# blairstar/NaturalDiffusion

Measured on AMD Instinct MI355X. Metric: images/sec at 15-step Natural Inference (CIFAR10 32x32, NCSN++), 3-stream throughput, higher is better.
Workload: dtype bf16; 1 GPU; CIFAR10 NI 15-step step_15_weight_173.npz B=512/GPU NCSN++ 61.8M bf16, ni_step fp64 history; nfe=15, batch_per_gpu=512, streams=3

## Files before the change

include/natinf_ncsnpp.h:

```cpp
#ifndef NATINF_NCSNPP_H
#define NATINF_NCSNPP_H

#include <stdint.h>
#include "natinf.h"

#ifdef __cplusplus
extern "C" {
#endif

typedef struct natinf_ncsnpp* natinf_ncsnpp_t;

#define NATINF_NCSNPP_KEEP_ACTIVATIONS 1
#define NATINF_NCSNPP_DDPM 2

int64_t natinf_ncsnpp_param_count(void);
int64_t natinf_ncsnpp_packed_bytes(void);
int64_t natinf_ncsnpp_handle_param_count(natinf_ncsnpp_t h);
int64_t natinf_ncsnpp_handle_packed_bytes(natinf_ncsnpp_t h);
int64_t natinf_ncsnpp_workspace_bytes(natinf_ncsnpp_t h, int max_batch);

int natinf_ncsnpp_create(natinf_ncsnpp_t* out, int flags);
int natinf_ncsnpp_destroy(natinf_ncsnpp_t h);

int natinf_ncsnpp_describe(natinf_ncsnpp_t h, char* buf, int cap);

int natinf_ncsnpp_load(natinf_ncsnpp_t h, const float* params_f32, int64_t n_params,
                       void* packed, int64_t packed_bytes, natinf_stream_t stream);

int natinf_ncsnpp_share(natinf_ncsnpp_t h, natinf_ncsnpp_t loaded);

int natinf_ncsnpp_forward(natinf_ncsnpp_t h, const float* x, const float* labels, float* out, int B,
                          void* workspace, int64_t workspace_bytes, natinf_stream_t stream);

int natinf_ncsnpp_describe_gemms(natinf_ncsnpp_t h, int B, char* buf, int cap);

int natinf_debug_gemm(int variant, int M, int N, int K0, int K1, int taps, int logW, int batch,
                      const void* a0, const void* a1, const void* b, const float* bias_n, void* c, int c_f32, float scale,
                      int iters, natinf_stream_t stream);
int natinf_debug_quant_fp8_rows(const float* w, void* q, float* row_scale, int rows, int cols, natinf_stream_t stream);
int natinf_debug_gemm_fused(int variant, int M, int N, int K, const void* a, const void* b, const float* bias_n, const float* bias_m,
                            const float* rowvec, const float* gate, int log_rows_per_sample, const void* resid_bf16, const float* resid_f32,
                            float scale, int act, void* c, int c_f32, float* gn_part, int* bm_out, int fp32_slab, natinf_stream_t stream);
int natinf_debug_set_conv_operand(int logW, const void* a1, int c1);
int natinf_debug_gemm_fp8(int M, int N, int K, const void* a8, const float* a_scale, const void* a_mx, const void* b8, const float* b_scale,
                          const float* bias_n, void* c, void* c_mx, int c_mode, int iters, natinf_stream_t stream);
int natinf_debug_conv_gn_up(int flags);
int natinf_debug_conv_gn_fin(float* fin_scale, float* fin_shift, const float* gamma, const float* beta, int channels_per_group, float mul);
int natinf_debug_conv_gn(int res, int B, int N, int cin, int c1, const void* x, const float* scale, const float* shift, const void* w_packed, void* w_frag,
                         const void* a1, const float* bias_n, const void* resid, float out_scale, void* out, float* gn_part, int iters,
                         natinf_stream_t stream);
#define NATINF_ATTN_BLOCK_OFF_WQKV 0
#define NATINF_ATTN_BLOCK_OFF_W3 393216
#define NATINF_ATTN_BLOCK_OFF_FOLD_WQK 524288
#define NATINF_ATTN_BLOCK_OFF_FOLD_WVO 786432
#define NATINF_ATTN_BLOCK_OFF_FOLD_CQ 1048576
#define NATINF_ATTN_BLOCK_OFF_FOLD_BO 1049600
#define NATINF_ATTN_BLOCK_OFF_WQK_PACKED 1050624
#define NATINF_ATTN_BLOCK_OFF_WVO_PACKED 1181696
#define NATINF_ATTN_BLOCK_PACKED_BYTES 1312768
#define NATINF_ATTN_BLOCK_SCRATCH_BYTES_PER_SAMPLE 393216
int natinf_debug_attn_block(int plan, int B, const void* x, int x_ld, const float* scale, const float* shift, const float* w, const float* bias,
                            void* packed, void* scratch, void* out, int o_ld, float out_scale, float* gn_part, natinf_stream_t stream);
int natinf_set_gemm_variant(int variant);
int natinf_set_gemm_epilogue(int fp32_slab);
int natinf_set_gemm_pref512(int on);
int natinf_set_gemm_half_issue(int on);
int natinf_set_gemm_round_model(int on);
int natinf_set_gemm_w128(int on);
int natinf_set_gemm_raster(int rows);
int natinf_set_fuse_gn(int on);
int natinf_set_conv_gn_wide(int mask);
int natinf_set_conv_gn_w128(int mask);
int natinf_set_conv_gn_w128_min_k(int shape, int k);
int natinf_set_conv_gn_regw(int on);
int natinf_set_fuse_up(int on);
int natinf_set_fuse_up_fold(int on);
int natinf_debug_fold_up_weights(const float* w, int N, int cin, float w_mul, float* out_f32, void* out_packed, natinf_stream_t stream);
int natinf_debug_conv_up_fold(int B, int N, int cin, const void* x, const float* scale, const float* shift, const float* w, void* w_packed, void* h_scratch,
                              const float* bias_n, const float* rowvec, float out_scale, void* out, float* gn_part, int iters, natinf_stream_t stream);
int natinf_set_fuse_head(int on);
int natinf_set_fuse_gn8(int on);
int natinf_set_fuse_gn4(int on);
int natinf_set_fuse_fin(int on);
int natinf_set_conv_gn_warm(int mask);
int natinf_set_attn256(int on);
int natinf_set_attn_proj(int on);
int natinf_set_attn_waves8(int on);
int natinf_set_attn_block(int on);
int natinf_set_attn_qkv(int on);
int natinf_set_conv_gn8_tile(int one_image);
int natinf_set_gemm_splitk(int on);
int natinf_debug_set_splitk_workspace(float* ws, int max_slices);
int natinf_debug_timestamps(void* dev_buf16);

int natinf_ncsnpp_profile(natinf_ncsnpp_t h, int enable);
int natinf_ncsnpp_profile_read(natinf_ncsnpp_t h, double* ms_by_class , int64_t* launches_by_class );

int natinf_gemm_profile(int enable);
int natinf_gemm_profile_read(char* buf, int cap);

int natinf_ncsnpp_debug_tap(natinf_ncsnpp_t h, int module_idx, float* out, int64_t capacity_elems,
                            natinf_stream_t stream);

int natinf_debug_gn_stats(const void* x, int ld, int C, int HW, int B, const float* gamma, const float* beta, float* scale, float* shift, float eps, float out_mul,
                          natinf_stream_t stream);
int natinf_debug_gn_finalize(const float* P0, int tps0, int quads0, const float* P1, int tps1, int quads1, int C, int HW, int B, const float* gamma, const float* beta,
                             float* scale, float* shift, float eps, float out_mul, natinf_stream_t stream);
int natinf_debug_gn_fold(const float* P, int tps, int quads, int fold, int B, float* out, natinf_stream_t stream);
int natinf_debug_gn_apply(const void* x, int ld, int C, int logW, int logHW, int B, const float* scale, const float* shift, void* y, void* xr, int act, int mode, int pad,
                          natinf_stream_t stream);
int natinf_debug_head_conv(const void* x, int ld, int B, const float* scale, const float* shift, const void* w16, const float* bias, float* out, natinf_stream_t stream);
int natinf_debug_time_embed(const float* labels, void* emb, int B, natinf_stream_t stream);
int natinf_debug_stem_im2col(const float* x, void* A, int B, natinf_stream_t stream);
int natinf_debug_pack_conv(const float* src, void* dst, int N, int Cin, int taps, int dst_ld, int koff, int tap_stride_c, int chunked, float wmul, natinf_stream_t stream);
int natinf_debug_pack_transpose(const float* src, void* dst, int K, int N, int dst_ld, natinf_stream_t stream);
int natinf_debug_nhwc_to_nchw(const void* x, int ld, int C, int HW, int B, float* out, natinf_stream_t stream);

#ifdef __cplusplus
}
#endif
#endif
```

naturaldiffusion_amd/_lib.py:

```python
from __future__ import annotations

import ctypes as C
import os
from pathlib import Path

os.environ.setdefault("GPU_MAX_HW_QUEUES", "8")

_HERE = Path(__file__).resolve().parent
LIB_PATH = Path(os.environ.get("NATINF_LIB", _HERE / "libnatinf.so"))

if not LIB_PATH.exists():
    raise ImportError(
        f"{LIB_PATH} not found: build it with `make -C {_HERE / 'csrc'}` "
        "(or `python -c 'import __graft_entry__ as g; g.build()'`). "
        "naturaldiffusion_amd has no CPU or eager-PyTorch fallback.")

lib = C.CDLL(str(LIB_PATH))

_p, _i32, _i64, _f32, _f64 = C.c_void_p, C.c_int, C.c_int64, C.c_float, C.c_double

SIGNATURES = {
    "natinf_abi_version": (C.c_int, []),
    "natinf_strerror": (C.c_char_p, [_i32]),
    "natinf_probe": (C.c_int, []),
    "natinf_step_f64hist": (C.c_int, [_p, _p, _p, _p, _p, _p, _p, _i32, _f64, _i32, _f64, _f64, _f32, _f32, _i64, _p]),
    "natinf_step_f32hist": (C.c_int, [_p, _p, _p, _p, _p, _p, _p, _i32, _f32, _i32, _f32, _f32, _f32, _f32, _i64, _p]),
    "natinf_weighted_sum_f64": (C.c_int, [_p, _p, _p, _p, _i32, _i64, _p]),
    "natinf_randn_philox_f32": (C.c_int, [_p, _i64, _i64, _p, _i64, _i64, C.c_uint64, _p]),
    "natinf_randn_philox_col_f32": (C.c_int, [_p, _i64, _i64, _p, _i64, _i64, C.c_uint64, C.c_uint32, _p]),
    "natinf_step_f64hist_noise": (C.c_int, [_p, _p, _p, _p, _p, _p, _p, _i32, _f64, _p, _p, _i32, _i32, _f64, _f64, _f32,
                                            C.c_uint64, _p, _i64, _i64, _i64, _i64, _p]),
    "natinf_known_blend_f32": (C.c_int, [_p, _p, _p, _p, _i64, _i64, _f32, _f32, C.c_uint32, C.c_uint64, _p, _i64, _i64, _i64, _i64, _p]),
    "natinf_step_f64hist_inpaint": (C.c_int, [_p, _p, _p, _p, _p, _p, _p, _i32, _f64, _p, _p, _i32, _i32, _f64, _f64, _f32,
                                              C.c_uint64, _p, _i64, _i64, _i64, _i64, _p, _p, _i64, _i64, _f32, _f32, C.c_uint32, _p]),
    "natinf_x0_threshold_f64": (C.c_int, [_p, _p, _i64, _i64, _i32, _f64, _f64, _p]),
    "natinf_step_f64hist_x0fix": (C.c_int, [_p, _p, _p, _p, _p, _p, _p, _i32, _f64, _p, _p, _i32, _i32, _f64, _f64, _f32,
                                            C.c_uint64, _p, _i64, _i64, _i64, _i64, _p, _p, _i64, _i64, _f32, _f32, C.c_uint32,
                                            _i32, _f64, _f64, _p, _p]),
    "natinf_color_blend_f32": (C.c_int, [_p, _p, _p, _i64, _p, _p, _f32, _f32, C.c_uint32, C.c_uint64, _p, _i64, _i64, _i64, _i64, _p]),
    "natinf_step_f64hist_colorize": (C.c_int, [_p, _p, _p, _p, _p, _p, _p, _i32, _f64, _p, _p, _i32, _i32, _f64, _f64, _f32,
                                               C.c_uint64, _p, _i64, _i64, _i64, _i64, _p, _i64, _p, _p, _f32, _f32, C.c_uint32, _p]),
    "natinf_to_pixel_u8": (C.c_int, [_p, _p, _i32, _i32, _i32, _i32, _i32, _p]),
    "natinf_step_f32prod": (C.c_int, [_p, _p, _p, _f32, _i64, _i64, _p, _p, _p, _p, _p, _i32, _f32, _p, _p, _i32,
                                      _i32, _f32, _f32, _i64, _p]),
    "natinf_step_f32prod_noise": (C.c_int, [_p, _p, _p, _f32, _i64, _i64, _p, _p, _p, _p, _p, _i32, _f32, _p, _p, _i32,
                                            _i32, _f32, _f32, C.c_uint64, _p, _i64, _i64, _i64, _p]),
    "natinf_step_f32prod_noise_guided": (C.c_int, [_p, _p, _p, _p, _p, _i32, _i64, _i64, _p, _p, _p, _p, _p, _i32, _f32, _p, _p, _i32,
                                                   _i32, _f32, _f32, C.c_uint64, _p, _i64, _i64, _i64, _p]),
    "natinf_step_f32prod_inpaint": (C.c_int, [_p, _p, _p, _p, _p, _i32, _i64, _i64, _p, _p, _p, _p, _p, _i32, _f32, _p, _p, _i32,
                                              _i32, _f32, _f32, C.c_uint64, _p, _i64, _i64, _i64,
                                              _p, _p, _i64, _i64, _f32, _f32, C.c_uint32, _p]),
    "natinf_weighted_sum_f32prod": (C.c_int, [_p, _p, _p, _p, _i32, _i64, _p]),
    "natinf_step_f16chain": (C.c_int, [_p, _p, _p, _p, _p, _p, _p, _p, _p, _i32, _f32, _f32, _i32, _f32, _f32, _f32,
                                       _f32, _i32, _i64, _p]),
    "natinf_step_f16chain_guided": (C.c_int, [_p, _p, _p, _p, _p, _i32, _i64, _p, _p, _p, _p, _p, _p, _i32, _f32, _f32, _i32, _f32, _f32,
                                              _f32, _i32, _i64, _p]),
    "natinf_known_blend_f16": (C.c_int, [_p, _p, _p, _p, _p, _i64, _i64, _f32, _f32, C.c_uint32, C.c_uint64, _p, _i64, _i64, _i64, _i64, _p]),
    "natinf_step_f16chain_inpaint": (C.c_int, [_p, _p, _p, _p, _p, _i32, _i64, _p, _p, _p, _p, _p, _p, _i32, _f32, _f32, _i32, _f32, _f32,
                                               _f32, _i32, _i64, _p, _p, _i64, _i64, C.c_uint32, C.c_uint64, _p, _i64, _i64, _p]),
    "natinf_weighted_mean_f16": (C.c_int, [_p, _p, _p, _p, _i32, _f32, _i64, _p]),
    "natinf_flow_input_f16": (C.c_int, [_p, _p, _p, _f32, _f32, _i64, _p]),
    "natinf_ncsnpp_param_count": (C.c_int64, []),
    "natinf_ncsnpp_workspace_bytes": (C.c_int64, [_p, _i32]),
    "natinf_ncsnpp_packed_bytes": (C.c_int64, []),
    "natinf_ncsnpp_handle_param_count": (_i64, [_p]),
    "natinf_ncsnpp_handle_packed_bytes": (_i64, [_p]),
    "natinf_ncsnpp_create": (C.c_int, [C.POINTER(_p), _i32]),
    "natinf_ncsnpp_describe": (C.c_int, [_p, C.c_char_p, _i32]),
    "natinf_ncsnpp_destroy": (C.c_int, [_p]),
    "natinf_ncsnpp_load": (C.c_int, [_p, _p, _i64, _p, _i64, _p]),
    "natinf_ncsnpp_share": (C.c_int, [_p, _p]),
    "natinf_ncsnpp_forward": (C.c_int, [_p, _p, _p, _p, _i32, _p, _i64, _p]),
    "natinf_ncsnpp_debug_tap": (C.c_int, [_p, _i32, _p, _i64, _p]),
    "natinf_ncsnpp_describe_gemms": (C.c_int, [_p, _i32, C.c_char_p, _i32]),
    "natinf_debug_gemm": (C.c_int, [_i32, _i32, _i32, _i32, _i32, _i32, _i32, _i32, _p, _p, _p, _p, _p, _i32, _f32, _i32, _p]),
    "natinf_set_gemm_variant": (C.c_int, [_i32]),
    "natinf_debug_timestamps": (C.c_int, [_p]),
    "natinf_set_gemm_epilogue": (C.c_int, [_i32]),
    "natinf_debug_gemm_fused": (C.c_int, [_i32, _i32, _i32, _i32, _p, _p, _p, _p, _p, _p, _i32, _p, _p, _f32, _i32, _p, _i32, _p, _p, _i32, _p]),
    "natinf_set_gemm_pref512": (C.c_int, [_i32]),
    "natinf_set_gemm_half_issue": (C.c_int, [_i32]),
    "natinf_set_gemm_raster": (C.c_int, [_i32]),
    "natinf_set_gemm_round_model": (C.c_int, [_i32]),
    "natinf_set_gemm_w128": (C.c_int, [_i32]),
    "natinf_set_fuse_gn": (C.c_int, [_i32]),
    "natinf_set_conv_gn_wide": (C.c_int, [_i32]),
    "natinf_set_attn_block": (C.c_int, [_i32]),
    "natinf_set_conv_gn_w128": (C.c_int, [_i32]),
    "natinf_set_conv_gn_w128_min_k": (C.c_int, [_i32, _i32]),
    "natinf_set_conv_gn_regw": (C.c_int, [_i32]),
    "natinf_set_fuse_up": (C.c_int, [_i32]),
    "natinf_set_fuse_up_fold": (C.c_int, [_i32]),
    "natinf_debug_fold_up_weights": (C.c_int, [_p, _i32, _i32, _f32, _p, _p, _p]),
    "natinf_debug_conv_up_fold": (C.c_int, [_i32, _i32, _i32, _p, _p, _p, _p, _p, _p, _p, _p, _f32, _p, _p, _i32, _p]),
    "natinf_set_fuse_head": (C.c_int, [_i32]),
    "natinf_set_fuse_gn8": (C.c_int, [_i32]),
    "natinf_set_fuse_gn4": (C.c_int, [_i32]),
    "natinf_set_fuse_fin": (C.c_int, [_i32]),
    "natinf_set_attn_proj": (C.c_int, [_i32]),
    "natinf_set_attn_waves8": (C.c_int, [_i32]),
    "natinf_set_attn_qkv": (C.c_int, [_i32]),
    "natinf_set_conv_gn_warm": (C.c_int, [_i32]),
    "natinf_set_attn256": (C.c_int, [_i32]),
    "natinf_set_conv_gn8_tile": (C.c_int, [_i32]),
    "natinf_set_gemm_splitk": (C.c_int, [_i32]),
    "natinf_debug_set_splitk_workspace": (C.c_int, [_p, _i32]),
    "natinf_debug_set_conv_operand": (C.c_int, [_i32, _p, _i32]),
    "natinf_debug_conv_gn": (C.c_int, [_i32, _i32, _i32, _i32, _i32, _p, _p, _p, _p, _p, _p, _p, _p, _f32, _p, _p, _i32, _p]),
    "natinf_debug_conv_gn_up": (C.c_int, [_i32]),
    "natinf_debug_conv_gn_fin": (C.c_int, [_p, _p, _p, _p, _i32, _f32]),
    "natinf_debug_attn_block": (C.c_int, [_i32, _i32, _p, _i32, _p, _p, _p, _p, _p, _p, _p, _i32, _f32, _p, _p]),
    "natinf_debug_gn_stats": (C.c_int, [_p, _i32, _i32, _i32, _i32, _p, _p, _p, _p, _f32, _f32, _p]),
    "natinf_debug_gn_finalize": (C.c_int, [_p, _i32, _i32, _p, _i32, _i32, _i32, _i32, _i32, _p, _p, _p, _p, _f32, _f32, _p]),
    "natinf_debug_gn_fold": (C.c_int, [_p, _i32, _i32, _i32, _i32, _p, _p]),
    "natinf_debug_gn_apply": (C.c_int, [_p, _i32, _i32, _i32, _i32, _i32, _p, _p, _p, _p, _i32, _i32, _i32, _p]),
    "natinf_debug_head_conv": (C.c_int, [_p, _i32, _i32, _p, _p, _p, _p, _p, _p]),
    "natinf_debug_time_embed": (C.c_int, [_p, _p, _i32, _p]),
    "natinf_debug_stem_im2col": (C.c_int, [_p, _p, _i32, _p]),
    "natinf_debug_pack_conv": (C.c_int, [_p, _p, _i32, _i32, _i32, _i32, _i32, _i32, _i32, _f32, _p]),
    "natinf_debug_pack_transpose": (C.c_int, [_p, _p, _i32, _i32, _i32, _p]),
    "natinf_debug_nhwc_to_nchw": (C.c_int, [_p, _i32, _i32, _i32, _i32, _p, _p]),
    "natinf_ncsnpp_profile": (C.c_int, [_p, _i32]),
    "natinf_ncsnpp_profile_read": (C.c_int, [_p, C.POINTER(C.c_double), C.POINTER(C.c_int64)]),
    "natinf_debug_quant_fp8_rows": (C.c_int, [_p, _p, _p, _i32, _i32, _p]),
    "natinf_debug_gemm_fp8": (C.c_int, [_i32, _i32, _i32, _p, _p, _p, _p, _p, _p, _p, _p, _i32, _i32, _p]),
    "natinf_dit_create": (C.c_int, [C.POINTER(_p), _i32, _i32, _i32, _i32]),
    "natinf_dit_create_sized": (C.c_int, [C.POINTER(_p), _i32, _i32, _i32, _i32, _i32]),
    "natinf_dit_input_size": (C.c_int, [_p]),
    "natinf_dit_attention_bf16": (C.c_int, [_p, _p, _p, _i32, _p, _i32, _i32, _i32, _i32, _i32, _i32, _p]),
    "natinf_dit_destroy": (C.c_int, [_p]),
    "natinf_dit_param_count": (C.c_int64, [_p]),
    "natinf_dit_packed_bytes": (C.c_int64, [_p]),
    "natinf_dit_workspace_bytes": (C.c_int64, [_p, _i32]),
    "natinf_dit_load": (C.c_int, [_p, _p, _i64, _p, _i64, _p]),
    "natinf_dit_forward": (C.c_int, [_p, _p, _p, _p, _p, _i32, _p, _i64, _p]),
    "natinf_dit_stream_sites": (C.c_int, [_p]),
    "natinf_dit_stream_status_reset": (C.c_int, [_p, _p, _p]),
    "natinf_dit_stream_status": (C.c_int, [_p, _p, _p, _p]),
    "natinf_debug_ln_modulate": (C.c_int, [_p, _i32, _p, _p, _i32, _p, _p, _p, _i32, _i64, _i32, C.POINTER(_i32), _p]),
    "natinf_debug_softmax_rows": (C.c_int, [_i32, _p, _p, _i32, _i64, _p]),
    "natinf_mmdit_create": (C.c_int, [C.POINTER(_p), _i32, _i32, _i32, _i32, _i32, _i32, _i32, _i32]),
    "natinf_mmdit_destroy": (C.c_int, [_p]),
    "natinf_mmdit_param_count": (C.c_int64, [_p]),
    "natinf_mmdit_packed_bytes": (C.c_int64, [_p]),
    "natinf_mmdit_workspace_bytes": (C.c_int64, [_p, _i32]),
    "natinf_mmdit_load": (C.c_int, [_p, _p, _i64, _p, _i64, _p]),
    "natinf_mmdit_forward": (C.c_int, [_p, _p, _p, _p, _p, _p, _i32, _p, _i64, _p]),
    "natinf_mmdit_stream_sites": (C.c_int, [_p]),
    "natinf_mmdit_stream_status_reset": (C.c_int, [_p, _p, _p]),
    "natinf_mmdit_stream_status": (C.c_int, [_p, _p, _p, _p]),
    "natinf_attention_hd64_bf16": (C.c_int, [_p, _p, _i32, _i64, _p, _p, _i32, _i64, _i32, _i32, _i32, _i32, C.c_float, _p]),
    "natinf_debug_attention_hd64_fp8out": (C.c_int, [_p, _p, _i32, _i64, _p, _p, _p, _i32, _i32, _i32, _i32, C.c_float, _p]),
    "natinf_inception_create": (C.c_int, [_p, _i32, _i32]),
    "natinf_inception_destroy": (C.c_int, [_p]),
    "natinf_set_inception_conv": (C.c_int, [_i32]),
    "natinf_debug_conv_ring": (C.c_int, [_i32] * 14 + [_p, _p, _p, _p, _p, _p, _i32, _p]),
    "natinf_debug_inc_stem": (C.c_int, [_p, _i32, _i32, _i32, _i32, _i32, _i32, _p, _p]),
    "natinf_debug_inc_pool": (C.c_int, [_i32] * 8 + [_p, _i32, _p, _i32, _p]),
    "natinf_debug_inc_global_avg": (C.c_int, [_i32, _i32, _i32, _i32, _p, _p, _p]),
    "natinf_debug_inc_pack": (C.c_int, [_i32, _p, _p, _p, _p, _p] + [_i32] * 7 + [_p, _p, _p, _p]),
    "natinf_debug_inc_im2col": (C.c_int, [_i32] * 11 + [_p, _p, _p]),
    "natinf_inception_param_count": (_i64, [_p]),
    "natinf_inception_packed_bytes": (_i64, [_p]),
    "natinf_inception_workspace_bytes": (_i64, [_p, _i32]),
    "natinf_inception_load": (C.c_int, [_p, _p, _i64, _p, _i64, _p]),
    "natinf_inception_forward": (C.c_int, [_p, _p, _i32, _p, _i32, _p, _i64, _p]),
    "natinf_gemm_profile": (C.c_int, [_i32]),
    "natinf_gemm_profile_read": (C.c_int, [_p, _i32]),
    "natinf_set_mmdit_stream16": (C.c_int, [_i32]),
    "natinf_set_dit_stream16": (C.c_int, [_i32]),
    "natinf_set_mmdit_text_flat": (C.c_int, [_i32]),
    "natinf_attention_profile": (C.c_int, [_i32]),
    "natinf_set_mmdit_text_stream": (C.c_int, [_i32]),
    "natinf_set_flash_mode": (C.c_int, [_i32]),
    "natinf_attention_profile_read": (C.c_int, [_p, _p]),
    "natinf_vae_create": (C.c_int, [C.POINTER(_p), _i32, _i32]),
    "natinf_vae_destroy": (C.c_int, [_p]),
    "natinf_vae_param_count": (C.c_int64, [_p]),
    "natinf_vae_packed_bytes": (C.c_int64, [_p]),
    "natinf_vae_workspace_bytes": (C.c_int64, [_p, _i32]),
    "natinf_vae_load": (C.c_int, [_p, _p, _i64, _p, _i64, _p]),
# ... 100 lines not shown
```

naturaldiffusion_amd/csrc/attn_blk256.h:

```cpp
#pragma once
#include "attn_qkv.h"
#include "attn256.h"

namespace ncsn {

constexpr int ABLK_STAGES = 4, ABLK_LDS_BYTES = ABLK_STAGES * A256_STAGE + QKV_BIAS_BYTES;

__device__ __forceinline__ float dpp_row_sum_tau(float a, float b) {
    asm volatile("s_nop 4" : "+v"(a), "+v"(b));
    a += __builtin_bit_cast(float, __builtin_amdgcn_update_dpp(0, __builtin_bit_cast(int, a), 0x128, 0xF, 0xF, true));
    b += __builtin_bit_cast(float, __builtin_amdgcn_update_dpp(0, __builtin_bit_cast(int, b), 0x128, 0xF, 0xF, true));
    asm volatile("" : "+v"(a), "+v"(b));
    a += __builtin_bit_cast(float, __builtin_amdgcn_update_dpp(0, __builtin_bit_cast(int, a), 0xB1, 0xF, 0xF, true));
    b += __builtin_bit_cast(float, __builtin_amdgcn_update_dpp(0, __builtin_bit_cast(int, b), 0xB1, 0xF, 0xF, true));
    asm volatile("" : "+v"(a), "+v"(b));
    a += __builtin_bit_cast(float, __builtin_amdgcn_update_dpp(0, __builtin_bit_cast(int, a), 0x4E, 0xF, 0xF, true));
    b += __builtin_bit_cast(float, __builtin_amdgcn_update_dpp(0, __builtin_bit_cast(int, b), 0x4E, 0xF, 0xF, true));
    asm volatile("" : "+v"(a), "+v"(b));
    float v = a + b;
    asm volatile("s_nop 1" : "+v"(v));
    v += __builtin_bit_cast(float, __builtin_amdgcn_update_dpp(0, __builtin_bit_cast(int, v), 0x141, 0xF, 0xF, true));
    asm volatile("" : "+v"(v));
    return v;
}
// ... 237 lines not shown
            for (int i = 0; i < 4; ++i) { of[g][kc][i] = (bf16)oacc[g][2 * kc][i]; of[g][kc][4 + i] = (bf16)oacc[g][2 * kc + 1][i]; }
    __builtin_amdgcn_sched_barrier(0);
    int le;
    asm volatile("v_mbcnt_lo_u32_b32 %0, -1, 0\n\tv_mbcnt_hi_u32_b32 %0, -1, %0" : "=v"(le));
    const int re = le & 15, qe = le >> 4;
    float2* const sred = reinterpret_cast<float2*>(smem);
    float2 part[16];
#pragma unroll
    for (int t = 0; t < 4; ++t) {
        asm volatile("s_waitcnt vmcnt(0)" ::: "memory");
        __syncthreads();
        if (t + 3 < 4) issue(2 * NKT + t + 3);
        __builtin_amdgcn_sched_barrier(0);
        const unsigned char* sW = smem + ((2 * NKT + t) & 3) * A256_STAGE;
        f32x4 a3[2][4];
#pragma unroll
        for (int ntl = 0; ntl < 4; ++ntl) { a3[0][ntl] = f32x4{0.f, 0.f, 0.f, 0.f}; a3[1][ntl] = f32x4{0.f, 0.f, 0.f, 0.f}; }
#pragma unroll
        for (int ntl = 0; ntl < 4; ++ntl)
#pragma unroll
            for (int kc = 0; kc < 8; ++kc) {
                const bf16x8 fa = *reinterpret_cast<const bf16x8*>(sW + (ntl * 8 + kc) * 1024 + le * 16);
                a3[0][ntl] = __builtin_amdgcn_mfma_f32_16x16x32_bf16(fa, of[0][kc], a3[0][ntl], 0, 0, 0);
                a3[1][ntl] = __builtin_amdgcn_mfma_f32_16x16x32_bf16(fa, of[1][kc], a3[1][ntl], 0, 0, 0);
            }
#pragma unroll
        for (int pr = 0; pr < 2; ++pr) {
            const int n = 64 * t + 32 * pr + 8 * qe;
            const float4 b0 = *reinterpret_cast<const float4*>(b3 + n), b1 = *reinterpret_cast<const float4*>(b3 + n + 4);
            float s0[2], ss0[2], s1[2], ss1[2];
#pragma unroll
            for (int g = 0; g < 2; ++g) {
                const int64_t row = (int64_t)b * T + tok0 + 8 * (re >> 2) + 4 * g + (re & 3);
                const bf16x8 rx = *reinterpret_cast<const bf16x8*>(x + row * x_ld + n);
                const f32x4 lo = a3[g][2 * pr], hi = a3[g][2 * pr + 1];
                float v[8] = {lo[0] + b0.x, lo[1] + b0.y, lo[2] + b0.z, lo[3] + b0.w, hi[0] + b1.x, hi[1] + b1.y, hi[2] + b1.z, hi[3] + b1.w};
                bf16x8 w;
#pragma unroll
                for (int i = 0; i < 8; ++i) { v[i] = (v[i] + (float)rx[i]) * out_scale; w[i] = (bf16)v[i]; }
                *reinterpret_cast<bf16x8*>(o + row * o_ld + n) = w;
                s0[g] = (v[0] + v[1]) + (v[2] + v[3]);  ss0[g] = (v[0] * v[0] + v[1] * v[1]) + (v[2] * v[2] + v[3] * v[3]);
                s1[g] = (v[4] + v[5]) + (v[6] + v[7]);  ss1[g] = (v[4] * v[4] + v[5] * v[5]) + (v[6] * v[6] + v[7] * v[7]);
            }
            part[4 * t + 2 * pr] = make_float2(dpp_row_sum_tau(s0[0], s0[1]), dpp_row_sum_tau(ss0[0], ss0[1]));
            part[4 * t + 2 * pr + 1] = make_float2(dpp_row_sum_tau(s1[0], s1[1]), dpp_row_sum_tau(ss1[0], ss1[1]));
        }
    }
    if (gn_part) {
        __syncthreads();
        if (re == 0) {
#pragma unroll
            for (int k = 0; k < 16; ++k) sred[wave * 64 + 8 * (k >> 1) + 2 * qe + (k & 1)] = part[k];
        }
        __syncthreads();
        if (tid < 64) {
            float s = 0.f, ss = 0.f;
#pragma unroll
            for (int w = 0; w < 8; ++w) { s += sred[w * 64 + tid].x; ss += sred[w * 64 + tid].y; }
            gn_part[(int64_t)b * gn_quads + tid] = make_float2(s, ss);
        }
    }
}

constexpr int ABLK2_IMG = 131072, ABLK2_LDS_BYTES = ABLK2_IMG + A256_STAGE;
static_assert(4 * QKV_STAGE <= ABLK2_IMG && ABLK2_LDS_BYTES <= 163840, "the q phase's four stages inside the image's bytes; image + one W3 tile in 160 KB");

__global__ __launch_bounds__(256) void k_attn_fold_w(const float* __restrict__ w0, const float* __restrict__ w1, const float* __restrict__ w2, const float* __restrict__ w3,
                                                      const float* __restrict__ b0, const float* __restrict__ b2, const float* __restrict__ b3,
                                                      float* __restrict__ wqk, float* __restrict__ cq, float* __restrict__ wvo, float* __restrict__ bo)
{
    const int o = threadIdx.x, i = blockIdx.x;
    float a = 0.f, c = 0.f;
    if (i < 256) {
        for (int m = 0; m < 256; ++m) { a += w0[i * 256 + m] * w1[o * 256 + m]; c += w2[i * 256 + m] * w3[m * 256 + o]; }
        wqk[i * 256 + o] = a; wvo[i * 256 + o] = c;
    } else {
        for (int m = 0; m < 256; ++m) { a += b0[m] * w1[o * 256 + m]; c += b2[m] * w3[m * 256 + o]; }
        cq[o] = a; bo[o] = c + b3[o];
    }
}

__global__ __launch_bounds__(512, 1) void k_attn_blk256_v2(const bf16* __restrict__ x, int x_ld, const float* __restrict__ gsc, const float* __restrict__ gsh,
                                                          const bf16* __restrict__ wqf, const float* __restrict__ cq, float scale, const bf16* __restrict__ wvof,
                                                          const float* __restrict__ bo, bf16* __restrict__ o, int o_ld, float out_scale, float2* __restrict__ gn_part, int gn_quads)
{
    constexpr int T = 256, C = 256, NTQ = 8;
    extern __shared__ __attribute__((aligned(16))) unsigned char smem[];
    lds_poison();
    typedef __attribute__((address_space(3))) void lds_void;
    typedef __attribute__((address_space(3))) unsigned char lds_u8;
    const int tid = threadIdx.x, lane = tid & 63, r = lane & 15, q = lane >> 4;
    const int wave = __builtin_amdgcn_readfirstlane(tid >> 6);
    const int b = blockIdx.x;
    const int tok0 = wave * 32;
    const unsigned lds0 = (unsigned)(uintptr_t)((lds_u8*)smem);

    constexpr int NST = 4, AHEAD = NST - 1;
    auto issue_w = [&](int i) __attribute__((always_inline)) {
        unsigned char* st = smem + (i & (NST - 1)) * QKV_STAGE;
        int l;
        asm volatile("v_mbcnt_lo_u32_b32 %0, -1, 0\n\tv_mbcnt_hi_u32_b32 %0, -1, %0" : "=v"(l));
        const bf16* base = wqf + (int64_t)i * (QKV_STAGE / 2);
#pragma unroll
        for (int j = 0; j < QKV_STAGE / 8192; ++j) {
            const int p = wave * (QKV_STAGE / 8192) + j;
            __builtin_amdgcn_global_load_lds(base + p * 512 + l * 8, (lds_void*)(st + p * 1024), 16, 0, 0);
        }
    };
    issue_w(0); issue_w(1); issue_w(2);
    float* const sBias = reinterpret_cast<float*>(smem + ABLK2_IMG);
    const unsigned lds_bias = lds0 + ABLK2_IMG;
    if (tid < 64) reinterpret_cast<float4*>(sBias)[tid] = reinterpret_cast<const float4*>(cq)[tid];

    bf16x8 qf[2][8];
    {
        bf16x8 hf[2][8];
        {
            const bf16* xb = x + ((int64_t)b * T + tok0 + 8 * (r >> 2) + (r & 3)) * x_ld + 8 * q;
            bf16x8 raw[2][8];
#pragma unroll
            for (int g = 0; g < 2; ++g)
#pragma unroll
                for (int kc = 0; kc < 8; ++kc) raw[g][kc] = *reinterpret_cast<const bf16x8*>(xb + (int64_t)(4 * g) * x_ld + 32 * kc);
            const float* sc = gsc + (int64_t)b * C + 8 * q;
            const float* sh = gsh + (int64_t)b * C + 8 * q;
#pragma unroll
            for (int kc = 0; kc < 8; ++kc) {
                const float4 s0 = *reinterpret_cast<const float4*>(sc + 32 * kc), s1 = *reinterpret_cast<const float4*>(sc + 32 * kc + 4);
                const float4 h0 = *reinterpret_cast<const float4*>(sh + 32 * kc), h1 = *reinterpret_cast<const float4*>(sh + 32 * kc + 4);
                const float s[8] = {s0.x, s0.y, s0.z, s0.w, s1.x, s1.y, s1.z, s1.w}, h[8] = {h0.x, h0.y, h0.z, h0.w, h1.x, h1.y, h1.z, h1.w};
#pragma unroll
                for (int g = 0; g < 2; ++g)
#pragma unroll
                    for (int j = 0; j < 8; ++j) hf[g][kc][j] = (bf16)((float)raw[g][kc][j] * s[j] + h[j]);
            }
        }
        int le;
        asm volatile("v_mbcnt_lo_u32_b32 %0, -1, 0\n\tv_mbcnt_hi_u32_b32 %0, -1, %0" : "=v"(le));
        const int qe = le >> 4;
        auto q_tile = [&](auto t_tag, bf16x8 (&w)[2]) __attribute__((always_inline)) {
            constexpr int t = decltype(t_tag)::value;
            constexpr int ahead = 2 * ((t + 1 < NTQ) + (t + 2 < NTQ));
            asm volatile("s_waitcnt vmcnt(%0) lgkmcnt(0)" :: "n"(ahead) : "memory");
            __builtin_amdgcn_s_barrier();
            if constexpr (t + AHEAD < NTQ) issue_w(t + AHEAD);
            __builtin_amdgcn_sched_barrier(0);
            const unsigned char* sW = smem + (t & (NST - 1)) * QKV_STAGE;
            f32x4 a[2][2];
#pragma unroll
            for (int ntl = 0; ntl < 2; ++ntl) {
                a[ntl][0] = f32x4{0.f, 0.f, 0.f, 0.f}; a[ntl][1] = a[ntl][0];
#pragma unroll
                for (int kc = 0; kc < 8; ++kc) {
                    const bf16x8 fa = *reinterpret_cast<const bf16x8*>(sW + (ntl * 8 + kc) * 1024 + le * 16);
                    a[ntl][0] = __builtin_amdgcn_mfma_f32_16x16x32_bf16(fa, hf[0][kc], a[ntl][0], 0, 0, 0);
                    a[ntl][1] = __builtin_amdgcn_mfma_f32_16x16x32_bf16(fa, hf[1][kc], a[ntl][1], 0, 0, 0);
                }
            }
            const int n = 32 * t + 8 * qe;
            f32x4 b0, b1;
            asm volatile("ds_read_b128 %0, %2\n\tds_read_b128 %1, %2 offset:16" : "=&v"(b0), "=&v"(b1) : "v"(lds_bias + (unsigned)n * 4u) : "memory");
            asm volatile("s_waitcnt lgkmcnt(0)" : "+v"(b0), "+v"(b1) :: "memory");
#pragma unroll
            for (int g = 0; g < 2; ++g)
#pragma unroll
                for (int i = 0; i < 4; ++i) { w[g][i] = (bf16)(a[0][g][i] + b0[i]); w[g][4 + i] = (bf16)(a[1][g][i] + b1[i]); }
        };
// ... 89 lines not shown
            for (int cc = 0; cc < 2; ++cc)
#pragma unroll
                for (int dt = 0; dt < 16; ++dt) {
                    const unsigned a = abase + (unsigned)((64 * vt + 32 * cc) * 512) + ((((unsigned)dt ^ kh) << 5) | (kl << 4));
                    const s16x4 lo = __builtin_amdgcn_ds_read_tr16_b64_v4i16((lds_s16x4*)(uintptr_t)a);
                    const s16x4 hi = __builtin_amdgcn_ds_read_tr16_b64_v4i16((lds_s16x4*)(uintptr_t)(a + 4 * 512));
                    typedef short s16x8 __attribute__((ext_vector_type(8)));
                    const s16x8 both = {lo[0], lo[1], lo[2], lo[3], hi[0], hi[1], hi[2], hi[3]};
                    const bf16x8 fv = __builtin_bit_cast(bf16x8, both);
                    oacc[0][dt] = __builtin_amdgcn_mfma_f32_16x16x32_bf16(fv, pf[0][2 * vt + cc], oacc[0][dt], 0, 0, 0);
                    oacc[1][dt] = __builtin_amdgcn_mfma_f32_16x16x32_bf16(fv, pf[1][2 * vt + cc], oacc[1][dt], 0, 0, 0);
                }
    }
    bf16x8 of[2][8];
#pragma unroll
    for (int g = 0; g < 2; ++g)
#pragma unroll
        for (int kc = 0; kc < 8; ++kc)
#pragma unroll
            for (int i = 0; i < 4; ++i) { of[g][kc][i] = (bf16)oacc[g][2 * kc][i]; of[g][kc][4 + i] = (bf16)oacc[g][2 * kc + 1][i]; }
    __builtin_amdgcn_sched_barrier(0);
    asm volatile("s_waitcnt lgkmcnt(0)" ::: "memory");
    __syncthreads();
    issue3(1); issue3(2); issue3(3);

    int le;
    asm volatile("v_mbcnt_lo_u32_b32 %0, -1, 0\n\tv_mbcnt_hi_u32_b32 %0, -1, %0" : "=v"(le));
    const int re = le & 15, qe = le >> 4;
    float2 part[16];
#pragma unroll
    for (int t = 0; t < 4; ++t) {
        if (t == 0) {
            asm volatile("s_waitcnt vmcnt(0)" ::: "memory");
            __syncthreads();
        }
        __builtin_amdgcn_sched_barrier(0);
        const unsigned char* sW = t == 0 ? smem + ABLK2_IMG : smem + (t - 1) * A256_STAGE;
        f32x4 a3[2][4];
#pragma unroll
        for (int ntl = 0; ntl < 4; ++ntl) { a3[0][ntl] = f32x4{0.f, 0.f, 0.f, 0.f}; a3[1][ntl] = f32x4{0.f, 0.f, 0.f, 0.f}; }
#pragma unroll
        for (int ntl = 0; ntl < 4; ++ntl)
#pragma unroll
            for (int kc = 0; kc < 8; ++kc) {
                const bf16x8 fa = *reinterpret_cast<const bf16x8*>(sW + (ntl * 8 + kc) * 1024 + le * 16);
                a3[0][ntl] = __builtin_amdgcn_mfma_f32_16x16x32_bf16(fa, of[0][kc], a3[0][ntl], 0, 0, 0);
                a3[1][ntl] = __builtin_amdgcn_mfma_f32_16x16x32_bf16(fa, of[1][kc], a3[1][ntl], 0, 0, 0);
            }
#pragma unroll
        for (int pr = 0; pr < 2; ++pr) {
            const int n = 64 * t + 32 * pr + 8 * qe;
            const float4 b0 = *reinterpret_cast<const float4*>(bo + n), b1 = *reinterpret_cast<const float4*>(bo + n + 4);
            float s0[2], ss0[2], s1[2], ss1[2];
#pragma unroll
            for (int g = 0; g < 2; ++g) {
                const int64_t row = (int64_t)b * T + tok0 + 8 * (re >> 2) + 4 * g + (re & 3);
                const bf16x8 rx = *reinterpret_cast<const bf16x8*>(x + row * x_ld + n);
                const f32x4 lo = a3[g][2 * pr], hi = a3[g][2 * pr + 1];
                float v[8] = {lo[0] + b0.x, lo[1] + b0.y, lo[2] + b0.z, lo[3] + b0.w, hi[0] + b1.x, hi[1] + b1.y, hi[2] + b1.z, hi[3] + b1.w};
                bf16x8 w;
#pragma unroll
                for (int i = 0; i < 8; ++i) { v[i] = (v[i] + (float)rx[i]) * out_scale; w[i] = (bf16)v[i]; }
                *reinterpret_cast<bf16x8*>(o + row * o_ld + n) = w;
                s0[g] = (v[0] + v[1]) + (v[2] + v[3]);  ss0[g] = (v[0] * v[0] + v[1] * v[1]) + (v[2] * v[2] + v[3] * v[3]);
                s1[g] = (v[4] + v[5]) + (v[6] + v[7]);  ss1[g] = (v[4] * v[4] + v[5] * v[5]) + (v[6] * v[6] + v[7] * v[7]);
            }
            part[4 * t + 2 * pr] = make_float2(dpp_row_sum_tau(s0[0], s0[1]), dpp_row_sum_tau(ss0[0], ss0[1]));
            part[4 * t + 2 * pr + 1] = make_float2(dpp_row_sum_tau(s1[0], s1[1]), dpp_row_sum_tau(ss1[0], ss1[1]));
        }
    }
    if (gn_part) {
        float2* const sred = reinterpret_cast<float2*>(smem + 3 * A256_STAGE);
        __syncthreads();
        if (re == 0) {
#pragma unroll
            for (int k = 0; k < 16; ++k) sred[wave * 64 + 8 * (k >> 1) + 2 * qe + (k & 1)] = part[k];
        }
        __syncthreads();
        if (tid < 64) {
            float s = 0.f, ss = 0.f;
#pragma unroll
            for (int w = 0; w < 8; ++w) { s += sred[w * 64 + tid].x; ss += sred[w * 64 + tid].y; }
            gn_part[(int64_t)b * gn_quads + tid] = make_float2(s, ss);
        }
    }
}

}
```

naturaldiffusion_amd/csrc/engine_core.h:

```cpp
#pragma once
#include <functional>
#include <map>
#include <vector>

#include "natinf_ncsnpp.h"
#include "gemm_launch.h"

namespace ncsn {

__global__ void k_transpose_f32(const float* __restrict__ src, float* __restrict__ dst, int N, int K)
{
    const int64_t i = (int64_t)blockIdx.x * blockDim.x + threadIdx.x;
    if (i >= (int64_t)N * K) return;
    const int n = (int)(i / K), k = (int)(i - (int64_t)n * K);
    dst[(int64_t)k * N + n] = src[i];
}
}

namespace {

inline int ilog2(int v) { int l = 0; while ((1 << l) < v) ++l; return l; }
inline int64_t align_up(int64_t v, int64_t a) { return (v + a - 1) / a * a; }

struct TRef { int64_t off = -1; int C = 0, ld = 0, res = 0, coff = 0, pad = 0; };

struct Ctx {
    int B; unsigned char* ws; const unsigned char* wp; hipStream_t stream;
    const float* x; const float* labels; float* out;
    int* part_bm;
    hipStream_t stream2 = nullptr; hipEvent_t* ev = nullptr;
    unsigned char* fin_done = nullptr;
    uint32_t* guard = nullptr;
    uint32_t* site(int i) const { return guard ? guard + 2 * i : nullptr; }
    bf16* act(const TRef& t) const { return reinterpret_cast<bf16*>(ws + t.off * B) + t.coff; }
    template <class T> T* at(int64_t off) const { return reinterpret_cast<T*>(ws + off * B); }
    template <class T> const T* w(int64_t off) const { return reinterpret_cast<const T*>(wp + off); }
};
using OpFn = std::function<void(const Ctx&)>;

struct PackCtx { const float* params; unsigned char* packed; hipStream_t stream; };
using PackFn = std::function<void(const PackCtx&)>;

struct Arena {
    bool keep = false; int64_t top = 0, peak = 0;
    std::map<int64_t, int64_t> free_;
    std::map<int64_t, int64_t> live_;
    int64_t alloc(int64_t bytes) {
        bytes = align_up(bytes, 256);
        if (!keep)
            for (auto it = free_.begin(); it != free_.end(); ++it)
                if (it->second >= bytes) {
                    const int64_t off = it->first, rest = it->second - bytes;
                    free_.erase(it);
                    if (rest) free_[off + bytes] = rest;
                    live_[off] = bytes;
                    return off;
                }
        const int64_t off = top; top += bytes; if (top > peak) peak = top;
        live_[off] = bytes;
        return off;
    }
    void release(int64_t off) {
        if (keep || off < 0) return;
        auto it = live_.find(off);
        if (it == live_.end()) return;
        int64_t o = off, s = it->second;
        live_.erase(it);
        auto nx = free_.lower_bound(o);
        if (nx != free_.end() && o + s == nx->first) { s += nx->second; nx = free_.erase(nx); }
        if (nx != free_.begin()) { auto pv = std::prev(nx); if (pv->first + pv->second == o) { o = pv->first; s += pv->second; free_.erase(pv); } }
        if (o + s == top) top = o; else free_[o] = s;
    }
};

}

struct EngineCore {
    int64_t n_params = 0, packed_bytes = 0, ws_per_image = 0;
    std::vector<OpFn> ops;
    std::vector<PackFn> packs;
    const unsigned char* packed = nullptr;
    bool configured = false;
    std::vector<int> part_bm{128};
    int guard_sites = 0;
    int64_t guard_bytes() const { return guard_sites ? align_up((int64_t)guard_sites * 8, 256) : 0; }
    int64_t workspace_bytes(int max_batch) const { return ws_per_image * (int64_t)max_batch + guard_bytes(); }
    int status_reset(void* ws, hipStream_t s) const {
        if (!guard_sites || !ws) return NATINF_EINVAL;
        return hipMemsetAsync(ws, 0, (size_t)guard_sites * 8, s) == hipSuccess ? NATINF_OK : NATINF_ELAUNCH;
    }
    int status_read(const void* ws, uint32_t* out_dev, hipStream_t s) const {
        if (!guard_sites || !ws || !out_dev) return NATINF_EINVAL;
        return hipMemcpyAsync(out_dev, ws, (size_t)guard_sites * 8, hipMemcpyDeviceToDevice, s) == hipSuccess ? NATINF_OK : NATINF_ELAUNCH;
    }
    int load(const float* params_f32, int64_t n, void* dst, int64_t dst_bytes, hipStream_t s) {
        if (!params_f32 || !dst || n != n_params || dst_bytes < packed_bytes) return NATINF_EINVAL;
        PackCtx p{params_f32, reinterpret_cast<unsigned char*>(dst), s};
        for (const auto& f : packs) f(p);
        packed = reinterpret_cast<const unsigned char*>(dst);
        return hipGetLastError() == hipSuccess ? NATINF_OK : NATINF_ELAUNCH;
    }
    int run(const float* x, const float* t, float* out, int B, void* ws, int64_t ws_bytes, hipStream_t s, hipStream_t s2 = nullptr, hipEvent_t* ev = nullptr) {
        if (!x || !t || !out || !ws || B <= 0) return NATINF_EINVAL;
        if (!packed) return NATINF_ESTATE;
        if (ws_bytes < workspace_bytes(B)) return NATINF_EINVAL;
        if (!configured) { if (!configure_gemm_kernels()) return NATINF_ENODEV; configured = true; }
        Ctx c{B, reinterpret_cast<unsigned char*>(ws) + guard_bytes(), packed, s, x, t, out, part_bm.data()};
        c.stream2 = s2; c.ev = ev;
        if (guard_sites) { c.guard = reinterpret_cast<uint32_t*>(ws); g_launch_error = 0; }
        for (const auto& f : ops) f(c);
        if (guard_sites && g_launch_error) { g_launch_error = 0; return NATINF_ESTATE; }
        return hipGetLastError() == hipSuccess ? NATINF_OK : NATINF_ELAUNCH;
    }
};

// ... 59 lines not shown
```

naturaldiffusion_amd/csrc/gemm_launch.h:

```cpp
#pragma once
#include <hip/hip_runtime.h>
#include <stdint.h>
#include <stdio.h>
#include <string.h>
#include <string>
#include <type_traits>
#include <utility>
#include <vector>

#include "ncsnpp_kernels.h"
#include "gemm_dma.h"
#include "gemm_w128.h"
#include "conv_gn2.h"
#include "gemm_fp8.h"

using namespace ncsn;

bool configure_conv_ring();
namespace { bool configure_ncsnpp_kernels();
            bool configure_dit_attention();
            bool configure_flash_attention(); }
namespace ncsn_sg { bool configure(); bool has_tile(int variant); void launch_tile(const void* gemm_args, int variant, int raster, void* stream);
                    void launch_fp8(const void* gemm_args, int mxa, int w128, int raster, void* stream); void launch_splitk_reduce(const void* gemm_args, int slices, void* stream);
                    void launch_patch_embed(const float* z, const float* Wt, const float* bias, const float* pos, float* x, int C, int g, int D, int64_t rows, int x_f16, uint32_t* guard, void* stream); }
namespace ncsn_upf { bool configure(); void launch(const void* gemm_args, int epi, void* stream); void fold(const float* w, void* dst_bf16, float* dst_f32, int N, int Cin, float wmul, void* stream); }
namespace ncsn_cg3 { bool configure(); int tile_rows(int shape); int tile_cols(int shape); void launch(const void* gemm_args, int shape, int epi, void* stream); }

namespace {

int g_epi_fp32_slab = 0;
GemmArgs gemm_defaults() {
    GemmArgs g;
    memset(&g, 0, sizeof(g));
    g.epi_fp32_slab = g_epi_fp32_slab;
    g.taps = 1; g.batch = 1; g.scale = 1.0f; g.act = ACT_NONE; g.c_mode = OUT_BF16;
    return g;
}
constexpr int NUM_CU = 256;
enum GemmVariant {
    V_AUTO = 0, V_GENERIC = 1,
    V_DMA_256x256 = 2, V_DMA_256x128 = 3, V_DMA_128x128 = 4,
    V_RING_256x256 = 5, V_RING_256x128 = 6, V_RING_128x128 = 7,
    V_RING_64x128 = 8,
    V_RING_256x128_W4 = 9,
    V_DMA_256x128_W4 = 10,
    V_DMA_256x256_S = 11, V_DMA_128x128_S = 12,
    V_DMA_512x128 = 13,
    V_PATCH_256x256 = 14, V_PATCH_256x128 = 15,
    V_DMA_256x256_P = 16, V_DMA_256x128W4_P = 18,
    V_DMA_128x128_P = 17,
    V_8PH_256x256 = 19, V_8PH_NOPRIO = 20, V_8PH_READFIRST = 21, V_8PH_BOTH = 22,
    V_FP8_256x256 = 23,
    V_ABL_NODMA = 24, V_ABL_NOMFMA = 25,
    V_DMA_256x256_H = 26, V_DMA_512x128_H = 27,
    V_CONV_GN = 28,
    V_W128 = 29,
    V_W128_A = 30, V_W128_D = 31, V_W128_X = 32,
    V_COUNT
};
const char* variant_name(int v) {
    static const char* n[] = {"auto", "generic128", "dma256x256", "dma256x128", "dma128x128", "ring256x256", "ring256x128",
                              "ring128x128", "ring64x128", "ring256x128w4", "dma256x128w4", "dma256x256s", "dma128x128s", "dma512x128", "patch256x256", "patch256x128", "dma256x256p", "dma128x128p", "dma256x128w4p", "gemm8ph", "gemm8ph_np", "gemm8ph_rf", "gemm8ph_nprf", "fp8_256x256", "abl_nodma", "abl_nomfma", "dma256x256h", "dma512x128h", "conv_gn", "w128_256x256", "w128_a", "w128_d", "w128_x"};
    return v >= 0 && v < V_COUNT ? n[v] : "?";
}
unsigned long long* g_dbg_ts = nullptr;
int g_force_variant = V_AUTO;
int g_round_model = 1;
int g_round_model_w128 = 13;
int g_pref_512 = 1;
std::string* g_record = nullptr;

int g_raster_g = 8;
template <class Cfg, class K>
inline void launch_tiles(K kernel, const GemmArgs& g0, hipStream_t s) {
    const int nM = (g0.M + Cfg::BM_ - 1) / Cfg::BM_, nN = (g0.N + Cfg::BN_ - 1) / Cfg::BN_;
    GemmArgs g = g0;
    g.raster_g = (g_raster_g > 1 && nN >= 8 && nM >= g_raster_g) ? g_raster_g : 0;
    hipLaunchKernelGGL(kernel, dim3(nM * nN, 1, g.batch), dim3(Cfg::THREADS), Cfg::LDS_BYTES, s, g);
}
template <class Cfg, class K>
inline bool set_lds(K kernel) {
    return hipFuncSetAttribute(reinterpret_cast<const void*>(kernel), hipFuncAttributeMaxDynamicSharedMemorySize, Cfg::LDS_BYTES) == hipSuccess;
}
int g_cg_warm = 15;

constexpr unsigned EPI_ALL = 0x1FF;
template <unsigned MASK, int E, class F> inline void epi_case(F&& f) { if constexpr ((MASK >> E) & 1u) f(std::integral_constant<int, E>{}); }
template <unsigned MASK, class F> inline bool for_each_epi(F&& f) {
    bool ok = true;
    auto one = [&](auto tag) { ok = ok && f(tag); };
    epi_case<MASK, 0>(one); epi_case<MASK, 1>(one); epi_case<MASK, 2>(one); epi_case<MASK, 3>(one); epi_case<MASK, 4>(one);
    epi_case<MASK, 5>(one); epi_case<MASK, 6>(one); epi_case<MASK, 7>(one); epi_case<MASK, 8>(one);
    return ok;
}
#define NATINF_EPI_OF(tag) decltype(tag)::value

template <class... F> struct FamList {};
template <class Fam> bool configure_family() {
    return for_each_epi<Fam::EPI>([](auto t) { return set_lds<typename Fam::Cfg>(Fam::template kernel<NATINF_EPI_OF(t)>()); });
}
template <class... F> bool configure_families(FamList<F...>) { return (configure_family<F>() && ...); }
template <class Fam> void launch_family(int e, const GemmArgs& g, hipStream_t s) {
    for_each_epi<Fam::EPI>([&](auto t) {
        if (NATINF_EPI_OF(t) != e) return true;
        launch_tiles<typename Fam::Cfg>(Fam::template kernel<NATINF_EPI_OF(t)>(), g, s);
        return false;
    });
}
// ... 310 lines not shown
```

naturaldiffusion_amd/csrc/ncsnpp.hip:

```cpp
#include <hip/hip_runtime.h>
#include <stdint.h>
#include <stdio.h>
#include <string.h>
#include <stdlib.h>
#include <functional>
#include <map>
#include <memory>
#include <string>
#include <vector>

#include "natinf_ncsnpp.h"
#include "gemm_launch.h"
#include "engine_core.h"
#include "head_conv.h"
#include "attn256.h"
#include "attn_qkv.h"
#include "attn_blk256.h"

namespace {

constexpr int NF = 128, IMG = 32, TEMB = 512, NLEVEL = 4;
constexpr int CH_MULT[NLEVEL] = {1, 2, 2, 2};
constexpr float GN_EPS = 1e-6f;
constexpr float INV_SQRT2 = 0.70710678118654752440f;
inline bool attn_at(int res) { return res == 16; }

enum Kind { K_LIN, K_CONV, K_RES, K_ATTN, K_GN, K_DOWN, K_UP };
const char* kind_name(int k) { static const char* n[] = {"lin", "conv", "res", "attn", "gn", "down", "up"}; return n[k]; }

struct Mod { int idx, kind, cin, cout, up, down, res; int64_t poff; };

enum { CLS_GEMM = 0, CLS_OTHER = 1, CLS_CONV_GN = 2, CLS_CONV_GN8 = 3, N_CLS = 4 };

int g_fuse_head = 1;
constexpr int ATTN_BLK_DEFAULT = 2;
int g_attn_blk = ATTN_BLK_DEFAULT;
int g_attn_qkv = 1;
int g_attn_w8 = 1;
int g_attn_proj = 1;
int g_fuse_gn8 = 1;
int g_fuse_fin = 3;
int g_fuse_gn4 = 1;
int g_fuse_gn = 1;
constexpr int UP_FOLD_DEFAULT = 1;
int g_fuse_up_fold = UP_FOLD_DEFAULT;
int g_fuse_up = 1;

}

struct natinf_ncsnpp : EngineCore {
    int flags = 0;
    std::vector<Mod> mods;
    std::vector<int> op_cls;
    bool prof = false;
    struct Rec { hipEvent_t a, b; int cls; };
    std::vector<Rec> recs;
    std::vector<hipEvent_t> pool;
    std::map<int, TRef> taps;
    uint64_t plan_sig = 0;
    int last_B = 0; unsigned char* last_ws = nullptr;
    std::vector<unsigned char> fin_done;
};

namespace {

bool configure_ncsnpp_kernels() {
    return hipFuncSetAttribute(reinterpret_cast<const void*>(&k_head_conv), hipFuncAttributeMaxDynamicSharedMemorySize, HeadConvCfg::LDS_BYTES) == hipSuccess &&
           hipFuncSetAttribute(reinterpret_cast<const void*>(&k_qkv256), hipFuncAttributeMaxDynamicSharedMemorySize, QKV_LDS_BYTES) == hipSuccess &&
           hipFuncSetAttribute(reinterpret_cast<const void*>(&k_attn256<false>), hipFuncAttributeMaxDynamicSharedMemorySize, A256_LDS_BYTES) == hipSuccess &&
           hipFuncSetAttribute(reinterpret_cast<const void*>(&k_attn256<true>), hipFuncAttributeMaxDynamicSharedMemorySize, A256_LDS_BYTES) == hipSuccess &&
           hipFuncSetAttribute(reinterpret_cast<const void*>(&k_attn256<true, 8>), hipFuncAttributeMaxDynamicSharedMemorySize, A256_LDS_BYTES) == hipSuccess &&
           hipFuncSetAttribute(reinterpret_cast<const void*>(&k_attn_blk256), hipFuncAttributeMaxDynamicSharedMemorySize, ABLK_LDS_BYTES) == hipSuccess &&
           hipFuncSetAttribute(reinterpret_cast<const void*>(&k_attn_blk256_v2), hipFuncAttributeMaxDynamicSharedMemorySize, ABLK2_LDS_BYTES) == hipSuccess;
}

struct AttnBlk256 {
    int plan = 0;
    int B = 0;
    const bf16* x = nullptr; int x_ld = 0;
    const float* sc = nullptr; const float* sh = nullptr;
    const bf16* wqkvf = nullptr; const float* bqk = nullptr; const float* bv = nullptr; bf16* qk = nullptr; bf16* vT = nullptr;
    const bf16* w3f = nullptr; const float* b3 = nullptr;
    const bf16* wqf2 = nullptr; const float* cq2 = nullptr; const bf16* wvof2 = nullptr; const float* bo2 = nullptr;
    bf16* out = nullptr; int o_ld = 0; float out_scale = 1.0f;
    float2* gn_part = nullptr; int gn_quads = 0;
};
void pack_attn_qkv_w(const float* w0, const float* w1, const float* w2, bf16* wqkvf, hipStream_t s) {
    hipLaunchKernelGGL(k_pack_qkv_w, dim3(3 * 256), dim3(256), 0, s, w0, w1, w2, wqkvf);
}
void pack_attn_w3(const float* w3, bf16* w3f, hipStream_t s) { hipLaunchKernelGGL(k_pack_attn_w3, dim3(256), dim3(256), 0, s, w3, w3f); }
void pack_attn_fold(const float* w0, const float* w1, const float* w2, const float* w3, const float* b0, const float* b2, const float* b3,
                    float* fq, float* cq, float* fv, float* bo, bf16* wqf2, bf16* wvof2, hipStream_t s) {
    hipLaunchKernelGGL(k_attn_fold_w, dim3(257), dim3(256), 0, s, w0, w1, w2, w3, b0, b2, b3, fq, cq, fv, bo);
    hipLaunchKernelGGL(k_pack_qkv_w, dim3(256), dim3(256), 0, s, (const float*)fq, (const float*)fq, (const float*)fq, wqf2, 1);
    hipLaunchKernelGGL(k_pack_attn_w3, dim3(256), dim3(256), 0, s, (const float*)fv, wvof2);
}
void launch_attn_qkv256(const AttnBlk256& a, hipStream_t s) {
    hipLaunchKernelGGL(k_qkv256, dim3((unsigned)a.B), dim3(512), QKV_LDS_BYTES, s, a.x, a.x_ld, a.sc, a.sh, a.wqkvf, a.bqk, a.bv, a.qk, a.vT);
}
int launch_attn_blk256(const AttnBlk256& a, hipStream_t s) {
    constexpr int C = 256;
    if (a.plan == 2) {
        hipLaunchKernelGGL(k_attn_blk256_v2, dim3((unsigned)a.B), dim3(512), ABLK2_LDS_BYTES, s, a.x, a.x_ld, a.sc, a.sh,
                           a.wqf2, a.cq2, 1.0f / sqrtf((float)C), a.wvof2, a.bo2, a.out, a.o_ld, a.out_scale, a.gn_part, a.gn_quads);
        return 256;
    }
    if (a.plan == 1) {
        hipLaunchKernelGGL(k_attn_blk256, dim3((unsigned)a.B), dim3(512), ABLK_LDS_BYTES, s, a.x, a.x_ld, a.sc, a.sh,
                           a.wqkvf, a.bqk, a.bv, a.qk, a.vT, 1.0f / sqrtf((float)C), a.w3f, a.b3, a.out, a.o_ld, a.out_scale, a.gn_part, a.gn_quads);
        return 256;
    }
    if (g_attn_w8) {
        hipLaunchKernelGGL((k_attn256<true, 8>), dim3((unsigned)a.B), dim3(512), A256_LDS_BYTES, s, (const bf16*)a.qk, 2 * C, C, (const bf16*)a.vT, a.out, a.o_ld,
                           1.0f / sqrtf((float)C), a.w3f, a.b3, a.x, a.x_ld, a.out_scale, a.gn_part, a.gn_quads);
        return 256;
    }
    hipLaunchKernelGGL(k_attn256<true>, dim3((unsigned)(2 * a.B)), dim3(256), A256_LDS_BYTES, s, (const bf16*)a.qk, 2 * C, C, (const bf16*)a.vT, a.out, a.o_ld,
                       1.0f / sqrtf((float)C), a.w3f, a.b3, a.x, a.x_ld, a.out_scale, a.gn_part, a.gn_quads);
    return 128;
}

struct Builder : PlanBuilder {
    natinf_ncsnpp& E;
    int dense_total = 0; int64_t dense_w = 0, dense_b = 0, dense_out = 0;

    const bool ddpm;
    const int NUM_RES;
    const float res_scale;
    explicit Builder(natinf_ncsnpp& e) : PlanBuilder(e), E(e), ddpm((e.flags & NATINF_NCSNPP_DDPM) != 0), NUM_RES(ddpm ? 2 : 4), res_scale(ddpm ? 1.0f : INV_SQRT2) {
        arena.keep = (e.flags & NATINF_NCSNPP_KEEP_ACTIVATIONS) != 0;
    }

    void op(int cls, OpFn f) { E.ops.push_back(std::move(f)); E.op_cls.push_back(cls); }

    void pack_conv(int64_t src, int64_t dst, int N, int Cin, int taps, int dst_ld, int koff, int tapstride, float wmul = 1.0f) {
        const int chunked = taps == 9 && Cin % BK == 0;
        E.packs.push_back([=](const PackCtx& p) {
            const int64_t n = (int64_t)N * Cin * taps;
            hipLaunchKernelGGL(k_pack_conv, dim3(grid1d(n, 256, 1 << 30)), dim3(256), 0, p.stream, p.params + src,
                               reinterpret_cast<bf16*>(p.packed + dst), N, Cin, taps, dst_ld, koff, tapstride, chunked, wmul);
        });
    }
    void pack_frag(int64_t src_packed, int64_t dst, int N, int ld, int cin, int c1) {
        E.packs.push_back([=](const PackCtx& p) {
            const int64_t n = (int64_t)(N / 16) * (9 * (cin / 32) + c1 / 32) * 64;
            hipLaunchKernelGGL(k_pack_frag, dim3(grid1d(n, 256, 1 << 30)), dim3(256), 0, p.stream, reinterpret_cast<const bf16*>(p.packed + src_packed),
                               reinterpret_cast<bf16*>(p.packed + dst), N, ld, cin, c1);
        });
    }
    void pack_fold_up(int64_t src, int64_t dst, int N, int Cin, float wmul) {
        E.packs.push_back([=](const PackCtx& p) {
            ncsn_upf::fold(p.params + src, p.packed + dst, nullptr, N, Cin, wmul, (void*)p.stream);
        });
    }
    void pack_transpose(int64_t src, int64_t dst, int K, int N, int dst_ld) {
        E.packs.push_back([=](const PackCtx& p) {
            hipLaunchKernelGGL(k_pack_transpose, dim3(grid1d((int64_t)K * N, 256, 1 << 30)), dim3(256), 0, p.stream,
                               p.params + src, reinterpret_cast<bf16*>(p.packed + dst), K, N, dst_ld);
        });
    }
    void pack_zero(int64_t dst, int64_t n) {
        E.packs.push_back([=](const PackCtx& p) {
            hipLaunchKernelGGL(k_fill_bf16_zero, dim3(grid1d(n, 256, 1 << 30)), dim3(256), 0, p.stream,
                               reinterpret_cast<bf16*>(p.packed + dst), n);
        });
    }

    struct GN { int64_t gamma, beta; };
    GN take_gn(int C) { GN g; g.gamma = pack_f32(take(C), C); g.beta = pack_f32(take(C), C); return g; }

    void emit_gn_stats(const TRef& x, GN gn, int64_t& sc, int64_t& sh, float out_mul = 1.0f) {
        if (emit_gn_from_parts(x, gn, sc, sh, out_mul)) return;
        const int HW = x.res * x.res;
        op(CLS_OTHER, [=](const Ctx& c) {
            hipLaunchKernelGGL(k_gn_stats, dim3(c.B), dim3(256), 0, c.stream, c.act(x), x.ld, x.C, HW,
                               c.w<float>(gn.gamma), c.w<float>(gn.beta), c.at<float>(sc), c.at<float>(sh), GN_EPS, out_mul);
        });
    }
    void emit_gn_apply(const TRef& x, int64_t sc, int64_t sh, const TRef& y, const TRef* xr, int act, int mode) {
        const int logW = ilog2(x.res), logHW = 2 * logW;
        const int rd = mode == RS_UP ? 2 * x.res : (mode == RS_DOWN ? x.res / 2 : x.res);
        const int rows_per_img = rd + 2 * y.pad;
        const TRef xrr = xr ? *xr : TRef();
        op(CLS_OTHER, [=](const Ctx& c) {
            hipLaunchKernelGGL(k_gn_apply, dim3((unsigned)((rows_per_img + GN_ROWS - 1) / GN_ROWS), (unsigned)c.B), dim3(256), 0, c.stream, c.act(x), x.ld, x.C,
                               logW, logHW, c.at<float>(sc), c.at<float>(sh), c.act(y),
                               xrr.off >= 0 ? c.act(xrr) : (bf16*)nullptr, act, mode, y.pad);
        });
    }
    TRef new_act(int res, int C, int pad = 0) {
        TRef t; t.off = arena.alloc((int64_t)(res + 2 * pad) * (res + 2 * pad) * C * 2); t.C = C; t.ld = C; t.res = res; t.pad = pad;
        return t;
    }

    void emit_res(const Mod& m, const TRef& x, const TRef& out) {
        const int cin = m.cin, cout = m.cout;
        const int ro = m.up ? m.res * 2 : (m.down ? m.res / 2 : m.res);
        const bool shortcut = cin != cout || m.up || m.down;
        const GN gn0 = take_gn(cin);
        const int64_t p_c0w = take((int64_t)cout * cin * 9), p_c0b = take(cout);
        const int64_t p_dw = take((int64_t)cout * TEMB), p_db = take(cout);
        const GN gn1 = take_gn(cout);
        const int64_t p_c1w = take((int64_t)cout * cout * 9), p_c1b = take(cout);
        const int64_t p_c2w = shortcut ? take((int64_t)cout * cin) : -1, p_c2b = shortcut ? take(cout) : -1;

        const int K0a = 9 * cin, K1tot = 9 * cout + (shortcut ? cin : 0);
        const bool fusable_res = g_fuse_gn && (ro == 32 || ro == 16 || (ro == 8 && g_fuse_gn8 && cout % 256 == 0) || (ro == 4 && g_fuse_gn4 && cout % 256 == 0));
        const bool fuse1 = fusable_res && cout % BK == 0;
        const bool fuse_up = fuse1 && ro > 8 && g_fuse_up && m.up && cin % BK == 0 && cout % 128 == 0;
        const bool fold_up = fuse_up && g_fuse_up_fold && !ddpm && ro == 2 * UPFOLD_W && cout == UPFOLD_BN;
        const bool fuse = (fusable_res && !m.up && !m.down && cin % BK == 0) || (fuse_up && !fold_up);
        const float LOG2E = 1.4426950408889634f, LN2 = 0.6931471805599453f;
        const float gn_mul = fuse ? -LOG2E : 1.0f, w_mul = fuse ? -LN2 : 1.0f, gn_mul1 = fuse1 ? -LOG2E : 1.0f, w_mul1 = fuse1 ? -LN2 : 1.0f;
        const int64_t w0 = wres((int64_t)cout * (fold_up ? 16 * cin : K0a) * 2), w1 = wres((int64_t)cout * K1tot * 2);
        if (fold_up) pack_fold_up(p_c0w, w0, cout, cin, w_mul);
        else pack_conv(p_c0w, w0, cout, cin, 9, K0a, 0, cin, w_mul);
        pack_conv(p_c1w, w1, cout, cout, 9, K1tot, 0, cout, w_mul1);
        if (shortcut && !ddpm) pack_conv(p_c2w, w1, cout, cin, 1, K1tot, 9 * cout, cin);
        if (shortcut && ddpm) pack_transpose(p_c2w, w1 + (int64_t)9 * cout * 2, cin, cout, K1tot);
        const int64_t w0f = (fuse && cout % 16 == 0) ? wres((int64_t)cout * K0a * 2) : -1, w1f = (fuse1 && cout % 16 == 0) ? wres((int64_t)cout * K1tot * 2) : -1;
        if (w0f >= 0) pack_frag(w0, w0f, cout, K0a, cin, 0);
        if (w1f >= 0) pack_frag(w1, w1f, cout, K1tot, cout, shortcut ? cin : 0);
        const int64_t b0 = pack_f32(p_c0b, cout), b1 = pack_f32(p_c1b, cout, shortcut ? p_c2b : -1);
        const int drow = dense_rows_next;
        pack_conv(p_dw, dense_w + (int64_t)drow * TEMB * 2, cout, TEMB, 1, TEMB, 0, TEMB);
        pack_f32_at(p_db, cout, dense_b + (int64_t)drow * 4);
        dense_rows_next += cout;

        const int64_t own_sc = arena.alloc((int64_t)std::max(cin, cout) * 4), own_sh = arena.alloc((int64_t)std::max(cin, cout) * 4);
        int64_t sc = own_sc, sh = own_sh;
        emit_gn_stats(x, gn0, sc, sh, gn_mul);
        TRef h, xr;
        if (fold_up) {
            h = new_act(m.res, cin, 1);
            emit_gn_apply(x, sc, sh, h, nullptr, ACT_SILU, RS_NONE);
        } else if (!fuse) {
            h = new_act(ro, cin, 1);
            if (m.up || m.down) xr = new_act(ro, cin);
            emit_gn_apply(x, sc, sh, h, (m.up || m.down) ? &xr : nullptr, ACT_SILU, m.up ? RS_UP : (m.down ? RS_DOWN : RS_NONE));
        }

        const int SK_MAX = 4;
        const int64_t skws = (ro <= 8) ? arena.alloc((int64_t)SK_MAX * ro * ro * cout * 4) : -1;
        TRef t = new_act(ro, cout);
        const Part pt = register_output(t, fuse);
        const int logW = ilog2(ro), logHW = 2 * logW, HWo = ro * ro;
        const int dtotal = dense_total; const int64_t dout = dense_out;
        op((fuse || fold_up) ? (ro <= 8 ? CLS_CONV_GN8 : CLS_CONV_GN) : CLS_GEMM, [=](const Ctx& c) {
            GemmArgs g = gemm_defaults();
            if (fold_up) {
                g.a0 = c.act(h); g.a0_ld = h.ld; g.a0_padded = 1; g.a0_C = cin; g.taps = 4; g.logW = logW - 1; g.logHW = logHW - 2;
                g.M = c.B * (HWo / 4); g.N = 4 * cout; g.b = c.w<bf16>(w0); g.b_ld = 4 * cin; g.bias_n = c.w<float>(b0);
                g.rowvec = c.at<float>(dout) + drow; g.rowvec_ld = dtotal; g.log_rows_per_sample = logHW - 2;
                g.c = c.act(t); g.c_ld = t.ld;
                if (pt.valid) { g.gn_part = c.at<float>(pt.off); g.gn_quads = pt.quads; }
                const int bm = launch_gemm(g, c.stream);
                if (pt.valid) c.part_bm[pt.id] = bm;
                return;
            }
            if (fuse) { g.a0 = c.act(x); g.a0_ld = x.ld; g.gn_scale = c.at<float>(sc); g.gn_shift = c.at<float>(sh); g.gn_ld = cin; g.gn_folded = 1; g.a0_up = fuse_up; }
            else { g.a0 = c.act(h); g.a0_ld = h.ld; g.a0_padded = 1; }
            g.a0_C = cin; g.taps = 9; g.logW = logW; g.logHW = logHW;
            g.M = c.B * HWo; g.N = cout; g.b = c.w<bf16>(w0); g.b_ld = K0a;
            if (w0f >= 0) g.b_frag = c.w<bf16>(w0f);
            g.bias_n = c.w<float>(b0);
            g.rowvec = c.at<float>(dout) + drow; g.rowvec_ld = dtotal; g.log_rows_per_sample = logHW;
            if (skws >= 0) { g.splitk_ws = c.at<float>(skws); g.splitk_max = SK_MAX; }
            g.c = c.act(t); g.c_ld = t.ld;
            if (pt.valid) { g.gn_part = c.at<float>(pt.off); g.gn_quads = pt.quads; set_fin(g, pt, c); }
            g_fin_written = false;
            const int bm = launch_gemm(g, c.stream);
            if (pt.valid) c.part_bm[pt.id] = bm;
            if (pt.fin && pt.fin->check) c.fin_done[pt.id] = g_fin_written;
        });
        if (!fuse) arena.release(h.off);
        int64_t sc1 = own_sc, sh1 = own_sh;
        emit_gn_stats(t, gn1, sc1, sh1, gn_mul1);
        TRef u;
        if (!fuse1) {
            u = new_act(ro, cout, 1);
            emit_gn_apply(t, sc1, sh1, u, nullptr, ACT_SILU, RS_NONE);
            arena.release(t.off);
        }
        if (pt.valid) arena.release(pt.off);
        const TRef xs = ((m.up || m.down) && !fuse_up) ? xr : x;
        const float rs = res_scale;
        const Part po = register_output(out, fuse1);
        op(fuse1 ? (ro <= 8 ? CLS_CONV_GN8 : CLS_CONV_GN) : CLS_GEMM, [=](const Ctx& c) {
            GemmArgs g = gemm_defaults();
            if (fuse1) { g.a0 = c.act(t); g.a0_ld = t.ld; g.gn_scale = c.at<float>(sc1); g.gn_shift = c.at<float>(sh1); g.gn_ld = cout; g.gn_folded = 1; }
            else { g.a0 = c.act(u); g.a0_ld = u.ld; g.a0_padded = 1; }
            g.a0_C = cout; g.taps = 9; g.logW = logW; g.logHW = logHW;
            if (shortcut) { g.a1 = c.act(xs); g.a1_ld = xs.ld; g.a1_C = cin; g.a1_up = fuse_up; }
            else { g.resid = c.act(xs); g.resid_ld = xs.ld; }
            g.M = c.B * HWo; g.N = cout; g.b = c.w<bf16>(w1); g.b_ld = K1tot;
            if (w1f >= 0) g.b_frag = c.w<bf16>(w1f);
            g.bias_n = c.w<float>(b1); g.scale = rs;
            if (skws >= 0) { g.splitk_ws = c.at<float>(skws); g.splitk_max = SK_MAX; }
            g.c = c.act(out); g.c_ld = out.ld;
            if (po.valid) { g.gn_part = c.at<float>(po.off); g.gn_quads = po.quads; set_fin(g, po, c); }
            g_fin_written = false;
            const int bm = launch_gemm(g, c.stream);
            if (po.valid) c.part_bm[po.id] = bm;
            if (po.fin && po.fin->check) c.fin_done[po.id] = g_fin_written;
        });
        if (skws >= 0) arena.release(skws);
        if (fuse1) arena.release(t.off); else arena.release(u.off);
        if ((m.up || m.down) && !fuse_up) arena.release(xr.off);
        arena.release(own_sc); arena.release(own_sh);
        if (sc != own_sc) { arena.release(sc); arena.release(sh); }
        if (sc1 != own_sc) { arena.release(sc1); arena.release(sh1); }
        E.taps[m.idx] = out;
    }

    void emit_attn(const Mod& m, const TRef& x, const TRef& out) {
        const int C = m.cin, T = m.res * m.res;
        const GN gn = take_gn(C);
        int64_t pw[4], pb[4];
        for (int i = 0; i < 4; ++i) { pw[i] = take((int64_t)C * C); pb[i] = take(C); }
        const int64_t wqk = wres((int64_t)2 * C * C * 2), wv = wres((int64_t)C * C * 2), w3 = wres((int64_t)C * C * 2);
        pack_transpose(pw[0], wqk, C, C, C);
        pack_transpose(pw[1], wqk + (int64_t)C * C * 2, C, C, C);
        pack_transpose(pw[2], wv, C, C, C);
        pack_transpose(pw[3], w3, C, C, C);
        const int64_t bqk = wres((int64_t)2 * C * 4);
        pack_f32_at(pb[0], C, bqk); pack_f32_at(pb[1], C, bqk + (int64_t)C * 4);
        const int64_t bv = pack_f32(pb[2], C), b3 = pack_f32(pb[3], C);

        const int64_t own_sc = arena.alloc((int64_t)C * 4), own_sh = arena.alloc((int64_t)C * 4);
        int64_t sc = own_sc, sh = own_sh;
        emit_gn_stats(x, gn, sc, sh);
        const bool fuse_qkv = T == 256 && C == 256 && g_attn_qkv;
        TRef h = new_act(m.res, C);
        if (!fuse_qkv) emit_gn_apply(x, sc, sh, h, nullptr, ACT_NONE, RS_NONE);
        const int64_t qk = arena.alloc((int64_t)T * 2 * C * 2), vT = arena.alloc((int64_t)C * T * 2);
        const bool blk = fuse_qkv && g_attn_proj && g_attn_w8 && g_attn_blk;
        int64_t wqkvf = -1;
        const int64_t sc_q = sc, sh_q = sh;
        if (fuse_qkv) {
            wqkvf = wres((int64_t)3 * C * C * 2);
            const int64_t s0 = pw[0], s1 = pw[1], s2 = pw[2];
            E.packs.push_back([=](const PackCtx& p) { pack_attn_qkv_w(p.params + s0, p.params + s1, p.params + s2, reinterpret_cast<bf16*>(p.packed + wqkvf), p.stream); });
            const int64_t sc_ = sc, sh_ = sh;
            if (!blk)
            op(CLS_GEMM, [=](const Ctx& c) {
                if (g_record) return;
                AttnBlk256 a;
                a.B = c.B; a.x = c.act(x); a.x_ld = x.ld; a.sc = c.at<float>(sc_); a.sh = c.at<float>(sh_);
                a.wqkvf = c.w<bf16>(wqkvf); a.bqk = c.w<float>(bqk); a.bv = c.w<float>(bv); a.qk = c.at<bf16>(qk); a.vT = c.at<bf16>(vT);
                launch_attn_qkv256(a, c.stream);
            });
        }
        if (!fuse_qkv)
        op(CLS_GEMM, [=](const Ctx& c) {
            GemmArgs g = gemm_defaults();
            g.a0 = c.act(h); g.a0_ld = C; g.a0_C = C; g.M = c.B * T; g.N = 2 * C;
            g.b = c.w<bf16>(wqk); g.b_ld = C; g.bias_n = c.w<float>(bqk);
            g.c = c.at<bf16>(qk); g.c_ld = 2 * C;
            launch_gemm(g, c.stream);
        });
        if (!fuse_qkv)
        op(CLS_GEMM, [=](const Ctx& c) {
            GemmArgs g = gemm_defaults();
            g.a0 = c.w<bf16>(wv); g.a0_ld = C; g.a0_C = C; g.a_bs = 0; g.M = C; g.N = T;
            g.b = c.act(h); g.b_ld = C; g.b_bs = (int64_t)T * C; g.bias_m = c.w<float>(bv);
            g.c = c.at<bf16>(vT); g.c_ld = T; g.c_bs = (int64_t)C * T; g.batch = c.B;
            launch_gemm(g, c.stream);
        });
        arena.release(h.off);
        const bool proj = T == 256 && C == 256 && g_attn_proj;
        int64_t w3f = -1;
        if (proj) {
            w3f = wres((int64_t)C * C * 2);
            const int64_t src = pw[3];
            E.packs.push_back([=](const PackCtx& p) { pack_attn_w3(p.params + src, reinterpret_cast<bf16*>(p.packed + w3f), p.stream); });
        }
        const bool blk2 = blk && g_attn_blk == 2;
        int64_t wqf2 = -1, wvof2 = -1, cq2 = -1, bo2 = -1;
        if (blk2) {
            const int64_t fq = wres((int64_t)C * C * 4), fv = wres((int64_t)C * C * 4);
            cq2 = wres((int64_t)C * 4); bo2 = wres((int64_t)C * 4);
            wqf2 = wres((int64_t)C * C * 2); wvof2 = wres((int64_t)C * C * 2);
            const int64_t w0_ = pw[0], w1_ = pw[1], w2_ = pw[2], w3_ = pw[3], b0_ = pb[0], b2_ = pb[2], b3_ = pb[3], cq_ = cq2, bo_ = bo2, wq_ = wqf2, wv_ = wvof2;
            E.packs.push_back([=](const PackCtx& p) {
                pack_attn_fold(p.params + w0_, p.params + w1_, p.params + w2_, p.params + w3_, p.params + b0_, p.params + b2_, p.params + b3_,
                               reinterpret_cast<float*>(p.packed + fq), reinterpret_cast<float*>(p.packed + cq_), reinterpret_cast<float*>(p.packed + fv),
                               reinterpret_cast<float*>(p.packed + bo_), reinterpret_cast<bf16*>(p.packed + wq_), reinterpret_cast<bf16*>(p.packed + wv_), p.stream);
            });
        }
        const Part po_attn = proj ? register_output(out) : Part();
        const float rs_attn = res_scale;
        TRef O = new_act(m.res, C);
        if (T == 256 && C == 256) {
            op(CLS_GEMM, [=](const Ctx& c) {
                if (g_record) return;
                if (proj) {
                    AttnBlk256 a;
                    a.plan = blk2 ? 2 : (blk ? 1 : 0); a.B = c.B; a.x = c.act(x); a.x_ld = x.ld; a.sc = c.at<float>(sc_q); a.sh = c.at<float>(sh_q);
                    if (wqkvf >= 0) a.wqkvf = c.w<bf16>(wqkvf);
                    a.bqk = c.w<float>(bqk); a.bv = c.w<float>(bv); a.qk = c.at<bf16>(qk); a.vT = c.at<bf16>(vT); a.w3f = c.w<bf16>(w3f); a.b3 = c.w<float>(b3);
                    if (blk2) { a.wqf2 = c.w<bf16>(wqf2); a.cq2 = c.w<float>(cq2); a.wvof2 = c.w<bf16>(wvof2); a.bo2 = c.w<float>(bo2); }
                    a.out = c.act(out); a.o_ld = out.ld; a.out_scale = rs_attn;
                    if (po_attn.valid) { a.gn_part = c.at<float2>(po_attn.off); a.gn_quads = po_attn.quads; }
                    const int rows = launch_attn_blk256(a, c.stream);
                    if (po_attn.valid) c.part_bm[po_attn.id] = rows;
                }
                else
                    hipLaunchKernelGGL(k_attn256<false>, dim3((unsigned)(2 * c.B)), dim3(256), A256_LDS_BYTES, c.stream, c.at<bf16>(qk), 2 * C, C, c.at<bf16>(vT), c.act(O), C,
                                       1.0f / sqrtf((float)C), (const bf16*)nullptr, (const float*)nullptr, (const bf16*)nullptr, 0, 1.0f, (float2*)nullptr, 0);
            });
            arena.release(vT); arena.release(qk);
        } else {
        const int64_t S = arena.alloc((int64_t)T * T * 4);
            op(CLS_GEMM, [=](const Ctx& c) {
                GemmArgs g = gemm_defaults();
                g.a0 = c.at<bf16>(qk); g.a0_ld = 2 * C; g.a0_C = C; g.a_bs = (int64_t)T * 2 * C; g.M = T; g.N = T;
                g.b = c.at<bf16>(qk) + C; g.b_ld = 2 * C; g.b_bs = (int64_t)T * 2 * C;
                g.scale = 1.0f / sqrtf((float)C);
                g.c = c.at<float>(S); g.c_ld = T; g.c_bs = (int64_t)T * T; g.c_mode = OUT_F32; g.batch = c.B;
                launch_gemm(g, c.stream);
            });
            const int64_t P = arena.alloc((int64_t)T * T * 2);
            op(CLS_OTHER, [=](const Ctx& c) {
                const int64_t rows = (int64_t)c.B * T;
                hipLaunchKernelGGL(k_softmax_rows, dim3((unsigned)((rows + 3) / 4)), dim3(256), 0, c.stream,
                                   c.at<float>(S), c.at<bf16>(P), T, rows);
            });
            arena.release(S);
            op(CLS_GEMM, [=](const Ctx& c) {
                GemmArgs g = gemm_defaults();
                g.a0 = c.at<bf16>(P); g.a0_ld = T; g.a0_C = T; g.a_bs = (int64_t)T * T; g.M = T; g.N = C;
                g.b = c.at<bf16>(vT); g.b_ld = T; g.b_bs = (int64_t)C * T;
                g.c = c.act(O); g.c_ld = C; g.c_bs = (int64_t)T * C; g.batch = c.B;
                launch_gemm(g, c.stream);
            });
            arena.release(P); arena.release(vT); arena.release(qk);
        }
        if (proj) {
            arena.release(O.off); arena.release(own_sc); arena.release(own_sh);
            if (sc != own_sc) { arena.release(sc); arena.release(sh); }
            E.taps[m.idx] = out;
            return;
        }
        const Part po = register_output(out);
        const float rs = res_scale;
        op(CLS_GEMM, [=](const Ctx& c) {
            GemmArgs g = gemm_defaults();
            g.a0 = c.act(O); g.a0_ld = C; g.a0_C = C; g.M = c.B * T; g.N = C;
            g.b = c.w<bf16>(w3); g.b_ld = C; g.bias_n = c.w<float>(b3);
            g.resid = c.act(x); g.resid_ld = x.ld; g.scale = rs;
            g.c = c.act(out); g.c_ld = out.ld;
            if (po.valid) { g.gn_part = c.at<float>(po.off); g.gn_quads = po.quads; }
            const int bm = launch_gemm(g, c.stream);
            if (po.valid) c.part_bm[po.id] = bm;
        });
        arena.release(O.off); arena.release(own_sc); arena.release(own_sh);
        if (sc != own_sc) { arena.release(sc); arena.release(sh); }
        E.taps[m.idx] = out;
    }

    void emit_downconv(const Mod& m, const TRef& x, const TRef& out) {
        const int C = m.cin, ro = m.res / 2, Kd = 9 * C;
        const int64_t pw = take((int64_t)C * C * 9), pb = take(C);
        const int64_t w = wres((int64_t)C * Kd * 2);
        E.packs.push_back([=](const PackCtx& p) {
            const int64_t n = (int64_t)C * C * 9;
            hipLaunchKernelGGL(k_pack_conv, dim3(grid1d(n, 256, 1 << 30)), dim3(256), 0, p.stream, p.params + pw, reinterpret_cast<bf16*>(p.packed + w), C, C, 9, Kd, 0, C, 0, 1.0f);
        });
        const int64_t b = pack_f32(pb, C);
        const int64_t col = arena.alloc((int64_t)ro * ro * Kd * 2);
        const Part po = register_output(out);
        const int rin = m.res;
        op(CLS_GEMM, [=](const Ctx& c) {
            const int64_t M = (int64_t)c.B * ro * ro;
            if (!g_record) {
                const int64_t total = M * (Kd / 8);
                hipLaunchKernelGGL(k_inc_im2col, dim3(grid1d(total, 256, 1 << 30)), dim3(256), 0, c.stream, c.act(x), rin, rin, x.ld, C, 3, 3, 2, 0, 0, ro, ro, Kd,
                                   c.at<bf16>(col), total);
            }
            GemmArgs g = gemm_defaults();
            g.a0 = c.at<bf16>(col); g.a0_ld = Kd; g.a0_C = Kd; g.M = (int)M; g.N = C; g.b = c.w<bf16>(w); g.b_ld = Kd; g.bias_n = c.w<float>(b);
            g.log_rows_per_sample = 2 * ilog2(ro); g.logHW = 2 * ilog2(ro); g.logW = ilog2(ro);
            g.c = c.act(out); g.c_ld = out.ld;
            if (po.valid) { g.gn_part = c.at<float>(po.off); g.gn_quads = po.quads; }
            const int bm = launch_gemm(g, c.stream);
            if (po.valid) c.part_bm[po.id] = bm;
        });
        arena.release(col);
        E.taps[m.idx] = out;
    }
    int64_t ident_sc = -1, ident_sh = -1;
    void emit_upconv(const Mod& m, const TRef& x, const TRef& out) {
        const int C = m.cin, ro = m.res * 2, Ku = 9 * C;
        const int64_t pw = take((int64_t)C * C * 9), pb = take(C);
        const int64_t w = wres((int64_t)C * Ku * 2);
        pack_conv(pw, w, C, C, 9, Ku, 0, C);
        const int64_t b = pack_f32(pb, C);
        if (ident_sc < 0) {
            ident_sc = arena.alloc((int64_t)2 * NF * 4); ident_sh = arena.alloc((int64_t)2 * NF * 4);
            const int64_t isc = ident_sc, ish = ident_sh;
            op(CLS_OTHER, [=](const Ctx& c) {
                const int64_t n = (int64_t)c.B * 2 * NF;
                hipLaunchKernelGGL(k_fill_f32, dim3(grid1d(n, 256, 1 << 30)), dim3(256), 0, c.stream, c.at<float>(isc), 1.0f, n);
                hipLaunchKernelGGL(k_fill_f32, dim3(grid1d(n, 256, 1 << 30)), dim3(256), 0, c.stream, c.at<float>(ish), 0.0f, n);
            });
        }
        TRef u = new_act(ro, C, 1);
        emit_gn_apply(x, ident_sc, ident_sh, u, nullptr, ACT_NONE, RS_UP);
        const Part po = register_output(out);
        const int logW = ilog2(ro);
        op(CLS_GEMM, [=](const Ctx& c) {
            GemmArgs g = gemm_defaults();
            g.a0 = c.act(u); g.a0_ld = u.ld; g.a0_C = C; g.taps = 9; g.logW = logW; g.logHW = 2 * logW; g.a0_padded = 1;
            g.M = c.B * ro * ro; g.N = C; g.b = c.w<bf16>(w); g.b_ld = Ku; g.bias_n = c.w<float>(b); g.log_rows_per_sample = 2 * logW;
            g.c = c.act(out); g.c_ld = out.ld;
            if (po.valid) { g.gn_part = c.at<float>(po.off); g.gn_quads = po.quads; }
            const int bm = launch_gemm(g, c.stream);
            if (po.valid) c.part_bm[po.id] = bm;
        });
        arena.release(u.off);
        E.taps[m.idx] = out;
    }

    int dense_rows_next = 0;

    struct Fin { int64_t sc = -1, sh = -1, gamma = -1, beta = -1; int C = 0; float out_mul = 1.0f; bool claimed = false, check = false; };
    struct Part { int64_t off = -1; int quads = 0, id = -1, res = 0; bool valid = false; std::shared_ptr<Fin> fin; };
    static void set_fin(GemmArgs& g, const Part& p, const Ctx& c) {
        if (!p.fin || !p.fin->claimed) return;
        const Fin& f = *p.fin;
        g.fin_scale = c.at<float>(f.sc); g.fin_shift = c.at<float>(f.sh); g.fin_gamma = c.w<float>(f.gamma); g.fin_beta = c.w<float>(f.beta);
        g.fin_ld = f.C; g.fin_cg = f.C / 32; g.fin_mul = f.out_mul; g.fin_eps = GN_EPS;
    }
    std::map<std::pair<int64_t, int>, Part> parts;
    int n_parts = 0;
    static bool fusable(int res) { return res >= 16; }
    Part new_part(int res, int C) {
        Part p; p.quads = C / 4; p.res = res; p.id = n_parts++; p.valid = true;
        p.off = arena.alloc((int64_t)std::max(res * res / 64, 1) * p.quads * 8);
        return p;
    }
    Part register_output(const TRef& out, bool fused8 = false) {
        Part p;
        if (fusable(out.res) || (out.res <= 8 && fused8)) p = new_part(out.res, out.C);
        if (p.valid && out.res <= 8 && fused8 && (g_fuse_fin & 1) && out.C == 256) {
            p.fin = std::make_shared<Fin>();
            p.fin->sc = arena.alloc((int64_t)out.C * 4); p.fin->sh = arena.alloc((int64_t)out.C * 4); p.fin->C = out.C;
        }
        if (p.valid && out.res == 16 && fused8 && (g_fuse_fin & 2) && out.C == 256 && !ddpm) {
            p.fin = std::make_shared<Fin>();
            p.fin->sc = arena.alloc((int64_t)out.C * 4); p.fin->sh = arena.alloc((int64_t)out.C * 4); p.fin->C = out.C; p.fin->check = true;
        }
        parts[{out.off, out.coff}] = p;
        return p;
    }
    bool emit_gn_from_parts(const TRef& x, GN gn, int64_t& sc, int64_t& sh, float out_mul) {
        std::vector<Part> src;
        int ch = 0;
        while (ch < x.C) {
            auto it = parts.find({x.off, x.coff + ch});
            if (it == parts.end() || !it->second.valid || it->second.res != x.res) return false;
            src.push_back(it->second);
            ch += it->second.quads * 4;
        }
        if (ch != x.C || src.empty() || src.size() > 2) return false;
        const Part p0 = src[0], p1 = src.size() > 1 ? src[1] : Part();
        const int HW = x.res * x.res, C = x.C;
        if (src.size() == 1 && p0.fin && !p0.fin->claimed && p0.fin->C == C) {
            Fin& f = *p0.fin;
            f.gamma = gn.gamma; f.beta = gn.beta; f.out_mul = out_mul; f.claimed = true;
            sc = f.sc; sh = f.sh;
            if (f.check) {
                const std::shared_ptr<Fin> fp = p0.fin;
                const int64_t fsc = f.sc, fsh = f.sh;
                op(CLS_OTHER, [=](const Ctx& c) {
                    if (c.fin_done[p0.id]) return;
                    hipLaunchKernelGGL(k_gn_finalize, dim3(c.B), dim3(256), 0, c.stream, c.at<float2>(p0.off), HW / c.part_bm[p0.id], p0.quads, (const float2*)nullptr, 0, 0, C, HW,
                                       c.w<float>(gn.gamma), c.w<float>(gn.beta), c.at<float>(fsc), c.at<float>(fsh), GN_EPS, out_mul);
                });
            }
            return true;
        }
        const int64_t sc_ = sc, sh_ = sh;
        op(CLS_OTHER, [=](const Ctx& c) {
            const int tps0 = HW / c.part_bm[p0.id], tps1 = p1.valid ? HW / c.part_bm[p1.id] : 0;
            hipLaunchKernelGGL(k_gn_finalize, dim3(c.B), dim3(256), 0, c.stream, c.at<float2>(p0.off), tps0, p0.quads,
                               p1.valid ? c.at<float2>(p1.off) : (const float2*)nullptr, tps1, p1.valid ? p1.quads : 0, C, HW,
                               c.w<float>(gn.gamma), c.w<float>(gn.beta), c.at<float>(sc_), c.at<float>(sh_), GN_EPS, out_mul);
        });
        return true;
    }

    void list_modules() {
        auto add = [&](int kind, int cin, int cout, int up, int down, int res) {
            Mod m; m.idx = (int)E.mods.size(); m.kind = kind; m.cin = cin; m.cout = cout; m.up = up; m.down = down; m.res = res; m.poff = 0;
            E.mods.push_back(m);
        };
        add(K_LIN, NF, TEMB, 0, 0, 0); add(K_LIN, TEMB, TEMB, 0, 0, 0); add(K_CONV, 3, NF, 0, 0, IMG);
        std::vector<int> skip = {NF};
        int ch = NF, res = IMG;
        for (int l = 0; l < NLEVEL; ++l) {
            for (int b = 0; b < NUM_RES; ++b) {
                add(K_RES, ch, NF * CH_MULT[l], 0, 0, res); ch = NF * CH_MULT[l];
                if (attn_at(res)) add(K_ATTN, ch, ch, 0, 0, res);
                skip.push_back(ch);
            }
            if (l != NLEVEL - 1) { if (ddpm) add(K_DOWN, ch, ch, 0, 0, res); else add(K_RES, ch, ch, 0, 1, res); res /= 2; skip.push_back(ch); }
        }
        add(K_RES, ch, ch, 0, 0, res); add(K_ATTN, ch, ch, 0, 0, res); add(K_RES, ch, ch, 0, 0, res);
        for (int l = NLEVEL - 1; l >= 0; --l) {
            for (int b = 0; b < NUM_RES + 1; ++b) { add(K_RES, ch + skip.back(), NF * CH_MULT[l], 0, 0, res); skip.pop_back(); ch = NF * CH_MULT[l]; }
            if (attn_at(res)) add(K_ATTN, ch, ch, 0, 0, res);
            if (l != 0) { if (ddpm) add(K_UP, ch, ch, 0, 0, res); else add(K_RES, ch, ch, 1, 0, res); res *= 2; }
        }
        add(K_GN, ch, ch, 0, 0, res); add(K_CONV, ch, 3, 0, 0, res);
    }

    void build() {
        list_modules();
        auto& M = E.mods;
        struct Cat { TRef buf; int ch_h, ch_s; };
        std::vector<Cat> cats;
        std::vector<int> skip_ch, skip_res;
        {
            int ch = NF, res = IMG; skip_ch.push_back(NF); skip_res.push_back(IMG);
            for (int l = 0; l < NLEVEL; ++l) {
                for (int b = 0; b < NUM_RES; ++b) { ch = NF * CH_MULT[l]; skip_ch.push_back(ch); skip_res.push_back(res); }
                if (l != NLEVEL - 1) { res /= 2; skip_ch.push_back(ch); skip_res.push_back(res); }
            }
            int sp = (int)skip_ch.size();
            for (int l = NLEVEL - 1; l >= 0; --l) {
                for (int b = 0; b < NUM_RES + 1; ++b) {
                    --sp;
                    Cat c; c.ch_h = ch; c.ch_s = skip_ch[sp];
                    c.buf = new_act(res, c.ch_h + c.ch_s);
                    cats.push_back(c);
                    ch = NF * CH_MULT[l];
                }
                if (l != 0) res *= 2;
            }
        }
        const int P = (int)skip_ch.size();
        auto skip_slot = [&](int i) { const Cat& c = cats[P - 1 - i]; TRef t = c.buf; t.C = c.ch_s; t.coff = c.ch_h; return t; };
        auto h_slot = [&](int j) { const Cat& c = cats[j]; TRef t = c.buf; t.C = c.ch_h; t.coff = 0; return t; };

        for (auto& m : M) if (m.kind == K_RES) dense_total += m.cout;
        dense_w = wres((int64_t)dense_total * TEMB * 2); dense_b = wres((int64_t)dense_total * 4);
        dense_out = arena.alloc((int64_t)dense_total * 4);
        const int64_t emb = arena.alloc(128 * 2), t1 = arena.alloc(TEMB * 2), t2 = arena.alloc(TEMB * 2);

        size_t mi = 0;
        {
            const Mod& m0 = M[mi++]; const Mod& m1 = M[mi++]; (void)m0; (void)m1;
            const int64_t pw0 = take((int64_t)TEMB * NF), pb0 = take(TEMB), pw1 = take((int64_t)TEMB * TEMB), pb1 = take(TEMB);
            const int64_t w0 = wres((int64_t)TEMB * NF * 2), w1 = wres((int64_t)TEMB * TEMB * 2);
            pack_conv(pw0, w0, TEMB, NF, 1, NF, 0, NF); pack_conv(pw1, w1, TEMB, TEMB, 1, TEMB, 0, TEMB);
            const int64_t b0 = pack_f32(pb0, TEMB), b1 = pack_f32(pb1, TEMB);
            const int64_t dw = dense_w, db = dense_b, dout = dense_out; const int dtot = dense_total;
            op(CLS_OTHER, [=](const Ctx& c) {
                hipLaunchKernelGGL(k_time_embed, dim3(grid1d((int64_t)c.B * 128, 256, 1 << 30)), dim3(256), 0, c.stream, c.labels, c.at<bf16>(emb), c.B);
            });
            op(CLS_GEMM, [=](const Ctx& c) {
                GemmArgs g = gemm_defaults();
                g.a0 = c.at<bf16>(emb); g.a0_ld = NF; g.a0_C = NF; g.M = c.B; g.N = TEMB;
                g.b = c.w<bf16>(w0); g.b_ld = NF; g.bias_n = c.w<float>(b0); g.act = ACT_SILU;
                g.c = c.at<bf16>(t1); g.c_ld = TEMB;
                launch_gemm(g, c.stream);
                g = gemm_defaults();
                g.a0 = c.at<bf16>(t1); g.a0_ld = TEMB; g.a0_C = TEMB; g.M = c.B; g.N = TEMB;
                g.b = c.w<bf16>(w1); g.b_ld = TEMB; g.bias_n = c.w<float>(b1); g.act = ACT_SILU;
                g.c = c.at<bf16>(t2); g.c_ld = TEMB;
                launch_gemm(g, c.stream);
                g = gemm_defaults();
                g.a0 = c.at<bf16>(t2); g.a0_ld = TEMB; g.a0_C = TEMB; g.M = c.B; g.N = dtot;
                g.b = c.w<bf16>(dw); g.b_ld = TEMB; g.bias_n = c.w<float>(db);
                g.c = c.at<float>(dout); g.c_ld = dtot; g.c_mode = OUT_F32;
                launch_gemm(g, c.stream);
            });
        }
        int si = 0;
        TRef cur = skip_slot(si++);
        {
            const Mod& m = M[mi++];
            const int64_t pw = take((int64_t)NF * 27), pb = take(NF);
            const int64_t w = wres((int64_t)NF * 64 * 2);
            pack_zero(w, (int64_t)NF * 64);
            pack_conv(pw, w, NF, 3, 9, 64, 0, 3);
            const int64_t b = pack_f32(pb, NF);
            const int64_t a0 = arena.alloc((int64_t)IMG * IMG * 64 * 2);
            const TRef dst = cur;
            const Part po = register_output(dst);
            op(CLS_OTHER, [=](const Ctx& c) {
                const int64_t rows = (int64_t)c.B * IMG * IMG;
                hipLaunchKernelGGL(k_stem_im2col, dim3((unsigned)((rows * 8 + 255) / 256)), dim3(256), 0, c.stream, c.x, c.at<bf16>(a0), rows);
            });
            op(CLS_GEMM, [=](const Ctx& c) {
                const int64_t rows = (int64_t)c.B * IMG * IMG;
                GemmArgs g = gemm_defaults();
                g.a0 = c.at<bf16>(a0); g.a0_ld = 64; g.a0_C = 64; g.M = (int)rows; g.N = NF;
                g.b = c.w<bf16>(w); g.b_ld = 64; g.bias_n = c.w<float>(b);
                g.c = c.act(dst); g.c_ld = dst.ld;
                if (po.valid) { g.gn_part = c.at<float>(po.off); g.gn_quads = po.quads; }
                const int bm = launch_gemm(g, c.stream);
                if (po.valid) c.part_bm[po.id] = bm;
            });
            arena.release(a0);
            E.taps[m.idx] = dst;
        }
        int res = IMG;
        for (int l = 0; l < NLEVEL; ++l) {
            for (int b = 0; b < NUM_RES; ++b) {
                const Mod& m = M[mi++];
                const TRef dst = skip_slot(si++);
                if (attn_at(res)) {
                    TRef tmp = new_act(res, m.cout);
                    emit_res(m, cur, tmp);
                    emit_attn(M[mi++], tmp, dst);
                    arena.release(tmp.off);
                } else {
                    emit_res(m, cur, dst);
                }
                cur = dst;
            }
            if (l != NLEVEL - 1) {
                const Mod& m = M[mi++];
                const TRef dst = skip_slot(si++);
                if (ddpm) emit_downconv(m, cur, dst); else emit_res(m, cur, dst);
                cur = dst; res /= 2;
            }
        }
        {
            TRef a = new_act(res, cur.C), b = new_act(res, cur.C);
            emit_res(M[mi++], cur, a);
            emit_attn(M[mi++], a, b);
            arena.release(a.off);
            emit_res(M[mi++], b, h_slot(0));
            arena.release(b.off);
        }
        int j = 0;
        TRef last;
        for (int l = NLEVEL - 1; l >= 0; --l) {
            for (int b = 0; b < NUM_RES + 1; ++b) {
                const Mod& m = M[mi++];
                const bool level_end = b == NUM_RES;
                TRef in = cats[j].buf;
                TRef dst = level_end ? new_act(res, m.cout) : h_slot(j + 1);
                emit_res(m, in, dst);
                arena.release(cats[j].buf.off);
                last = dst; ++j;
            }
            if (attn_at(res)) {
                TRef dst = new_act(res, last.C);
                emit_attn(M[mi++], last, dst);
                arena.release(last.off);
                last = dst;
            }
            if (l != 0) {
                const Mod& m = M[mi++];
                if (ddpm) emit_upconv(m, last, h_slot(j)); else emit_res(m, last, h_slot(j));
                arena.release(last.off);
                res *= 2;
            }
        }
        {
            const Mod& mg = M[mi++]; const Mod& mc = M[mi++];
            const GN gn = take_gn(mg.cin);
            const int64_t pw = take((int64_t)3 * mc.cin * 9), pb = take(3);
            const int Kf = 9 * mc.cin;
            const int64_t w = wres((int64_t)3 * Kf * 2);
            pack_conv(pw, w, 3, mc.cin, 9, Kf, 0, mc.cin);
            const int64_t b = pack_f32(pb, 3);
            int64_t sc = arena.alloc((int64_t)mg.cin * 4), sh = arena.alloc((int64_t)mg.cin * 4);
            const int logW = ilog2(res), cinf = mc.cin;
            if (g_fuse_head && res == HeadConvCfg::RES && mc.cin == HeadConvCfg::C) {
                const int64_t w16 = wres((int64_t)16 * Kf * 2);
                pack_zero(w16, (int64_t)16 * Kf);
                pack_conv(pw, w16, 3, mc.cin, 9, Kf, 0, mc.cin, -0.6931471805599453f);
                emit_gn_stats(last, gn, sc, sh, -1.4426950408889634f);
                const TRef src = last;
                op(CLS_GEMM, [=](const Ctx& c) {
                    if (g_record) { *g_record += gemm_row(c.B * res * res, 3, Kf, 0, 9, 1, "head_conv", 0) + "\n"; return; }
                    hipLaunchKernelGGL(k_head_conv, dim3((unsigned)(c.B * (HeadConvCfg::RES / HeadConvCfg::ROWS))), dim3(256), HeadConvCfg::LDS_BYTES, c.stream,
                                       c.act(src), src.ld, c.at<float>(sc), c.at<float>(sh), c.w<bf16>(w16), c.w<float>(b), c.out);
                });
            } else {
            emit_gn_stats(last, gn, sc, sh);
            TRef u = new_act(res, mg.cin, 1);
            emit_gn_apply(last, sc, sh, u, nullptr, ACT_SILU, RS_NONE);
            op(CLS_GEMM, [=](const Ctx& c) {
                GemmArgs g = gemm_defaults();
                g.a0 = c.act(u); g.a0_ld = u.ld; g.a0_C = cinf; g.taps = 9; g.logW = logW; g.logHW = 2 * logW; g.a0_padded = 1;
                g.M = c.B * res * res; g.N = 3; g.b = c.w<bf16>(w); g.b_ld = Kf; g.bias_n = c.w<float>(b);
                g.c = c.out; g.c_mode = OUT_F32_NCHW;
                launch_gemm(g, c.stream);
            });
            }
            E.taps[mg.idx] = last;
        }
        finish();
        E.part_bm.assign(n_parts > 0 ? n_parts : 1, 128);
        E.fin_done.assign(n_parts > 0 ? n_parts : 1, 0);
    }
};

int64_t module_param_count(const Mod& m) {
    switch (m.kind) {
        case K_LIN: return (int64_t)m.cout * m.cin + m.cout;
        case K_CONV: return (int64_t)m.cout * m.cin * 9 + m.cout;
        case K_GN: return 2 * (int64_t)m.cin;
        case K_DOWN: case K_UP: return (int64_t)m.cout * m.cin * 9 + m.cout;
        case K_ATTN: return 2 * (int64_t)m.cin + 4 * ((int64_t)m.cin * m.cin + m.cin);
        case K_RES: {
            int64_t n = 2 * (int64_t)m.cin + (int64_t)m.cout * m.cin * 9 + m.cout + (int64_t)m.cout * TEMB + m.cout +
                        2 * (int64_t)m.cout + (int64_t)m.cout * m.cout * 9 + m.cout;
            if (m.cin != m.cout || m.up || m.down) n += (int64_t)m.cout * m.cin + m.cout;
            return n;
        }
    }
    return 0;
}

natinf_ncsnpp* make_engine(int flags) {
    natinf_ncsnpp* e = new natinf_ncsnpp();
    e->flags = flags;
    Builder b(*e);
    b.build();
    int64_t off = 0;
    for (auto& m : e->mods) { m.poff = off; off += module_param_count(m); }
    if (off != e->n_params) { delete e; return nullptr; }
    return e;
}

const natinf_ncsnpp& reference_engine() {
    static natinf_ncsnpp* e = [] {
        int* knobs[] = {&g_fuse_gn, &g_fuse_up, &g_fuse_head, &g_fuse_gn8, &g_fuse_gn4, &g_fuse_fin, &g_attn_qkv, &g_attn_proj};
        int saved[sizeof(knobs) / sizeof(knobs[0])];
        for (size_t i = 0; i < sizeof(knobs) / sizeof(knobs[0]); ++i) { saved[i] = *knobs[i]; *knobs[i] = 1; }
        g_fuse_fin = 3;
        const int saved_fold = g_fuse_up_fold;
        g_fuse_up_fold = 0;
        natinf_ncsnpp* r = make_engine(0);
        g_fuse_up_fold = saved_fold;
        for (size_t i = 0; i < sizeof(knobs) / sizeof(knobs[0]); ++i) *knobs[i] = saved[i];
        return r;
    }();
    return *e;
}

}

extern "C" {

int64_t natinf_ncsnpp_param_count(void) { return reference_engine().n_params; }
int64_t natinf_ncsnpp_packed_bytes(void) { return reference_engine().packed_bytes; }

int64_t natinf_ncsnpp_handle_param_count(natinf_ncsnpp_t h) { return h ? h->n_params : NATINF_EINVAL; }
int64_t natinf_ncsnpp_handle_packed_bytes(natinf_ncsnpp_t h) { return h ? h->packed_bytes : NATINF_EINVAL; }

int64_t natinf_ncsnpp_workspace_bytes(natinf_ncsnpp_t h, int max_batch) {
    if (!h || max_batch <= 0) return NATINF_EINVAL;
    return h->ws_per_image * (int64_t)max_batch;
}

static uint64_t plan_signature() {
    const int k[] = {g_fuse_head, g_attn_qkv, g_attn_w8, g_attn_proj, g_fuse_gn8, g_fuse_fin, g_fuse_gn4, g_fuse_gn, g_cg_wide, g_fuse_up,
                     g_attn_blk , g_fuse_up_fold, g_cg3 };
    uint64_t h = 1469598103934665603ull;
    for (int v : k) h = (h ^ (uint64_t)(v & 0xff)) * 1099511628211ull;
    return h;
}

int natinf_ncsnpp_create(natinf_ncsnpp_t* out, int flags) {
    if (!out || (flags & ~(NATINF_NCSNPP_KEEP_ACTIVATIONS | NATINF_NCSNPP_DDPM))) return NATINF_EINVAL;
    natinf_ncsnpp* e = make_engine(flags);
    if (!e) return NATINF_ESTATE;
    e->plan_sig = plan_signature();
    *out = e;
    return NATINF_OK;
}

int natinf_ncsnpp_destroy(natinf_ncsnpp_t h) {
    if (!h) return NATINF_EINVAL;
    for (auto& r : h->recs) { (void)hipEventDestroy(r.a); (void)hipEventDestroy(r.b); }
    for (auto e : h->pool) (void)hipEventDestroy(e);
    delete h;
    return NATINF_OK;
}

int natinf_ncsnpp_describe(natinf_ncsnpp_t h, char* buf, int cap) {
    if (!h || !buf || cap <= 0) return NATINF_EINVAL;
    std::string s;
    char line[160];
    for (const auto& m : h->mods) {
        snprintf(line, sizeof(line), "%d %s %d %d %d %d %d %lld\n", m.idx, kind_name(m.kind), m.cin, m.cout, m.up, m.down, m.res,
                 (long long)m.poff);
        s += line;
    }
    if ((int)s.size() + 1 > cap) return NATINF_EINVAL;
    memcpy(buf, s.c_str(), s.size() + 1);
    return (int)s.size();
}

int natinf_ncsnpp_load(natinf_ncsnpp_t h, const float* params_f32, int64_t n_params, void* packed, int64_t packed_bytes,
                       natinf_stream_t stream) {
    return h ? h->load(params_f32, n_params, packed, packed_bytes, (hipStream_t)stream) : NATINF_EINVAL;
}

int natinf_ncsnpp_share(natinf_ncsnpp_t h, natinf_ncsnpp_t loaded) {
    if (!h || !loaded || h == loaded) return NATINF_EINVAL;
    if (!loaded->packed) return NATINF_ESTATE;
    if ((h->flags & NATINF_NCSNPP_DDPM) != (loaded->flags & NATINF_NCSNPP_DDPM) || h->n_params != loaded->n_params || h->packed_bytes != loaded->packed_bytes ||
        h->packs.size() != loaded->packs.size() || h->plan_sig != loaded->plan_sig)
        return NATINF_EINVAL;
    h->packed = loaded->packed;
    return NATINF_OK;
}

int natinf_ncsnpp_forward(natinf_ncsnpp_t h, const float* x, const float* labels, float* out, int B, void* workspace,
                          int64_t workspace_bytes, natinf_stream_t stream) {
    if (!h || !x || !labels || !out || !workspace || B <= 0) return NATINF_EINVAL;
    if (!h->packed) return NATINF_ESTATE;
    if (workspace_bytes < h->ws_per_image * (int64_t)B || (int64_t)B * IMG * IMG >= (1LL << 31)) return NATINF_EINVAL;
    if (!h->configured) {
        if (!configure_gemm_kernels()) return NATINF_ENODEV;
        h->configured = true;
    }
    Ctx c{B, reinterpret_cast<unsigned char*>(workspace), h->packed, (hipStream_t)stream, x, labels, out, h->part_bm.data()};
    c.fin_done = h->fin_done.data();
    g_launch_error = 0;
    if (!h->prof) {
        for (const auto& f : h->ops) f(c);
    } else {
        for (size_t i = 0; i < h->ops.size(); ++i) {
            natinf_ncsnpp::Rec r; r.cls = h->op_cls[i];
            for (hipEvent_t* e : {&r.a, &r.b}) {
                if (!h->pool.empty()) { *e = h->pool.back(); h->pool.pop_back(); }
                else if (hipEventCreate(e) != hipSuccess) return NATINF_ELAUNCH;
            }
            (void)hipEventRecord(r.a, c.stream);
            h->ops[i](c);
            (void)hipEventRecord(r.b, c.stream);
            h->recs.push_back(r);
        }
    }
    h->last_B = B; h->last_ws = c.ws;
    if (g_launch_error) { g_launch_error = 0; return NATINF_ESTATE; }
    return hipGetLastError() == hipSuccess ? NATINF_OK : NATINF_ELAUNCH;
}

int natinf_ncsnpp_describe_gemms(natinf_ncsnpp_t h, int B, char* buf, int cap) {
    if (!h || !buf || cap <= 0 || B <= 0) return NATINF_EINVAL;
    std::string out;
    g_record = &out;
    std::vector<int> scratch_bm(h->part_bm.size(), 128);
    std::vector<unsigned char> scratch_done(h->part_bm.size(), 0);
    Ctx c{B, reinterpret_cast<unsigned char*>(4096), reinterpret_cast<const unsigned char*>(4096), nullptr, nullptr, nullptr, nullptr, scratch_bm.data()};
    c.fin_done = scratch_done.data();
    for (size_t i = 0; i < h->ops.size(); ++i)
        if (h->op_cls[i] == CLS_GEMM || h->op_cls[i] == CLS_CONV_GN || h->op_cls[i] == CLS_CONV_GN8) h->ops[i](c);
    g_record = nullptr;
    if ((int)out.size() + 1 > cap) return NATINF_EINVAL;
    memcpy(buf, out.c_str(), out.size() + 1);
    return (int)out.size();
}

int natinf_debug_gemm(int variant, int M, int N, int K0, int K1, int taps, int logW, int batch,
                      const void* a0, const void* a1, const void* b, const float* bias_n, void* c, int c_f32, float scale,
                      int iters, natinf_stream_t stream) {
    if (variant < 0 || variant >= V_COUNT || !a0 || !b || !c || M <= 0 || N <= 0 || K0 <= 0 || K1 < 0 || iters <= 0 || (taps != 1 && taps != 9)) return NATINF_EINVAL;
    if (K0 % taps || N % 8 || (a1 != nullptr) != (K1 > 0)) return NATINF_EINVAL;
    if (taps == 9 && ((K0 / 9) % BK || logW < 1 || logW > 12 || M % (1 << (2 * logW)) || batch != 1)) return NATINF_EINVAL;
    if (!variant_shipped(variant) || variant == V_CONV_GN || variant == V_FP8_256x256) return NATINF_ESTATE;
#ifndef NATINF_DEV
    if (c_f32 >= 2) return NATINF_ESTATE;
#endif
    static bool configured = false;
    if (!configured) { if (!configure_gemm_kernels()) return NATINF_ENODEV; configured = true; }
    GemmArgs g = gemm_defaults();
    g.a0 = (const bf16*)a0; g.a0_C = K0 / taps; g.a0_ld = g.a0_C; g.taps = taps; g.logW = logW; g.logHW = 2 * logW; g.a0_padded = taps == 9;
    if (a1) { g.a1 = (const bf16*)a1; g.a1_C = K1; g.a1_ld = K1; }
    g.M = M; g.N = N; g.b = (const bf16*)b; g.b_ld = K0 + (a1 ? K1 : 0); g.batch = batch;
    if (batch > 1) { g.a_bs = (int64_t)M * g.a0_ld; g.b_bs = (int64_t)N * g.b_ld; g.c_bs = (int64_t)M * N; }
    g.bias_n = bias_n; g.scale = scale; g.c = c; g.c_ld = N; g.c_mode = c_f32 == 1 ? OUT_F32 : (c_f32 >= 2 ? 100 + c_f32 : OUT_BF16);
    g.dbg_ts = g_dbg_ts;
    g.splitk_ws = g_dbg_splitk_ws; g.splitk_max = g_dbg_splitk_max;
    const int saved = g_force_variant;
    g_force_variant = variant;
    g_launch_error = 0;
    for (int i = 0; i < iters; ++i) launch_gemm(g, (hipStream_t)stream);
    g_force_variant = saved;
    if (g_launch_error) { g_launch_error = 0; return NATINF_EINVAL; }
    return hipGetLastError() == hipSuccess ? NATINF_OK : NATINF_ELAUNCH;
}

int g_dbg_conv_logW = 0; const void* g_dbg_conv_a1 = nullptr; int g_dbg_conv_c1 = 0;
int natinf_debug_set_conv_operand(int logW, const void* a1, int c1) {
    if (logW < 0 || logW > 12 || c1 < 0 || c1 % BK || (c1 > 0) != (a1 != nullptr) || (logW == 0 && a1)) return NATINF_EINVAL;
    g_dbg_conv_logW = logW; g_dbg_conv_a1 = a1; g_dbg_conv_c1 = c1;
    return NATINF_OK;
}

int natinf_debug_gemm_fused(int variant, int M, int N, int K, const void* a, const void* b, const float* bias_n, const float* bias_m,
                            const float* rowvec, const float* gate, int log_rows_per_sample, const void* resid_bf16, const float* resid_f32,
                            float scale, int act, void* c, int c_f32, float* gn_part, int* bm_out, int fp32_slab, natinf_stream_t stream) {
    const int logW = g_dbg_conv_logW, c1 = g_dbg_conv_c1;
    const void* a1 = g_dbg_conv_a1;
    g_dbg_conv_logW = 0; g_dbg_conv_a1 = nullptr; g_dbg_conv_c1 = 0;
    if (variant < 0 || variant >= V_COUNT || !a || !b || !c || M <= 0 || N <= 0 || K <= 0 || c_f32 < 0 || c_f32 > 2) return NATINF_EINVAL;
    if (c_f32 == 2) {
        if (!logW || bias_m || rowvec || gate || resid_bf16 || resid_f32 || gn_part || act != ACT_NONE) return NATINF_EINVAL;
    } else if (N % 8) return NATINF_EINVAL;
    if (logW && (K % 9 || (K / 9) % BK || M % (1 << (2 * logW)))) return NATINF_EINVAL;
    if (!variant_shipped(variant) || variant == V_CONV_GN || variant == V_FP8_256x256) return NATINF_ESTATE;
    if (!configure_gemm_kernels()) return NATINF_ENODEV;
    GemmArgs g = gemm_defaults();
    g.a0 = (const bf16*)a; g.a0_C = K; g.a0_ld = K; g.M = M; g.N = N; g.b = (const bf16*)b; g.b_ld = K;
    if (logW) {
        g.taps = 9; g.a0_C = g.a0_ld = K / 9; g.logW = logW; g.logHW = 2 * logW; g.a0_padded = 1; g.b_ld = K + c1;
        if (a1) { g.a1 = (const bf16*)a1; g.a1_C = g.a1_ld = c1; }
    }
    g.bias_n = bias_n; g.bias_m = bias_m; g.rowvec = rowvec; g.rowvec_ld = N; g.gate = gate; g.gate_ld = N; g.log_rows_per_sample = log_rows_per_sample;
    g.resid = (const bf16*)resid_bf16; g.resid_ld = N; g.resid_f32 = resid_f32; g.resid_f32_ld = N;
    g.scale = scale; g.act = act; g.c = c; g.c_ld = N; g.c_mode = c_f32 == 2 ? OUT_F32_NCHW : (c_f32 ? OUT_F32 : OUT_BF16);
    g.gn_part = gn_part; g.gn_quads = N / 4; g.epi_fp32_slab = fp32_slab != 0;
    g.splitk_ws = g_dbg_splitk_ws; g.splitk_max = g_dbg_splitk_max;
    g.dbg_ts = g_dbg_ts;
    const int saved = g_force_variant;
    g_force_variant = variant;
    g_launch_error = 0;
    const int bm = launch_gemm(g, (hipStream_t)stream);
    g_force_variant = saved;
    if (bm_out) *bm_out = bm;
    if (g_launch_error) { g_launch_error = 0; return NATINF_EINVAL; }
    return hipGetLastError() == hipSuccess ? NATINF_OK : NATINF_ELAUNCH;
}

int g_dbg_cg_up = 0;
int natinf_debug_conv_gn_up(int flags) { if (flags & ~3) return NATINF_EINVAL; g_dbg_cg_up = flags; return NATINF_OK; }
float* g_dbg_fin_scale = nullptr; float* g_dbg_fin_shift = nullptr; const float* g_dbg_fin_gamma = nullptr; const float* g_dbg_fin_beta = nullptr;
int g_dbg_fin_cg = 0; float g_dbg_fin_mul = 1.0f;
int natinf_debug_conv_gn_fin(float* fin_scale, float* fin_shift, const float* gamma, const float* beta, int channels_per_group, float mul) {
    if (fin_scale && (!fin_shift || !gamma || !beta || channels_per_group < 4 || channels_per_group % 4)) return NATINF_EINVAL;
    g_dbg_fin_scale = fin_scale; g_dbg_fin_shift = fin_shift; g_dbg_fin_gamma = gamma; g_dbg_fin_beta = beta; g_dbg_fin_cg = channels_per_group; g_dbg_fin_mul = mul;
    return NATINF_OK;
}
int natinf_debug_conv_gn(int res, int B, int N, int cin, int c1, const void* x, const float* scale, const float* shift, const void* w_packed,
                         void* w_frag, const void* a1, const float* bias_n, const void* resid, float out_scale, void* out, float* gn_part, int iters,
                         natinf_stream_t stream) {
    if ((res != 32 && res != 16 && res != 8 && res != 4) || B <= 0 || N <= 0 || N % 8 || cin <= 0 || cin % 64 || c1 < 0 || c1 % 64 || (c1 > 0) != (a1 != nullptr) ||
        !x || !scale || !shift || !w_packed || !out || iters <= 0) return NATINF_EINVAL;
    static bool configured = false;
    if (!configured) { if (!configure_gemm_kernels()) return NATINF_ENODEV; configured = true; }
    GemmArgs g = gemm_defaults();
    g.a0 = (const bf16*)x; g.a0_ld = cin; g.a0_C = cin; g.taps = 9; g.logW = ilog2(res); g.logHW = 2 * g.logW;
    g.gn_scale = scale; g.gn_shift = shift; g.gn_ld = cin; g.gn_folded = 1;
    if (a1) { g.a1 = (const bf16*)a1; g.a1_ld = c1; g.a1_C = c1; }
    g.M = B * res * res; g.N = N; g.b = (const bf16*)w_packed; g.b_ld = 9 * cin + c1; g.bias_n = bias_n;
    g.resid = (const bf16*)resid; g.resid_ld = N; g.scale = out_scale; g.c = out; g.c_ld = N;
    g.gn_part = gn_part; g.gn_quads = N / 4;
    if (g_dbg_fin_scale) {
        if (!gn_part || N != 256 || res > 16 || N % g_dbg_fin_cg) return NATINF_EINVAL;
        g.fin_scale = g_dbg_fin_scale; g.fin_shift = g_dbg_fin_shift; g.fin_gamma = g_dbg_fin_gamma; g.fin_beta = g_dbg_fin_beta;
        g.fin_ld = N; g.fin_cg = g_dbg_fin_cg; g.fin_mul = g_dbg_fin_mul; g.fin_eps = GN_EPS;
    }
    g.dbg_ts = g_dbg_ts;
    g.a0_up = g_dbg_cg_up & 1; g.a1_up = (a1 && (g_dbg_cg_up & 2)) ? 1 : 0;
    if (w_frag && N % 16 == 0) g.b_frag = (const bf16*)w_frag;
    if (!conv_gn_ok(g)) return NATINF_EINVAL;
    if (g.b_frag) {
        const int64_t n = (int64_t)(N / 16) * (9 * (cin / 32) + c1 / 32) * 64;
        hipLaunchKernelGGL(k_pack_frag, dim3(grid1d(n, 256, 1 << 30)), dim3(256), 0, (hipStream_t)stream, (const bf16*)w_packed, (bf16*)w_frag, N, g.b_ld, cin, c1);
    }
    for (int i = 0; i < iters; ++i) launch_gemm(g, (hipStream_t)stream);
    return hipGetLastError() == hipSuccess ? NATINF_OK : NATINF_ELAUNCH;
}

int natinf_debug_fold_up_weights(const float* w, int N, int cin, float w_mul, float* out_f32, void* out_packed, natinf_stream_t stream) {
    if (!w || N <= 0 || cin <= 0 || (!out_f32 && !out_packed) || (out_packed && cin % 64)) return NATINF_EINVAL;
    ncsn_upf::fold(w, out_packed, out_f32, N, cin, w_mul, stream);
    return hipGetLastError() == hipSuccess ? NATINF_OK : NATINF_ELAUNCH;
}
int natinf_debug_conv_up_fold(int B, int N, int cin, const void* x, const float* scale, const float* shift, const float* w, void* w_packed, void* h_scratch,
                              const float* bias_n, const float* rowvec, float out_scale, void* out, float* gn_part, int iters, natinf_stream_t stream) {
    if (B <= 0 || N != UPFOLD_BN || cin <= 0 || cin % 64 || !x || !scale || !shift || !w || !w_packed || !h_scratch || !out || iters <= 0) return NATINF_EINVAL;
    static bool configured = false;
    if (!configured) { if (!configure_gemm_kernels()) return NATINF_ENODEV; configured = true; }
    hipStream_t s = (hipStream_t)stream;
    constexpr int W = UPFOLD_W, logW = 4;
    ncsn_upf::fold(w, w_packed, nullptr, N, cin, 1.0f, stream);
    hipLaunchKernelGGL(k_gn_apply, dim3((unsigned)((W + 2 + GN_ROWS - 1) / GN_ROWS), (unsigned)B), dim3(256), 0, s, (const bf16*)x, cin, cin, logW, 2 * logW, scale, shift,
                       (bf16*)h_scratch, (bf16*)nullptr, ACT_SILU, RS_NONE, 1);
    GemmArgs g = gemm_defaults();
    g.a0 = (const bf16*)h_scratch; g.a0_ld = cin; g.a0_padded = 1; g.a0_C = cin; g.taps = 4; g.logW = logW; g.logHW = 2 * logW;
    g.M = B * W * W; g.N = 4 * N; g.b = (const bf16*)w_packed; g.b_ld = 4 * cin; g.bias_n = bias_n;
    g.rowvec = rowvec; g.rowvec_ld = N; g.log_rows_per_sample = 2 * logW; g.scale = out_scale;
    g.c = out; g.c_ld = N; g.gn_part = gn_part; g.gn_quads = N / 4;
    if (!up_fold_epi(g)) return NATINF_EINVAL;
    g_launch_error = 0;
    for (int i = 0; i < iters; ++i) launch_gemm(g, s);
    if (g_launch_error) { g_launch_error = 0; return NATINF_EINVAL; }
    return hipGetLastError() == hipSuccess ? NATINF_OK : NATINF_ELAUNCH;
}

int natinf_debug_attn_block(int plan, int B, const void* x, int x_ld, const float* scale, const float* shift, const float* w, const float* bias,
                            void* packed, void* scratch, void* out, int o_ld, float out_scale, float* gn_part, natinf_stream_t stream) {
    if (plan < 0 || plan > 2 || B < 1 || !x || !scale || !shift || !w || !bias || !packed || !out || x_ld < 256 || x_ld % 8 || o_ld < 256 || o_ld % 8 ||
        (plan != 2 && !scratch)) return NATINF_EINVAL;
    static bool configured = false;
    if (!configured) { if (!configure_gemm_kernels()) return NATINF_ENODEV; configured = true; }
    constexpr int64_t WW = 256 * 256;
    unsigned char* pk = reinterpret_cast<unsigned char*>(packed);
    hipStream_t s = (hipStream_t)stream;
    AttnBlk256 a;
    a.plan = plan; a.B = B; a.x = (const bf16*)x; a.x_ld = x_ld; a.sc = scale; a.sh = shift;
    a.out = (bf16*)out; a.o_ld = o_ld; a.out_scale = out_scale; a.gn_part = reinterpret_cast<float2*>(gn_part); a.gn_quads = 64;
    if (plan == 2) {
        float* fq = reinterpret_cast<float*>(pk + NATINF_ATTN_BLOCK_OFF_FOLD_WQK); float* fv = reinterpret_cast<float*>(pk + NATINF_ATTN_BLOCK_OFF_FOLD_WVO);
        float* cq = reinterpret_cast<float*>(pk + NATINF_ATTN_BLOCK_OFF_FOLD_CQ); float* bo = reinterpret_cast<float*>(pk + NATINF_ATTN_BLOCK_OFF_FOLD_BO);
        bf16* wqf2 = reinterpret_cast<bf16*>(pk + NATINF_ATTN_BLOCK_OFF_WQK_PACKED); bf16* wvof2 = reinterpret_cast<bf16*>(pk + NATINF_ATTN_BLOCK_OFF_WVO_PACKED);
        pack_attn_fold(w, w + WW, w + 2 * WW, w + 3 * WW, bias, bias + 512, bias + 768, fq, cq, fv, bo, wqf2, wvof2, s);
        a.wqf2 = wqf2; a.cq2 = cq; a.wvof2 = wvof2; a.bo2 = bo;
    } else {
        bf16* wqkvf = reinterpret_cast<bf16*>(pk + NATINF_ATTN_BLOCK_OFF_WQKV); bf16* w3f = reinterpret_cast<bf16*>(pk + NATINF_ATTN_BLOCK_OFF_W3);
        pack_attn_qkv_w(w, w + WW, w + 2 * WW, wqkvf, s);
        pack_attn_w3(w + 3 * WW, w3f, s);
        a.wqkvf = wqkvf; a.bqk = bias; a.bv = bias + 512; a.w3f = w3f; a.b3 = bias + 768;
        a.qk = reinterpret_cast<bf16*>(scratch); a.vT = a.qk + (int64_t)B * 256 * 512;
        if (plan == 0) launch_attn_qkv256(a, s);
    }
    launch_attn_blk256(a, s);
    return hipGetLastError() == hipSuccess ? NATINF_OK : NATINF_ELAUNCH;
}

int natinf_debug_quant_fp8_rows(const float* w, void* q, float* row_scale, int rows, int cols, natinf_stream_t stream) {
    if (!w || !q || !row_scale || rows <= 0 || cols <= 0 || cols % 2) return NATINF_EINVAL;
    hipLaunchKernelGGL(k_pack_fp8_rows, dim3((unsigned)((rows + 3) / 4)), dim3(256), 0, (hipStream_t)stream, w, (uint8_t*)q, row_scale, rows, cols);
    return hipGetLastError() == hipSuccess ? NATINF_OK : NATINF_ELAUNCH;
}

int natinf_debug_gemm_fp8(int M, int N, int K, const void* a8, const float* a_scale, const void* a_mx, const void* b8, const float* b_scale,
                          const float* bias_n, void* c, void* c_mx, int c_mode, int iters, natinf_stream_t stream) {
    if (!a8 || !b8 || !c || M <= 0 || N <= 0 || K <= 0 || K % 128 || N % 8 || iters <= 0) return NATINF_EINVAL;
    static bool configured = false;
    if (!configured) { if (!configure_gemm_kernels()) return NATINF_ENODEV; configured = true; }
    GemmArgs g = gemm_defaults();
    g.a0 = (const bf16*)a8; g.a0_C = K; g.a0_ld = K; g.M = M; g.N = N; g.b = (const bf16*)b8; g.b_ld = K;
    const int act = c_mode >> 8; c_mode &= 0xff;
    if (act != ACT_NONE && act != ACT_GELU_TANH) return NATINF_EINVAL;
    g.deq_m = a_scale; g.deq_n = b_scale; g.bias_n = bias_n; g.c = c; g.c_ld = N; g.c_mode = c_mode; g.act = act;
    g.a_mx = (const uint8_t*)a_mx; g.a_mx_ld = M; g.c_mx = (uint8_t*)c_mx; g.c_mx_ld = M;
    if ((c_mode == OUT_FP8_MX && (!c_mx || N % 32)) || c_mode < 0 || c_mode > OUT_FP8_MX || c_mode == OUT_F32_NCHW) return NATINF_EINVAL;
    for (int i = 0; i < iters; ++i) launch_gemm_fp8(g, (hipStream_t)stream);
    return hipGetLastError() == hipSuccess ? NATINF_OK : NATINF_ELAUNCH;
}

int natinf_debug_timestamps(void* dev_buf16) {
#ifdef NATINF_DEV
    g_dbg_ts = reinterpret_cast<unsigned long long*>(dev_buf16); return NATINF_OK;
#else
    (void)dev_buf16; return NATINF_ESTATE;
#endif
}

int natinf_set_gemm_raster(int rows) { g_raster_g = rows; return NATINF_OK; }
int natinf_set_fuse_gn(int on) { g_fuse_gn = on != 0; return NATINF_OK; }
int natinf_set_fuse_gn8(int on) { g_fuse_gn8 = on != 0; return NATINF_OK; }
int natinf_set_attn256(int on) { return on ? NATINF_OK : NATINF_ESTATE; }
int natinf_set_conv_gn_warm(int mask) { if (mask < 0 || mask > 15) return NATINF_EINVAL; g_cg_warm = mask; return NATINF_OK; }
int natinf_set_attn_block(int on) { g_attn_blk = on < 0 ? ATTN_BLK_DEFAULT : (on > 2 ? 2 : on); return NATINF_OK; }
int natinf_set_attn_qkv(int on) { g_attn_qkv = on != 0; return NATINF_OK; }
int natinf_set_attn_waves8(int on) { g_attn_w8 = on != 0; return NATINF_OK; }
int natinf_set_attn_proj(int on) { g_attn_proj = on != 0; return NATINF_OK; }
int natinf_set_fuse_fin(int on) {
    if (on < 0 || on > 3) return NATINF_EINVAL;
    static const int mask[4] = {0, 3, 1, 2};
    g_fuse_fin = mask[on];
    return NATINF_OK;
}
int natinf_set_gemm_round_model(int on) { g_round_model = on != 0; g_round_model_w128 = on >= 10 ? on : 13; return NATINF_OK; }
int natinf_set_gemm_w128(int on) { g_w128 = on < 0 ? 0 : (on > 2 ? 2 : on); return NATINF_OK; }
int natinf_set_fuse_gn4(int on) { g_fuse_gn4 = on != 0; return NATINF_OK; }
int natinf_set_conv_gn8_tile(int one_image) { return one_image ? NATINF_OK : NATINF_ESTATE; }
int natinf_set_fuse_head(int on) { g_fuse_head = on != 0; return NATINF_OK; }
int natinf_set_conv_gn_w128(int mask) { if (mask < 0 || mask > 7) return NATINF_EINVAL; g_cg3 = mask; return NATINF_OK; }
int natinf_set_conv_gn_w128_min_k(int shape, int k) { if (shape < 0 || shape > 2 || k < 0) return NATINF_EINVAL; g_cg3_min_k[shape] = k; return NATINF_OK; }
int natinf_set_conv_gn_wide(int mask) { if (mask < 0 || mask > 3) return NATINF_EINVAL; g_cg_wide = mask; return NATINF_OK; }
int natinf_set_conv_gn_regw(int on) { return on ? NATINF_OK : NATINF_ESTATE; }
int natinf_set_fuse_up(int on) { g_fuse_up = on != 0; return NATINF_OK; }
int natinf_set_fuse_up_fold(int on) { g_fuse_up_fold = on < 0 ? UP_FOLD_DEFAULT : on != 0; return NATINF_OK; }
int natinf_set_gemm_splitk(int on) { g_splitk = on != 0; return NATINF_OK; }
int natinf_debug_set_splitk_workspace(float* ws, int max_slices) { g_dbg_splitk_ws = ws; g_dbg_splitk_max = ws ? max_slices : 0; return NATINF_OK; }
int natinf_set_gemm_half_issue(int on) { return on ? NATINF_OK : NATINF_ESTATE; }
int natinf_set_gemm_pref512(int on) { g_pref_512 = on != 0; return NATINF_OK; }
int natinf_set_gemm_epilogue(int fp32_slab) { g_epi_fp32_slab = fp32_slab != 0; return NATINF_OK; }

int natinf_set_gemm_variant(int variant) {
    if (variant < 0 || variant >= V_COUNT) return NATINF_EINVAL;
    if (!variant_shipped(variant) || variant == V_CONV_GN || variant == V_FP8_256x256) return NATINF_ESTATE;
    g_force_variant = variant;
    return NATINF_OK;
}

int natinf_gemm_profile(int enable) { g_gemm_prof.on = enable != 0; return NATINF_OK; }
int natinf_gemm_profile_read(char* buf, int cap) {
    if (!buf || cap <= 0) return NATINF_EINVAL;
    std::map<std::string, std::pair<double, int64_t>> by;
    std::vector<std::string> order;
    int rc = NATINF_OK;
    for (auto& e : g_gemm_prof.ev) {
        float ms = 0.f;
        if (hipEventSynchronize(e.b) != hipSuccess || hipEventElapsedTime(&ms, e.a, e.b) != hipSuccess) { (void)hipGetLastError(); rc = NATINF_ELAUNCH; }
        else {
            auto it = by.find(e.tag);
            if (it == by.end()) { order.push_back(e.tag); it = by.emplace(e.tag, std::make_pair(0.0, (int64_t)0)).first; }
            it->second.first += ms; it->second.second += 1;
        }
        g_gemm_prof.pool.emplace_back(e.a, e.b);
    }
    g_gemm_prof.ev.clear();
    if (rc != NATINF_OK) return rc;
    std::string out;
    for (auto& t : order) {
        char tail[64];
        snprintf(tail, sizeof(tail), " %lld %.6f\n", (long long)by[t].second, by[t].first);
        out += t + tail;
    }
    if ((int)out.size() + 1 > cap) return NATINF_EINVAL;
    memcpy(buf, out.c_str(), out.size() + 1);
    return (int)out.size();
}
int natinf_ncsnpp_profile(natinf_ncsnpp_t h, int enable) {
    if (!h) return NATINF_EINVAL;
    h->prof = enable != 0;
    return NATINF_OK;
}

int natinf_ncsnpp_profile_read(natinf_ncsnpp_t h, double* ms_by_class, int64_t* launches_by_class) {
    if (!h || !ms_by_class || !launches_by_class) return NATINF_EINVAL;
    for (int i = 0; i < N_CLS; ++i) { ms_by_class[i] = 0.0; launches_by_class[i] = 0; }
    for (const auto& r : h->recs) {
        float ms = 0.f;
        if (hipEventSynchronize(r.b) != hipSuccess || hipEventElapsedTime(&ms, r.a, r.b) != hipSuccess) {
            (void)hipGetLastError();
            return NATINF_ELAUNCH;
        }
        ms_by_class[r.cls] += ms; launches_by_class[r.cls] += 1;
        h->pool.push_back(r.a); h->pool.push_back(r.b);
    }
    h->recs.clear();
    return NATINF_OK;
}

int natinf_ncsnpp_debug_tap(natinf_ncsnpp_t h, int module_idx, float* out, int64_t capacity_elems, natinf_stream_t stream) {
    if (!h || !out) return NATINF_EINVAL;
    if (!(h->flags & NATINF_NCSNPP_KEEP_ACTIVATIONS) || !h->last_ws) return NATINF_ESTATE;
    auto it = h->taps.find(module_idx);
    if (it == h->taps.end()) return NATINF_EINVAL;
    const TRef& t = it->second;
    const int HW = t.res * t.res;
    const int64_t total = (int64_t)h->last_B * t.C * HW;
    if (capacity_elems < total) return NATINF_EINVAL;
    const bf16* src = reinterpret_cast<const bf16*>(h->last_ws + t.off * h->last_B) + t.coff;
    hipLaunchKernelGGL(k_nhwc_to_nchw_f32, dim3(grid1d(total, 256, 1 << 30)), dim3(256), 0, (hipStream_t)stream, src, t.ld, t.C, HW, out, total);
    return hipGetLastError() == hipSuccess ? NATINF_OK : NATINF_ELAUNCH;
}

static bool dbg_misaligned(const void* p, uintptr_t a) { return reinterpret_cast<uintptr_t>(p) % a != 0; }

int natinf_debug_gn_stats(const void* x, int ld, int C, int HW, int B, const float* gamma, const float* beta, float* scale, float* shift, float eps, float out_mul,
                          natinf_stream_t stream) {
    if (!x || !gamma || !beta || !scale || !shift || B < 1 || HW < 1 || C < 32 || C > 512 || C % 32 || ld < C || ld % 8 || dbg_misaligned(x, 16)) return NATINF_EINVAL;
    if ((256 / (C >> 3)) * C > 16 * 128 + 64) return NATINF_EINVAL;
    hipLaunchKernelGGL(k_gn_stats, dim3((unsigned)B), dim3(256), 0, (hipStream_t)stream, (const bf16*)x, ld, C, HW, gamma, beta, scale, shift, eps, out_mul);
    return hipGetLastError() == hipSuccess ? NATINF_OK : NATINF_ELAUNCH;
}

int natinf_debug_gn_finalize(const float* P0, int tps0, int quads0, const float* P1, int tps1, int quads1, int C, int HW, int B, const float* gamma, const float* beta,
                             float* scale, float* shift, float eps, float out_mul, natinf_stream_t stream) {
    if (!P0 || !gamma || !beta || !scale || !shift || B < 1 || HW < 1 || tps0 < 1 || quads0 < 1) return NATINF_EINVAL;
    if (P1 ? (tps1 < 1 || quads1 < 1) : (tps1 != 0 || quads1 != 0)) return NATINF_EINVAL;
    if (C < 128 || C > 512 || C % 128 || quads0 + quads1 > 128 || (quads0 + quads1) * 4 != C || dbg_misaligned(P0, 8) || dbg_misaligned(P1, 8)) return NATINF_EINVAL;
    hipLaunchKernelGGL(k_gn_finalize, dim3((unsigned)B), dim3(256), 0, (hipStream_t)stream, reinterpret_cast<const float2*>(P0), tps0, quads0,
                       reinterpret_cast<const float2*>(P1), tps1, quads1, C, HW, gamma, beta, scale, shift, eps, out_mul);
    return hipGetLastError() == hipSuccess ? NATINF_OK : NATINF_ELAUNCH;
}

int natinf_debug_gn_apply(const void* x, int ld, int C, int logW, int logHW, int B, const float* scale, const float* shift, void* y, void* xr, int act, int mode, int pad,
                          natinf_stream_t stream) {
    if (!x || !scale || !shift || !y || B < 1 || B > 65535 || C < 8 || C % 8 || (C >> 3) > 256 || ld < C || ld % 8) return NATINF_EINVAL;
    if (logW < 0 || logHW < logW || logHW > 24 || mode < RS_NONE || mode > RS_DOWN || (pad != 0 && pad != 1) || (act != ACT_NONE && act != ACT_SILU)) return NATINF_EINVAL;
    if (mode == RS_DOWN && (logW < 1 || logHW - logW < 1)) return NATINF_EINVAL;
    if (dbg_misaligned(x, 16) || dbg_misaligned(y, 16) || dbg_misaligned(xr, 16) || dbg_misaligned(scale, 16) || dbg_misaligned(shift, 16)) return NATINF_EINVAL;
    const int Hs = 1 << (logHW - logW), Hd = mode == RS_UP ? 2 * Hs : (mode == RS_DOWN ? Hs / 2 : Hs);
    const int rows_per_img = Hd + 2 * pad;
    hipLaunchKernelGGL(k_gn_apply, dim3((unsigned)((rows_per_img + GN_ROWS - 1) / GN_ROWS), (unsigned)B), dim3(256), 0, (hipStream_t)stream, (const bf16*)x, ld, C,
                       logW, logHW, scale, shift, (bf16*)y, (bf16*)xr, act, mode, pad);
    return hipGetLastError() == hipSuccess ? NATINF_OK : NATINF_ELAUNCH;
}

int natinf_debug_head_conv(const void* x, int ld, int B, const float* scale, const float* shift, const void* w16, const float* bias, float* out, natinf_stream_t stream) {
    if (!x || !scale || !shift || !w16 || !bias || !out || B < 1 || ld < HeadConvCfg::C || ld % 8) return NATINF_EINVAL;
    if (dbg_misaligned(x, 16) || dbg_misaligned(w16, 16) || dbg_misaligned(out, 16)) return NATINF_EINVAL;
    if (hipFuncSetAttribute(reinterpret_cast<const void*>(&k_head_conv), hipFuncAttributeMaxDynamicSharedMemorySize, HeadConvCfg::LDS_BYTES) != hipSuccess) {
        (void)hipGetLastError();
        return NATINF_ENODEV;
    }
    hipLaunchKernelGGL(k_head_conv, dim3((unsigned)(B * (HeadConvCfg::RES / HeadConvCfg::ROWS))), dim3(256), HeadConvCfg::LDS_BYTES, (hipStream_t)stream,
                       (const bf16*)x, ld, scale, shift, (const bf16*)w16, bias, out);
    return hipGetLastError() == hipSuccess ? NATINF_OK : NATINF_ELAUNCH;
}

int natinf_debug_time_embed(const float* labels, void* emb, int B, natinf_stream_t stream) {
    if (!labels || !emb || B < 1 || B >= (1 << 21)) return NATINF_EINVAL;
    hipLaunchKernelGGL(k_time_embed, dim3(grid1d((int64_t)B * 128, 256, 1 << 30)), dim3(256), 0, (hipStream_t)stream, labels, (bf16*)emb, B);
    return hipGetLastError() == hipSuccess ? NATINF_OK : NATINF_ELAUNCH;
}

int natinf_debug_stem_im2col(const float* x, void* A, int B, natinf_stream_t stream) {
    if (!x || !A || B < 1 || B > (1 << 17) || dbg_misaligned(A, 16)) return NATINF_EINVAL;
    const int64_t rows = (int64_t)B * 1024;
    hipLaunchKernelGGL(k_stem_im2col, dim3((unsigned)((rows * 8 + 255) / 256)), dim3(256), 0, (hipStream_t)stream, x, (bf16*)A, rows);
    return hipGetLastError() == hipSuccess ? NATINF_OK : NATINF_ELAUNCH;
}

int natinf_debug_pack_conv(const float* src, void* dst, int N, int Cin, int taps, int dst_ld, int koff, int tap_stride_c, int chunked, float wmul, natinf_stream_t stream) {
    if (!src || !dst || N < 1 || Cin < 1 || taps < 1 || koff < 0 || (chunked != 0 && chunked != 1)) return NATINF_EINVAL;
    const int64_t n = (int64_t)N * Cin * taps;
    const int64_t span = chunked ? (int64_t)((Cin + 63) / 64) * taps * 64 : (int64_t)(taps - 1) * tap_stride_c + Cin;
    if ((!chunked && tap_stride_c < Cin) || koff + span > dst_ld || n > ((int64_t)1 << 30) * 256) return NATINF_EINVAL;
    hipLaunchKernelGGL(k_pack_conv, dim3(grid1d(n, 256, 1 << 30)), dim3(256), 0, (hipStream_t)stream, src, (bf16*)dst, N, Cin, taps, dst_ld, koff, tap_stride_c, chunked, wmul);
    return hipGetLastError() == hipSuccess ? NATINF_OK : NATINF_ELAUNCH;
}

int natinf_debug_pack_transpose(const float* src, void* dst, int K, int N, int dst_ld, natinf_stream_t stream) {
    if (!src || !dst || K < 1 || N < 1 || dst_ld < K) return NATINF_EINVAL;
    hipLaunchKernelGGL(k_pack_transpose, dim3(grid1d((int64_t)K * N, 256, 1 << 30)), dim3(256), 0, (hipStream_t)stream, src, (bf16*)dst, K, N, dst_ld);
    return hipGetLastError() == hipSuccess ? NATINF_OK : NATINF_ELAUNCH;
}

int natinf_debug_nhwc_to_nchw(const void* x, int ld, int C, int HW, int B, float* out, natinf_stream_t stream) {
    if (!x || !out || B < 1 || C < 1 || HW < 1 || ld < C) return NATINF_EINVAL;
    const int64_t total = (int64_t)B * C * HW;
    if (total > ((int64_t)1 << 30) * 256) return NATINF_EINVAL;
    hipLaunchKernelGGL(k_nhwc_to_nchw_f32, dim3(grid1d(total, 256, 1 << 30)), dim3(256), 0, (hipStream_t)stream, (const bf16*)x, ld, C, HW, out, total);
    return hipGetLastError() == hipSuccess ? NATINF_OK : NATINF_ELAUNCH;
}

}
#include "dit_engine.inc"
#include "mmdit_engine.inc"
#include "vae_engine.inc"
#include "inception_engine.inc"
```

naturaldiffusion_amd/csrc/ncsnpp_kernels.h:

```cpp
#pragma once
#include <hip/hip_runtime.h>
#include <stdint.h>
#include <type_traits>

namespace ncsn {

typedef __bf16 bf16;
typedef __bf16 bf16x8 __attribute__((ext_vector_type(8)));
typedef float f32x4 __attribute__((ext_vector_type(4)));

#ifdef NATINF_ASM_PAD
#define NATINF_PAD_PRE "s_nop 7\n\ts_nop 7\n\t"
#define NATINF_PAD_POST "\n\ts_nop 7\n\ts_nop 7"
#else
#define NATINF_PAD_PRE ""
#define NATINF_PAD_POST ""
#endif

#define NATINF_M0_ASM_BEGIN _Pragma("clang diagnostic push") _Pragma("clang diagnostic ignored \"-Winline-asm\"")
#define NATINF_M0_ASM_END _Pragma("clang diagnostic pop")

__device__ __forceinline__ void lds_poison()
{
#ifdef NATINF_LDS_POISON
// ... 418 lines not shown
        for (int i = 0; i < 8; ++i) { s[i] = 0.f; q[i] = 0.f; }
        const bf16* base = x + (int64_t)b * HW * ld + chunk * 8;
        for (int p = pl; p < HW; p += lanes) {
            const bf16x8 v = *reinterpret_cast<const bf16x8*>(base + (int64_t)p * ld);
#pragma unroll
            for (int i = 0; i < 8; ++i) { const float f = (float)v[i]; s[i] += f; q[i] += f * f; }
        }
#pragma unroll
        for (int i = 0; i < 8; ++i) { s_part[0][pl * C + chunk * 8 + i] = s[i]; s_part[1][pl * C + chunk * 8 + i] = q[i]; }
    }
    __syncthreads();
    for (int c = tid; c < C; c += 256) {
        float s = 0.f, q = 0.f;
        for (int l = 0; l < lanes; ++l) { s += s_part[0][l * C + c]; q += s_part[1][l * C + c]; }
        s_sum[c] = s; s_sq[c] = q;
    }
    __syncthreads();
    const int cg = C >> 5;
    if (tid < 32) {
        float s = 0.f, q = 0.f;
        for (int i = 0; i < cg; ++i) { s += s_sum[tid * cg + i]; q += s_sq[tid * cg + i]; }
        const float inv = 1.0f / (float)(cg * HW);
        const float mean = s * inv;
        float var = q * inv - mean * mean;
        var = var < 0.f ? 0.f : var;
        s_mean[tid] = mean;
        s_rstd[tid] = 1.0f / sqrtf(var + eps);
    }
    __syncthreads();
    for (int c = tid; c < C; c += 256) {
        const int gi = c / cg;
        const float sc = s_rstd[gi] * gamma[c];
        scale[(int64_t)b * C + c] = sc * out_mul;
        shift[(int64_t)b * C + c] = (beta[c] - s_mean[gi] * sc) * out_mul;
    }
}

__global__ __launch_bounds__(256) void k_gn_finalize(const float2* __restrict__ P0, int tps0, int quads0,
                                                     const float2* __restrict__ P1, int tps1, int quads1, int C, int HW,
                                                     const float* __restrict__ gamma, const float* __restrict__ beta,
                                                     float* __restrict__ scale, float* __restrict__ shift, float eps, float out_mul)
{
    __shared__ float2 s_p[128];
    lds_poison();
    const int tid = threadIdx.x, b = blockIdx.x, nq = quads0 + quads1;
    float ga[2] = {0.f, 0.f}, be[2] = {0.f, 0.f};
#pragma unroll
    for (int k = 0; k < 2; ++k) {
        const int c = tid + 256 * k;
        if (c < C) { ga[k] = gamma[c]; be[k] = beta[c]; }
    }
    for (int q = tid; q < nq; q += 256) {
        const bool first = q < quads0;
        const float2* P = first ? P0 + (int64_t)b * tps0 * quads0 + q : P1 + (int64_t)b * tps1 * quads1 + (q - quads0);
        const int tps = first ? tps0 : tps1, st = first ? quads0 : quads1;
        float s = 0.f, qq = 0.f;
        int t = 0;
        for (; t + 4 <= tps; t += 4) {
            const float2 v0 = P[(int64_t)t * st], v1 = P[(int64_t)(t + 1) * st], v2 = P[(int64_t)(t + 2) * st], v3 = P[(int64_t)(t + 3) * st];
            s += v0.x; qq += v0.y; s += v1.x; qq += v1.y; s += v2.x; qq += v2.y; s += v3.x; qq += v3.y;
        }
        for (; t < tps; ++t) { const float2 v = P[(int64_t)t * st]; s += v.x; qq += v.y; }
        s_p[q] = make_float2(s, qq);
    }
    __syncthreads();
    const int cg = C >> 5, qpg = cg >> 2;
    const float inv = 1.0f / (float)(cg * HW);
#pragma unroll
    for (int k = 0; k < 2; ++k) {
        const int c = tid + 256 * k;
        if (c >= C) break;
        const int gi = c / cg;
        float s = 0.f, q = 0.f;
        for (int i = 0; i < qpg; ++i) { const float2 v = s_p[gi * qpg + i]; s += v.x; q += v.y; }
        const float mean = s * inv;
        float var = q * inv - mean * mean;
        var = var < 0.f ? 0.f : var;
        const float sc = (1.0f / sqrtf(var + eps)) * ga[k];
        scale[(int64_t)b * C + c] = sc * out_mul;
        shift[(int64_t)b * C + c] = (be[k] - mean * sc) * out_mul;
    }
}

enum { RS_NONE = 0, RS_UP = 1, RS_DOWN = 2 };
constexpr int GN_ROWS = 4;
#ifndef GN_UNROLL
#define GN_UNROLL 4
#endif
__global__ __launch_bounds__(256) void k_gn_apply(const bf16* __restrict__ x, int ld, int C, int logW, int logHW,
                                                  const float* __restrict__ scale, const float* __restrict__ shift,
                                                  bf16* __restrict__ y, bf16* __restrict__ xr, int act, int mode, int pad)
{
    const int cpp = C >> 3, lanes = 256 / cpp;
    const int chunk = threadIdx.x % cpp, pl = threadIdx.x / cpp;
    if (pl >= lanes) return;
    const int Ws = 1 << logW, Hs = 1 << (logHW - logW);
    const int Wd = mode == RS_UP ? 2 * Ws : (mode == RS_DOWN ? Ws >> 1 : Ws);
    const int Hd = mode == RS_UP ? 2 * Hs : (mode == RS_DOWN ? Hs >> 1 : Hs);
    const int Wp = Wd + 2 * pad, Hp = Hd + 2 * pad;
    const int b = blockIdx.y, row0 = blockIdx.x * GN_ROWS;
    const int nrows = min(GN_ROWS, Hp - row0);
    float sc[8], sh[8];
    {
        const float* ps = scale + (int64_t)b * C + chunk * 8;
        const float* ph = shift + (int64_t)b * C + chunk * 8;
        const float4 s0 = *reinterpret_cast<const float4*>(ps), s1 = *reinterpret_cast<const float4*>(ps + 4);
        const float4 h0 = *reinterpret_cast<const float4*>(ph), h1 = *reinterpret_cast<const float4*>(ph + 4);
        sc[0] = s0.x; sc[1] = s0.y; sc[2] = s0.z; sc[3] = s0.w; sc[4] = s1.x; sc[5] = s1.y; sc[6] = s1.z; sc[7] = s1.w;
        sh[0] = h0.x; sh[1] = h0.y; sh[2] = h0.z; sh[3] = h0.w; sh[4] = h1.x; sh[5] = h1.y; sh[6] = h1.z; sh[7] = h1.w;
    }
    const bf16* xb = x + (int64_t)b * Hs * Ws * ld + chunk * 8;
    bf16* yb = y + ((int64_t)b * Hp + row0) * Wp * C + chunk * 8;
    bf16* xrb = xr ? xr + (int64_t)b * Hd * Wd * C + chunk * 8 : nullptr;
    int rr = 0, xx = pl;
    while (xx >= Wp) { xx -= Wp; ++rr; }
    auto advance = [&](int& r, int& c) __attribute__((always_inline)) { c += lanes; while (c >= Wp) { c -= Wp; ++r; } };
    auto interior = [&](int r, int c) __attribute__((always_inline)) {
        const int Y = row0 + r - pad, X = c - pad;
        return r < nrows && Y >= 0 && Y < Hd && X >= 0 && X < Wd;
    };
    auto finish = [&](int r, int c, bool in, const bf16x8& v) __attribute__((always_inline)) {
        if (r >= nrows) return;
        bf16x8 o;
        if (!in) {
#pragma unroll
            for (int q = 0; q < 8; ++q) o[q] = (bf16)0.0f;
        } else {
#pragma unroll
            for (int q = 0; q < 8; ++q) {
                float f = (float)v[q] * sc[q] + sh[q];
                if (act == ACT_SILU) f = silu_fast(f);
                o[q] = (bf16)f;
            }
            if (xrb) *reinterpret_cast<bf16x8*>(xrb + ((int64_t)(row0 + r - pad) * Wd + (c - pad)) * C) = v;
        }
        *reinterpret_cast<bf16x8*>(yb + ((int64_t)r * Wp + c) * C) = o;
    };
    if (mode != RS_DOWN) {
        const int sh_ = mode == RS_UP ? 1 : 0;
        constexpr int U = GN_UNROLL;
        while (rr < nrows) {
            int r[U], c[U];
            bool in[U];
            bf16x8 v[U];
            r[0] = rr; c[0] = xx;
#pragma unroll
            for (int u = 1; u < U; ++u) { r[u] = r[u - 1]; c[u] = c[u - 1]; advance(r[u], c[u]); }
#pragma unroll
            for (int u = 0; u < U; ++u) {
                in[u] = interior(r[u], c[u]);
                if (in[u]) v[u] = *reinterpret_cast<const bf16x8*>(xb + ((int64_t)((row0 + r[u] - pad) >> sh_) * Ws + ((c[u] - pad) >> sh_)) * ld);
            }
#pragma unroll
            for (int u = 0; u < U; ++u) finish(r[u], c[u], in[u], v[u]);
            rr = r[U - 1]; xx = c[U - 1];
            advance(rr, xx);
        }
        return;
    }
    for (; rr < nrows; ) {
        const int Y = row0 + rr - pad, X = xx - pad;
        bf16x8 o;
        if (Y < 0 || Y >= Hd || X < 0 || X >= Wd) {
#pragma unroll
            for (int q = 0; q < 8; ++q) o[q] = (bf16)0.0f;
        } else {
// ... 143 lines not shown
```

naturaldiffusion_amd/ncsnpp.py:

```python
from __future__ import annotations

import ctypes as C
from typing import Dict, List, Tuple

import torch

from . import _lib
from ._lib import lib, check, ptr, stream_ptr

KEEP_ACTIVATIONS = 1
DDPM = 2
ARCH_FLAGS = {"ncsnpp": 0, "ddpm": DDPM}


def module_table(handle=None, arch: str = "ncsnpp") -> List[Tuple[int, str, int, int, int, int, int, int]]:
    own = handle is None
    if own:
        h = C.c_void_p()
        check(lib.natinf_ncsnpp_create(C.byref(h), ARCH_FLAGS[arch]), "natinf_ncsnpp_create")
        handle = h
    buf = C.create_string_buffer(1 << 14)
    n = lib.natinf_ncsnpp_describe(handle, buf, len(buf))
    if n < 0:
        check(n, "natinf_ncsnpp_describe")
# ... 36 lines not shown
                out += [(p + "Conv_2.weight", (cout, cin, 1, 1)), (p + "Conv_2.bias", (cout,))]
        elif kind in ("down", "up"):
            out += [(p + "Conv_0.weight", (cout, cin, 3, 3)), (p + "Conv_0.bias", (cout,))]
        else:
            raise RuntimeError(f"unknown module kind {kind}")
    return out


def flatten_state_dict(sd: Dict[str, torch.Tensor], arch: str = "ncsnpp") -> torch.Tensor:
    sd = {(k[7:] if k.startswith("module.") else k): v for k, v in sd.items()}
    parts = []
    for name, shape in param_layout(arch=arch):
        if name not in sd:
            raise KeyError(f"checkpoint lacks {name}")
        t = sd[name]
        if tuple(t.shape) != tuple(shape):
            raise ValueError(f"{name}: shape {tuple(t.shape)} != expected {shape}")
        parts.append(t.detach().to("cpu", torch.float32).reshape(-1))
    return torch.cat(parts)


def flatten_ema(shadow_params: List[torch.Tensor], nf: int = 128, arch: str = "ncsnpp") -> torch.Tensor:
    layout = param_layout(nf, arch)
    if len(shadow_params) != len(layout):
        raise ValueError(f"EMA list has {len(shadow_params)} tensors, the model has {len(layout)} parameters")
    parts = []
    for (name, shape), t in zip(layout, shadow_params):
        if tuple(t.shape) != tuple(shape):
            raise ValueError(f"EMA entry for {name}: shape {tuple(t.shape)} != expected {shape}")
        parts.append(t.detach().to("cpu", torch.float32).reshape(-1))
    return torch.cat(parts)


def load_score_sde_checkpoint(path: str, nf: int = 128, arch: str = "ncsnpp") -> torch.Tensor:
    state = torch.load(path, map_location="cpu", weights_only=False)
    for key in ("model", "ema", "step"):
        if key not in state:
            raise KeyError(f"{path}: not a score_sde checkpoint (no '{key}' entry; utils.py:22-29)")
    shadow = list(state["ema"]["shadow_params"])
    model_sd = {(k[7:] if k.startswith("module.") else k): v for k, v in state["model"].items()}
    for (name, shape), t in zip(param_layout(nf, arch), shadow):
        if name in model_sd and tuple(model_sd[name].shape) != tuple(t.shape):
            raise ValueError(f"{path}: EMA entry for {name} has shape {tuple(t.shape)}, the model's is {tuple(model_sd[name].shape)}")
    return flatten_ema(shadow, nf, arch)


class NCSNppEngine:
    def __init__(self, flat_params: torch.Tensor, max_batch: int, device="cuda:0", keep_activations: bool = False, arch: str = "ncsnpp"):
        _lib.require_gpu()
        self.device = torch.device(device)
        self.max_batch = int(max_batch)
        self.arch = arch
        self._h = C.c_void_p()
        self._flags = (KEEP_ACTIVATIONS if keep_activations else 0) | ARCH_FLAGS[arch]
        check(lib.natinf_ncsnpp_create(C.byref(self._h), self._flags), "natinf_ncsnpp_create")
        n = lib.natinf_ncsnpp_handle_param_count(self._h)
        if flat_params.numel() != n:
            raise ValueError(f"expected {n} parameters, got {flat_params.numel()}")
        with torch.cuda.device(self.device):
            params = flat_params.to(self.device, torch.float32).contiguous()
            self._packed = torch.empty(lib.natinf_ncsnpp_handle_packed_bytes(self._h), dtype=torch.uint8, device=self.device)
            check(lib.natinf_ncsnpp_load(self._h, ptr(params), n, ptr(self._packed), self._packed.numel(), stream_ptr()),
                  "natinf_ncsnpp_load")
            torch.cuda.current_stream().synchronize()
            ws = lib.natinf_ncsnpp_workspace_bytes(self._h, self.max_batch)
            self._ws = torch.empty(ws, dtype=torch.uint8, device=self.device)
        self.workspace_bytes = ws

    def clone(self, max_batch: int = None) -> "NCSNppEngine":
        other = object.__new__(NCSNppEngine)
        other.device, other.arch = self.device, self.arch
        other.max_batch = int(max_batch or self.max_batch)
        other._h = C.c_void_p()
        check(lib.natinf_ncsnpp_create(C.byref(other._h), self._flags), "natinf_ncsnpp_create")
        check(lib.natinf_ncsnpp_share(other._h, self._h), "natinf_ncsnpp_share")
        other._flags = self._flags
        other._packed = self._packed
        with torch.cuda.device(self.device):
            ws = lib.natinf_ncsnpp_workspace_bytes(other._h, other.max_batch)
            other._ws = torch.empty(ws, dtype=torch.uint8, device=self.device)
        other.workspace_bytes = ws
        return other

    def __call__(self, x: torch.Tensor, labels: torch.Tensor, out: torch.Tensor = None) -> torch.Tensor:
        if x.dtype != torch.float32 or x.dim() != 4 or tuple(x.shape[1:]) != (3, 32, 32) or not x.is_cuda:
            raise ValueError("x must be a CUDA fp32 tensor of shape [B,3,32,32]")
        B = x.shape[0]
        if B > self.max_batch:
            raise ValueError(f"batch {B} exceeds max_batch {self.max_batch}")
        x = x.contiguous()
        labels = labels.to(x.device, torch.float32).contiguous()
        if labels.numel() != B:
            raise ValueError("labels must have one entry per sample")
        if out is None:
            out = torch.empty_like(x)
        check(lib.natinf_ncsnpp_forward(self._h, ptr(x), ptr(labels), ptr(out), B, ptr(self._ws), self._ws.numel(),
                                        stream_ptr()), "natinf_ncsnpp_forward")
        return out

    def profile(self, enable: bool) -> None:
        check(lib.natinf_ncsnpp_profile(self._h, 1 if enable else 0), "natinf_ncsnpp_profile")

    def profile_read(self):
        ms = (C.c_double * 4)()
        n = (C.c_int64 * 4)()
        check(lib.natinf_ncsnpp_profile_read(self._h, ms, n), "natinf_ncsnpp_profile_read")
        return {"gemm": (ms[0], n[0]), "other": (ms[1], n[1]), "conv_gn": (ms[2], n[2]), "conv_gn8": (ms[3], n[3])}

    def describe_gemms(self, B: int):
        buf = C.create_string_buffer(1 << 16)
        n = lib.natinf_ncsnpp_describe_gemms(self._h, B, buf, len(buf))
        if n < 0:
            check(n, "natinf_ncsnpp_describe_gemms")
        rows = []
        for line in buf.value.decode().strip().split("\n"):
            f = line.split()
            rows.append((*map(int, f[:6]), f[6]))
        return rows

    def tap(self, module_idx: int, shape) -> torch.Tensor:
        out = torch.empty(shape, dtype=torch.float32, device=self.device)
        check(lib.natinf_ncsnpp_debug_tap(self._h, module_idx, ptr(out), out.numel(), stream_ptr()), "natinf_ncsnpp_debug_tap")
        return out

    def __del__(self):
        h = getattr(self, "_h", None)
        if h:
            lib.natinf_ncsnpp_destroy(h)
            self._h = None
```

naturaldiffusion_amd/sampler.py:

```python
from __future__ import annotations

import math
from typing import Callable, Optional

import numpy as np
import torch

from . import _lib
from ._lib import lib, check, ptr, stream_ptr
from .coeff import SparseRows, is_stochastic


def vp_std_f32(t: float, beta_0: float = 0.1, beta_1: float = 20.0) -> float:
    vt = torch.ones(1, dtype=torch.float32) * t
    lmc = -0.25 * vt ** 2 * (beta_1 - beta_0) - 0.5 * vt * beta_0
    return float(torch.sqrt(1.0 - torch.exp(2.0 * lmc))[0])


def image_index_args(index, n_images: int, device):
    if index is None:
        return None, 0, 1
    if isinstance(index, torch.Tensor):
        if (index.dtype != torch.int64 or index.device != device or not index.is_contiguous()
                or index.numel() != n_images):
# ... 309 lines not shown

    def step(self, k: int, x_k: torch.Tensor, model_out: torch.Tensor, noise: torch.Tensor,
             x_next: Optional[torch.Tensor] = None, index=None, elems_per_image: Optional[int] = None, *,
             known: Optional[torch.Tensor] = None, mask: Optional[torch.Tensor] = None, known_final: str = "mean",
             gray_u: Optional[torch.Tensor] = None) -> torch.Tensor:
        epi = self.epi if elems_per_image is None else int(elems_per_image)
        inpaint = known is not None or mask is not None
        if self.x0_mode:
            check_x0_fix(self.x0_fix, self.x0_ratio, self.x0_max, seed=self.seed, elems_per_image=epi, gray=gray_u is not None)
            _check_elems_per_image(epi, self.E)
        if gray_u is not None:
            if inpaint:
                raise ValueError("gray_u (colorization) does not go with known / mask (inpainting)")
            gs = check_gray(gray_u, self.E, epi, seed=self.seed, fast_f32=self.fast, device=x_k.device)
            ga, gstd, gcol = self._color_level(k + 1, known_final)
        if inpaint:
            ks, ms = check_known(known, mask, self.E, epi, seed=self.seed, fast_f32=self.fast, device=x_k.device)
            ka, kstd, kcol = self._known_level(k + 1, known_final)
        if x_next is None:
            x_next = _pingpong(self._x, k, x_k)
        for t in (x_k, model_out, noise):
            if t.dtype != torch.float32 or t.numel() != self.E or not t.is_contiguous():
                raise ValueError("x_k / model_out / noise must be contiguous fp32 tensors of n_elem elements")
        idx, val, n = self.rows.ptrs(k)
        r = self.rows.rows[k]
        a, s = float(self.node[k, 1]), float(self.node[k, 2])
        if inpaint or gray_u is not None or self.stochastic or self.x0_mode:
            if epi is None:
                raise ValueError("stochastic NI matrix: elems_per_image is needed to key the injected noise")
            ib, vb, nb = self._noise_rows().ptrs(k)
            index, first, stride = image_index_args(index, self.E // epi, x_k.device)
        if self.x0_mode:
            n_images = self.E // epi
            if self.x0_s is None or self.x0_s.shape[1] != n_images:
                self.x0_s = torch.zeros((self.n_step, n_images), dtype=torch.float64, device=self.device)
            kargs = (ptr(known), ptr(mask), ks, ms, ka, kstd, kcol) if inpaint else (0, 0, 0, 0, 0.0, 0.0, 0)
            check(lib.natinf_step_f64hist_x0fix(ptr(x_k), ptr(model_out), ptr(noise), ptr(self.hist), ptr(x_next), idx, val, n,
                                                r.diag, ib, vb, nb, k, a, s, self.std[k], self.seed, ptr(index), first, stride,
                                                epi, self.E, *kargs, self.x0_mode, self.x0_ratio, self.x0_max, ptr(self.x0_s[k]),
                                                stream_ptr()), "natinf_step_f64hist_x0fix")
            return x_next
        if inpaint:
            check(lib.natinf_step_f64hist_inpaint(ptr(x_k), ptr(model_out), ptr(noise), ptr(self.hist), ptr(x_next), idx, val, n,
                                                  r.diag, ib, vb, nb, k, a, s, self.std[k], self.seed, ptr(index), first, stride,
                                                  epi, self.E, ptr(known), ptr(mask), ks, ms, ka, kstd, kcol, stream_ptr()),
                  "natinf_step_f64hist_inpaint")
            return x_next
        if gray_u is not None:
            check(lib.natinf_step_f64hist_colorize(ptr(x_k), ptr(model_out), ptr(noise), ptr(self.hist), ptr(x_next), idx, val, n,
                                                   r.diag, ib, vb, nb, k, a, s, self.std[k], self.seed, ptr(index), first, stride,
                                                   epi, self.E, ptr(gray_u), gs, _f9(COLOR_M), _f9(COLOR_W), ga, gstd, gcol, stream_ptr()),
                  "natinf_step_f64hist_colorize")
            return x_next
        if self.stochastic:
            check(lib.natinf_step_f64hist_noise(ptr(x_k), ptr(model_out), ptr(noise), ptr(self.hist), ptr(x_next), idx, val, n,
                                                r.diag, ib, vb, nb, k, a, s, self.std[k], self.seed, ptr(index), first, stride,
                                                epi, self.E, stream_ptr()), "natinf_step_f64hist_noise")
            return x_next
        b0 = float(np.float32(self.B[k, 0]))
        fn = lib.natinf_step_f32hist if self.fast else lib.natinf_step_f64hist
        check(fn(ptr(x_k), ptr(model_out), ptr(noise), ptr(self.hist), ptr(x_next), idx, val, n, r.diag, k,
                 a, s, self.std[k], b0, self.E, stream_ptr()), "natinf_step_f64hist")
        return x_next

    def run(self, model_fn: Callable, noise: torch.Tensor, return_all: bool = False, index=None, *,
            known: Optional[torch.Tensor] = None, mask: Optional[torch.Tensor] = None, known_final: str = "mean",
            gray_u: Optional[torch.Tensor] = None):
        shape, B = noise.shape, noise.shape[0]
        noise = noise.contiguous()
        epi = self.epi if self.epi is not None else noise.numel() // B
        inpaint = known is not None or mask is not None
        if gray_u is not None and inpaint:
            raise ValueError("gray_u (colorization) does not go with known / mask (inpainting)")
        if self.x0_mode:
            check_x0_fix(self.x0_fix, self.x0_ratio, self.x0_max, seed=self.seed, elems_per_image=epi, gray=gray_u is not None)
        kw = dict(index=index, elems_per_image=epi) if self.stochastic or inpaint or gray_u is not None or self.x0_mode else {}
        if gray_u is not None:
            kw.update(gray_u=gray_u.reshape(-1), known_final=known_final)
        elif inpaint:
            flat = lambda t: t if t is None else (t.view(torch.uint8) if t.dtype == torch.bool else t).reshape(-1)
            kw.update(known=flat(known), mask=flat(mask), known_final=known_final)
        x = self.first_input(noise, **kw) if inpaint or gray_u is not None else noise
        xs = [x.view(shape)]
        for k in range(self.n_step):
            labels = torch.full((B,), self.labels[k], dtype=torch.float32, device=self.device)
            out = model_fn(x.view(shape), labels)
            x = self.step(k, x.reshape(-1), out.contiguous().reshape(-1), noise.reshape(-1), **kw)
            if return_all:
                x = x.clone()
                xs.append(x.view(shape))
        return xs if return_all else x.view(shape)


class ValidateNI:

    def __init__(self, C: np.ndarray, B: np.ndarray, node: np.ndarray, c1: np.ndarray, c2: np.ndarray, n_elem: int,
                 device="cuda:0", dense: bool = False, *, seed: Optional[int] = None, elems_per_image: Optional[int] = None):
        _lib.require_gpu()
        if n_elem % 4:
            raise ValueError("element count must be a multiple of 4")
        self.n_step = int(np.asarray(B).shape[0])
        self.node = np.asarray(node, np.float64)
        self.E = int(n_elem)
        self.device = torch.device(device)
        self.seed = None if seed is None else int(seed) & (2 ** 64 - 1)
        if elems_per_image is not None:
            if seed is None:
                raise ValueError("elems_per_image belongs to the seeded (in-kernel noise) form: give a seed")
            _check_elems_per_image(elems_per_image, self.E)
        self.epi = None if elems_per_image is None else int(elems_per_image)
        self.rows_c = SparseRows(C, lambda k: k + 1, torch.float32, self.device, dense=dense)
        self.rows_b = SparseRows(B, lambda k: min(k + 2, np.asarray(B).shape[1]), torch.float32, self.device, dense=dense, diag=False)
        self.c1 = [float(np.float32(v)) for v in c1]
        self.c2 = [float(np.float32(v)) for v in c2]
        self.hist_x0 = torch.empty((self.n_step, self.E), dtype=torch.float32, device=self.device)
        self.hist_eps = None if self.seed is not None else torch.empty((self.n_step + 1, self.E), dtype=torch.float32, device=self.device)
        self._z = [torch.empty(self.E, dtype=torch.float32, device=self.device) for _ in range(2)]
        self._known_level = _level_memo(lambda known_final: known_schedule(self.node, known_final))
        self._launch_wide = {}

    def _launch_wide_guidance(self, n: int, cfg: float, have_uncond: bool):
        key = (n, float(cfg), bool(have_uncond))
        if key not in self._launch_wide:
            slots = torch.arange(n, dtype=torch.int32) if have_uncond else torch.full((n,), -1, dtype=torch.int32)
            self._launch_wide[key] = (torch.full((n,), float(cfg), dtype=torch.float32).to(self.device), slots.to(self.device))
        return self._launch_wide[key]

    def first_input(self, noise: torch.Tensor, known: torch.Tensor, mask: torch.Tensor, index=None, known_final: str = "mean",
                    elems_per_image: Optional[int] = None) -> torch.Tensor:
        epi = self.epi if elems_per_image is None else int(elems_per_image)
        return _known_blend_f32(_flat_noise_f32(noise, self.E), known, mask, self.E, epi, self.seed, self._known_level, known_final, index)

    def step(self, k: int, z: torch.Tensor, cond: torch.Tensor, uncond: Optional[torch.Tensor], cfg,
             sample_elems: Optional[int] = None, eps_sample_stride: Optional[int] = None, *,
             noise: Optional[torch.Tensor] = None, index=None, uncond_slot: Optional[torch.Tensor] = None,
             n_uncond: Optional[int] = None, known: Optional[torch.Tensor] = None, mask: Optional[torch.Tensor] = None,
             known_final: str = "mean") -> torch.Tensor:
        se = self.E if sample_elems is None else int(sample_elems)
        st = se if eps_sample_stride is None else int(eps_sample_stride)
        guided = isinstance(cfg, torch.Tensor)
        inpaint = known is not None or mask is not None
        if inpaint:
            if self.seed is None:
                raise ValueError("known / mask belong to the seeded form: the slab form has no blend")
            ks, ms = check_known(known, mask, self.E, se, seed=self.seed, device=z.device)
            ka, kstd, kcol = self._known_level(k + 1, known_final)
        if guided and (self.seed is None or noise is None):
            raise ValueError("a tensor cfg (per-image scales) belongs to the seeded form with noise= / index=: the slab form takes one float")
        if not guided and (uncond_slot is not None or n_uncond is not None):
            raise ValueError("uncond_slot / n_uncond go with a tensor cfg (per-image scales)")
        z_next = _pingpong(self._z, k, z)
        ic, vc, nc = self.rows_c.ptrs(k)
        ib, vb, nb = self.rows_b.ptrs(k)
        if self.seed is None:
            if noise is not None or index is not None:
                raise ValueError("noise / index belong to the seeded form; without a seed the noises are read from hist_eps")
            check(lib.natinf_step_f32prod(ptr(z), ptr(cond), ptr(uncond), float(cfg), se, st, ptr(self.hist_x0),
                                          ptr(self.hist_eps), ptr(z_next), ic, vc, nc, self.rows_c.rows[k].diag,
                                          ib, vb, nb, k, self.c1[k], self.c2[k], self.E, stream_ptr()), "natinf_step_f32prod")
            return z_next
        if noise is None:
            raise ValueError("seeded form: step needs the initial noise (noise=); there is no hist_eps slab to read it from")
        if noise.dtype != torch.float32 or noise.numel() != self.E or not noise.is_contiguous() or noise.device != z.device:
            raise ValueError("noise must be a contiguous fp32 tensor of n_elem elements on the sampler's device")
        if se <= 0 or se % 4 or self.E % se or (self.epi is not None and se != self.epi):
            raise ValueError("sample_elems must be the per-image element count: a multiple of 4 dividing the element count"
                             + ("" if self.epi is None else f" (elems_per_image = {self.epi})"))
        index, first, stride = image_index_args(index, self.E // se, z.device)
# ... 142 lines not shown
```

Baseline: 3631 images/s.

## Fuse GN finalize into attention and skip paths, cache scalar-t time embedding

Adds a scalar-timestep forward path. It computes the time-embedding row once per distinct t, keeps it in a small device cache, and broadcasts it to the GEMM epilogues (row stride 0) in place of per-sample embedding rows. The 16x16 attention block kernel now also finalizes the following GroupNorm scale and shift itself, and a new batched kernel finalizes several skip-connection GroupNorm halves in one launch. The aim is to cut kernel launches and redundant per-sample time-embedding work. In exchange it adds cache state across calls, which assumes the weights do not change while a key is cached, plus extra synchronisation inside the attention kernel.

```diff
diff --git a/include/natinf_ncsnpp.h b/include/natinf_ncsnpp.h
--- a/include/natinf_ncsnpp.h
+++ b/include/natinf_ncsnpp.h
@@ -31,6 +31,8 @@
 
 int natinf_ncsnpp_forward(natinf_ncsnpp_t h, const float* x, const float* labels, float* out, int B,
                           void* workspace, int64_t workspace_bytes, natinf_stream_t stream);
+int natinf_ncsnpp_forward_t(natinf_ncsnpp_t h, const float* x, float t, float* out, int B,
+                            void* workspace, int64_t workspace_bytes, natinf_stream_t stream);
 
 int natinf_ncsnpp_describe_gemms(natinf_ncsnpp_t h, int B, char* buf, int cap);
 
@@ -59,6 +61,7 @@
 #define NATINF_ATTN_BLOCK_OFF_WVO_PACKED 1181696
 #define NATINF_ATTN_BLOCK_PACKED_BYTES 1312768
 #define NATINF_ATTN_BLOCK_SCRATCH_BYTES_PER_SAMPLE 393216
+int natinf_debug_attn_fin(float* fin_scale, float* fin_shift, const float* gamma, const float* beta, float mul);
 int natinf_debug_attn_block(int plan, int B, const void* x, int x_ld, const float* scale, const float* shift, const float* w, const float* bias,
                             void* packed, void* scratch, void* out, int o_ld, float out_scale, float* gn_part, natinf_stream_t stream);
 int natinf_set_gemm_variant(int variant);
@@ -106,6 +109,8 @@
                           natinf_stream_t stream);
 int natinf_debug_gn_finalize(const float* P0, int tps0, int quads0, const float* P1, int tps1, int quads1, int C, int HW, int B, const float* gamma, const float* beta,
                              float* scale, float* shift, float eps, float out_mul, natinf_stream_t stream);
+int natinf_debug_gn_finalize_skips(int n, const float* const* P, const int* tps, const int* quads, const int* coff, const int* C, const int* HW, const float* const* gamma,
+                                   const float* const* beta, float* const* scale, float* const* shift, const float* out_mul, int B, float eps, natinf_stream_t stream);
 int natinf_debug_gn_fold(const float* P, int tps, int quads, int fold, int B, float* out, natinf_stream_t stream);
 int natinf_debug_gn_apply(const void* x, int ld, int C, int logW, int logHW, int B, const float* scale, const float* shift, void* y, void* xr, int act, int mode, int pad,
                           natinf_stream_t stream);
diff --git a/naturaldiffusion_amd/_lib.py b/naturaldiffusion_amd/_lib.py
--- a/naturaldiffusion_amd/_lib.py
+++ b/naturaldiffusion_amd/_lib.py
@@ -71,6 +71,7 @@
     "natinf_ncsnpp_load": (C.c_int, [_p, _p, _i64, _p, _i64, _p]),
     "natinf_ncsnpp_share": (C.c_int, [_p, _p]),
     "natinf_ncsnpp_forward": (C.c_int, [_p, _p, _p, _p, _i32, _p, _i64, _p]),
+    "natinf_ncsnpp_forward_t": (C.c_int, [_p, _p, _f32, _p, _i32, _p, _i64, _p]),
     "natinf_ncsnpp_debug_tap": (C.c_int, [_p, _i32, _p, _i64, _p]),
     "natinf_ncsnpp_describe_gemms": (C.c_int, [_p, _i32, C.c_char_p, _i32]),
     "natinf_debug_gemm": (C.c_int, [_i32, _i32, _i32, _i32, _i32, _i32, _i32, _i32, _p, _p, _p, _p, _p, _i32, _f32, _i32, _p]),
@@ -97,6 +98,8 @@
     "natinf_set_fuse_gn8": (C.c_int, [_i32]),
     "natinf_set_fuse_gn4": (C.c_int, [_i32]),
     "natinf_set_fuse_fin": (C.c_int, [_i32]),
+    "natinf_debug_attn_fin": (C.c_int, [_p, _p, _p, _p, _f32]),
+    "natinf_debug_gn_finalize_skips": (C.c_int, [_i32, _p, _p, _p, _p, _p, _p, _p, _p, _p, _p, _p, _i32, _f32, _p]),
     "natinf_set_attn_proj": (C.c_int, [_i32]),
     "natinf_set_attn_waves8": (C.c_int, [_i32]),
     "natinf_set_attn_qkv": (C.c_int, [_i32]),
diff --git a/naturaldiffusion_amd/csrc/attn_blk256.h b/naturaldiffusion_amd/csrc/attn_blk256.h
--- a/naturaldiffusion_amd/csrc/attn_blk256.h
+++ b/naturaldiffusion_amd/csrc/attn_blk256.h
@@ -343,7 +343,9 @@
 
 __global__ __launch_bounds__(512, 1) void k_attn_blk256_v2(const bf16* __restrict__ x, int x_ld, const float* __restrict__ gsc, const float* __restrict__ gsh,
                                                           const bf16* __restrict__ wqf, const float* __restrict__ cq, float scale, const bf16* __restrict__ wvof,
-                                                          const float* __restrict__ bo, bf16* __restrict__ o, int o_ld, float out_scale, float2* __restrict__ gn_part, int gn_quads)
+                                                          const float* __restrict__ bo, bf16* __restrict__ o, int o_ld, float out_scale, float2* __restrict__ gn_part, int gn_quads,
+                                                          float* __restrict__ fin_scale, float* __restrict__ fin_shift, const float* __restrict__ fin_gamma,
+                                                          const float* __restrict__ fin_beta, float fin_mul, float fin_eps)
 {
     constexpr int T = 256, C = 256, NTQ = 8;
     extern __shared__ __attribute__((aligned(16))) unsigned char smem[];
@@ -599,6 +601,24 @@
 #pragma unroll
             for (int w = 0; w < 8; ++w) { s += sred[w * 64 + tid].x; ss += sred[w * 64 + tid].y; }
             gn_part[(int64_t)b * gn_quads + tid] = make_float2(s, ss);
+            if (fin_scale) sred[512 + tid] = make_float2(s, ss);
+        }
+        if (fin_scale) {
+            __syncthreads();
+            if (tid < C) {
+                constexpr int cg = C >> 5, qpg = cg >> 2;
+                const float inv = 1.0f / (float)(cg * T);
+                const int gi = tid / cg;
+                float s = 0.f, q2 = 0.f;
+#pragma unroll
+                for (int i = 0; i < qpg; ++i) { float2 v = sred[512 + gi * qpg + i]; float ts = 0.f, tq = 0.f; ts += v.x; tq += v.y; s += ts; q2 += tq; }
+                const float mean = s * inv;
+                float var = q2 * inv - mean * mean;
+                var = var < 0.f ? 0.f : var;
+                const float sc = (1.0f / sqrtf(var + fin_eps)) * fin_gamma[tid];
+                fin_scale[(int64_t)b * C + tid] = sc * fin_mul;
+                fin_shift[(int64_t)b * C + tid] = (fin_beta[tid] - mean * sc) * fin_mul;
+            }
         }
     }
 }
diff --git a/naturaldiffusion_amd/csrc/engine_core.h b/naturaldiffusion_amd/csrc/engine_core.h
--- a/naturaldiffusion_amd/csrc/engine_core.h
+++ b/naturaldiffusion_amd/csrc/engine_core.h
@@ -31,6 +31,7 @@
     hipStream_t stream2 = nullptr; hipEvent_t* ev = nullptr;
     unsigned char* fin_done = nullptr;
     uint32_t* guard = nullptr;
+    const float* temb_row = nullptr;
     uint32_t* site(int i) const { return guard ? guard + 2 * i : nullptr; }
     bf16* act(const TRef& t) const { return reinterpret_cast<bf16*>(ws + t.off * B) + t.coff; }
     template <class T> T* at(int64_t off) const { return reinterpret_cast<T*>(ws + off * B); }
diff --git a/naturaldiffusion_amd/csrc/gemm_launch.h b/naturaldiffusion_amd/csrc/gemm_launch.h
--- a/naturaldiffusion_amd/csrc/gemm_launch.h
+++ b/naturaldiffusion_amd/csrc/gemm_launch.h
@@ -24,6 +24,7 @@
                     void launch_fp8(const void* gemm_args, int mxa, int w128, int raster, void* stream); void launch_splitk_reduce(const void* gemm_args, int slices, void* stream);
                     void launch_patch_embed(const float* z, const float* Wt, const float* bias, const float* pos, float* x, int C, int g, int D, int64_t rows, int x_f16, uint32_t* guard, void* stream); }
 namespace ncsn_upf { bool configure(); void launch(const void* gemm_args, int epi, void* stream); void fold(const float* w, void* dst_bf16, float* dst_f32, int N, int Cin, float wmul, void* stream); }
+namespace ncsn_gns { void launch(const void* gn_skip_args, int n, int B, float eps, void* stream); }
 namespace ncsn_cg3 { bool configure(); int tile_rows(int shape); int tile_cols(int shape); void launch(const void* gemm_args, int shape, int epi, void* stream); }
 
 namespace {
diff --git a/naturaldiffusion_amd/csrc/gn_skips.hip b/naturaldiffusion_amd/csrc/gn_skips.hip
--- /dev/null
+++ b/naturaldiffusion_amd/csrc/gn_skips.hip
@@ -0,0 +1,56 @@
+#include <hip/hip_runtime.h>
+#include <stdint.h>
+#include <string.h>
+#include <type_traits>
+
+namespace {
+#include "ncsnpp_kernels.h"
+}
+using namespace ncsn;
+
+namespace {
+__global__ __launch_bounds__(256) void k_gn_finalize_skips(GnSkipArgs a, float eps)
+{
+    __shared__ float2 s_p[128];
+    lds_poison();
+    const GnSkipDesc& d = a.d[blockIdx.y];
+    const int tid = threadIdx.x, b = blockIdx.x, nc = 4 * d.quads;
+    float ga[2] = {0.f, 0.f}, be[2] = {0.f, 0.f};
+#pragma unroll
+    for (int k = 0; k < 2; ++k) {
+        const int c = tid + 256 * k;
+        if (c < nc) { ga[k] = d.gamma[d.coff + c]; be[k] = d.beta[d.coff + c]; }
+    }
+    for (int q = tid; q < d.quads; q += 256) {
+        const float2* P = d.part + (int64_t)b * d.tps * d.quads + q;
+        float s = 0.f, qq = 0.f;
+        for (int t = 0; t < d.tps; ++t) { const float2 v = P[(int64_t)t * d.quads]; s += v.x; qq += v.y; }
+        s_p[q] = make_float2(s, qq);
+    }
+    __syncthreads();
+    const int cg = d.C >> 5, qpg = cg >> 2;
+    const float inv = 1.0f / (float)(cg * d.HW);
+#pragma unroll
+    for (int k = 0; k < 2; ++k) {
+        const int c = tid + 256 * k;
+        if (c >= nc) break;
+        const int gi = c / cg;
+        float s = 0.f, q = 0.f;
+        for (int i = 0; i < qpg; ++i) { const float2 v = s_p[gi * qpg + i]; s += v.x; q += v.y; }
+        const float mean = s * inv;
+        float var = q * inv - mean * mean;
+        var = var < 0.f ? 0.f : var;
+        const float sc = (1.0f / sqrtf(var + eps)) * ga[k];
+        d.scale[(int64_t)b * d.C + d.coff + c] = sc * d.out_mul;
+        d.shift[(int64_t)b * d.C + d.coff + c] = (be[k] - mean * sc) * d.out_mul;
+    }
+}
+}
+
+namespace ncsn_gns {
+__attribute__((visibility("hidden"))) void launch(const void* gn_skip_args, int n, int B, float eps, void* stream) {
+    GnSkipArgs a;
+    memcpy(&a, gn_skip_args, sizeof(a));
+    hipLaunchKernelGGL(k_gn_finalize_skips, dim3((unsigned)B, (unsigned)n), dim3(256), 0, reinterpret_cast<hipStream_t>(stream), a, eps);
+}
+}
diff --git a/naturaldiffusion_amd/csrc/ncsnpp.hip b/naturaldiffusion_amd/csrc/ncsnpp.hip
--- a/naturaldiffusion_amd/csrc/ncsnpp.hip
+++ b/naturaldiffusion_amd/csrc/ncsnpp.hip
@@ -39,7 +39,7 @@
 int g_attn_w8 = 1;
 int g_attn_proj = 1;
 int g_fuse_gn8 = 1;
-int g_fuse_fin = 3;
+int g_fuse_fin = 15;
 int g_fuse_gn4 = 1;
 int g_fuse_gn = 1;
 constexpr int UP_FOLD_DEFAULT = 1;
@@ -60,6 +60,17 @@
     uint64_t plan_sig = 0;
     int last_B = 0; unsigned char* last_ws = nullptr;
     std::vector<unsigned char> fin_done;
+    std::function<void(hipStream_t, const unsigned char* wp, const float* labels, int M, bf16* emb, bf16* t1, bf16* t2, float* dout, int phase)> temb;
+    int dense_total = 0;
+    struct TembCache {
+        static constexpr int SLOTS = 64;
+        unsigned char* dev = nullptr;
+        uint32_t key[SLOTS];
+        uint64_t filled = 0;
+        hipStream_t stream = nullptr;
+        void clear() { filled = 0; }
+        int find(uint32_t k) const { const int n = filled < SLOTS ? (int)filled : SLOTS; for (int i = 0; i < n; ++i) if (key[i] == k) return i; return -1; }
+    } tcache;
 };
 
 namespace {
@@ -84,6 +95,7 @@
     const bf16* wqf2 = nullptr; const float* cq2 = nullptr; const bf16* wvof2 = nullptr; const float* bo2 = nullptr;
     bf16* out = nullptr; int o_ld = 0; float out_scale = 1.0f;
     float2* gn_part = nullptr; int gn_quads = 0;
+    float* fin_scale = nullptr; float* fin_shift = nullptr; const float* fin_gamma = nullptr; const float* fin_beta = nullptr; float fin_mul = 1.0f;
 };
 void pack_attn_qkv_w(const float* w0, const float* w1, const float* w2, bf16* wqkvf, hipStream_t s) {
     hipLaunchKernelGGL(k_pack_qkv_w, dim3(3 * 256), dim3(256), 0, s, w0, w1, w2, wqkvf);
@@ -102,7 +114,8 @@
     constexpr int C = 256;
     if (a.plan == 2) {
         hipLaunchKernelGGL(k_attn_blk256_v2, dim3((unsigned)a.B), dim3(512), ABLK2_LDS_BYTES, s, a.x, a.x_ld, a.sc, a.sh,
-                           a.wqf2, a.cq2, 1.0f / sqrtf((float)C), a.wvof2, a.bo2, a.out, a.o_ld, a.out_scale, a.gn_part, a.gn_quads);
+                           a.wqf2, a.cq2, 1.0f / sqrtf((float)C), a.wvof2, a.bo2, a.out, a.o_ld, a.out_scale, a.gn_part, a.gn_quads,
+                           a.gn_part ? a.fin_scale : (float*)nullptr, a.fin_shift, a.fin_gamma, a.fin_beta, a.fin_mul, GN_EPS);
         return 256;
     }
     if (a.plan == 1) {
@@ -251,7 +264,7 @@
             if (fold_up) {
                 g.a0 = c.act(h); g.a0_ld = h.ld; g.a0_padded = 1; g.a0_C = cin; g.taps = 4; g.logW = logW - 1; g.logHW = logHW - 2;
                 g.M = c.B * (HWo / 4); g.N = 4 * cout; g.b = c.w<bf16>(w0); g.b_ld = 4 * cin; g.bias_n = c.w<float>(b0);
-                g.rowvec = c.at<float>(dout) + drow; g.rowvec_ld = dtotal; g.log_rows_per_sample = logHW - 2;
+                g.rowvec = (c.temb_row ? c.temb_row : c.at<float>(dout)) + drow; g.rowvec_ld = c.temb_row ? 0 : dtotal; g.log_rows_per_sample = logHW - 2;
                 g.c = c.act(t); g.c_ld = t.ld;
                 if (pt.valid) { g.gn_part = c.at<float>(pt.off); g.gn_quads = pt.quads; }
                 const int bm = launch_gemm(g, c.stream);
@@ -264,7 +277,7 @@
             g.M = c.B * HWo; g.N = cout; g.b = c.w<bf16>(w0); g.b_ld = K0a;
             if (w0f >= 0) g.b_frag = c.w<bf16>(w0f);
             g.bias_n = c.w<float>(b0);
-            g.rowvec = c.at<float>(dout) + drow; g.rowvec_ld = dtotal; g.log_rows_per_sample = logHW;
+            g.rowvec = (c.temb_row ? c.temb_row : c.at<float>(dout)) + drow; g.rowvec_ld = c.temb_row ? 0 : dtotal; g.log_rows_per_sample = logHW;
             if (skws >= 0) { g.splitk_ws = c.at<float>(skws); g.splitk_max = SK_MAX; }
             g.c = c.act(t); g.c_ld = t.ld;
             if (pt.valid) { g.gn_part = c.at<float>(pt.off); g.gn_quads = pt.quads; set_fin(g, pt, c); }
@@ -388,7 +401,7 @@
                                reinterpret_cast<float*>(p.packed + bo_), reinterpret_cast<bf16*>(p.packed + wq_), reinterpret_cast<bf16*>(p.packed + wv_), p.stream);
             });
         }
-        const Part po_attn = proj ? register_output(out) : Part();
+        const Part po_attn = proj ? register_output(out, false, blk2) : Part();
         const float rs_attn = res_scale;
         TRef O = new_act(m.res, C);
         if (T == 256 && C == 256) {
@@ -402,6 +415,10 @@
                     if (blk2) { a.wqf2 = c.w<bf16>(wqf2); a.cq2 = c.w<float>(cq2); a.wvof2 = c.w<bf16>(wvof2); a.bo2 = c.w<float>(bo2); }
                     a.out = c.act(out); a.o_ld = out.ld; a.out_scale = rs_attn;
                     if (po_attn.valid) { a.gn_part = c.at<float2>(po_attn.off); a.gn_quads = po_attn.quads; }
+                    if (po_attn.fin && po_attn.fin->claimed) {
+                        const Fin& f = *po_attn.fin;
+                        a.fin_scale = c.at<float>(f.sc); a.fin_shift = c.at<float>(f.sh); a.fin_gamma = c.w<float>(f.gamma); a.fin_beta = c.w<float>(f.beta); a.fin_mul = f.out_mul;
+                    }
                     const int rows = launch_attn_blk256(a, c.stream);
                     if (po_attn.valid) c.part_bm[po_attn.id] = rows;
                 }
@@ -524,8 +541,12 @@
 
     int dense_rows_next = 0;
 
-    struct Fin { int64_t sc = -1, sh = -1, gamma = -1, beta = -1; int C = 0; float out_mul = 1.0f; bool claimed = false, check = false; };
+    struct Fin { int64_t sc = -1, sh = -1, gamma = -1, beta = -1; int C = 0; float out_mul = 1.0f; bool claimed = false, check = false, wide = false; };
     struct Part { int64_t off = -1; int quads = 0, id = -1, res = 0; bool valid = false; std::shared_ptr<Fin> fin; };
+    struct CatTab { int64_t sc = -1, sh = -1; int C = 0, ch_h = 0, res = 0; bool claimed = false; };
+    std::map<int64_t, CatTab> cat_tabs;
+    struct SkipHalf { Part p; int64_t gamma, beta, sc, sh; int C, coff, HW; float out_mul; };
+    std::shared_ptr<std::vector<SkipHalf>> skip_halves = std::make_shared<std::vector<SkipHalf>>();
     static void set_fin(GemmArgs& g, const Part& p, const Ctx& c) {
         if (!p.fin || !p.fin->claimed) return;
         const Fin& f = *p.fin;
@@ -540,16 +561,21 @@
         p.off = arena.alloc((int64_t)std::max(res * res / 64, 1) * p.quads * 8);
         return p;
     }
-    Part register_output(const TRef& out, bool fused8 = false) {
+    Part register_output(const TRef& out, bool fused8 = false, bool attn_fin = false) {
         Part p;
         if (fusable(out.res) || (out.res <= 8 && fused8)) p = new_part(out.res, out.C);
-        if (p.valid && out.res <= 8 && fused8 && (g_fuse_fin & 1) && out.C == 256) {
+        const bool fin8 = p.valid && out.res <= 8 && fused8 && (g_fuse_fin & 1) && out.C == 256;
+        const bool fin16 = p.valid && out.res == 16 && fused8 && (g_fuse_fin & 2) && out.C == 256 && !ddpm;
+        const bool fin_a = p.valid && attn_fin && out.res == 16 && out.C == 256 && (g_fuse_fin & 8) && !ddpm;
+        if (fin8 || fin16 || fin_a) {
             p.fin = std::make_shared<Fin>();
-            p.fin->sc = arena.alloc((int64_t)out.C * 4); p.fin->sh = arena.alloc((int64_t)out.C * 4); p.fin->C = out.C;
-        }
-        if (p.valid && out.res == 16 && fused8 && (g_fuse_fin & 2) && out.C == 256 && !ddpm) {
-            p.fin = std::make_shared<Fin>();
-            p.fin->sc = arena.alloc((int64_t)out.C * 4); p.fin->sh = arena.alloc((int64_t)out.C * 4); p.fin->C = out.C; p.fin->check = true;
+            p.fin->check = fin16;
+            const auto ct = (out.coff == 0 && !fin_a) ? cat_tabs.find(out.off) : cat_tabs.end();
+            if (ct != cat_tabs.end() && ct->second.ch_h == out.C && ct->second.res == out.res) {
+                p.fin->sc = ct->second.sc; p.fin->sh = ct->second.sh; p.fin->C = ct->second.C; p.fin->wide = true;
+            } else {
+                p.fin->sc = arena.alloc((int64_t)out.C * 4); p.fin->sh = arena.alloc((int64_t)out.C * 4); p.fin->C = out.C;
+            }
         }
         parts[{out.off, out.coff}] = p;
         return p;
@@ -581,6 +607,23 @@
             }
             return true;
         }
+        if (src.size() == 2 && p0.fin && !p0.fin->claimed && p0.fin->wide && p0.fin->C == C && (p0.quads + p1.quads) * 4 == C) {
+            Fin& f = *p0.fin;
+            f.gamma = gn.gamma; f.beta = gn.beta; f.out_mul = out_mul; f.claimed = true;
+            sc = f.sc; sh = f.sh;
+            cat_tabs[x.off].claimed = true;
+            skip_halves->push_back(SkipHalf{p1, gn.gamma, gn.beta, f.sc, f.sh, C, p0.quads * 4, HW, out_mul});
+            if (f.check) {
+                const int64_t fsc = f.sc, fsh = f.sh;
+                op(CLS_OTHER, [=](const Ctx& c) {
+                    if (c.fin_done[p0.id]) return;
+                    hipLaunchKernelGGL(k_gn_finalize, dim3(c.B), dim3(256), 0, c.stream, c.at<float2>(p0.off), HW / c.part_bm[p0.id], p0.quads,
+                                       c.at<float2>(p1.off), HW / c.part_bm[p1.id], p1.quads, C, HW,
+                                       c.w<float>(gn.gamma), c.w<float>(gn.beta), c.at<float>(fsc), c.at<float>(fsh), GN_EPS, out_mul);
+                });
+            }
+            return true;
+        }
         const int64_t sc_ = sc, sh_ = sh;
         op(CLS_OTHER, [=](const Ctx& c) {
             const int tps0 = HW / c.part_bm[p0.id], tps1 = p1.valid ? HW / c.part_bm[p1.id] : 0;
@@ -657,25 +700,37 @@
             pack_conv(pw0, w0, TEMB, NF, 1, NF, 0, NF); pack_conv(pw1, w1, TEMB, TEMB, 1, TEMB, 0, TEMB);
             const int64_t b0 = pack_f32(pb0, TEMB), b1 = pack_f32(pb1, TEMB);
             const int64_t dw = dense_w, db = dense_b, dout = dense_out; const int dtot = dense_total;
+            E.dense_total = dense_total;
+            E.temb = [=](hipStream_t s, const unsigned char* wp, const float* labels, int M, bf16* e_, bf16* t1_, bf16* t2_, float* dout_, int phase) {
+                auto w = [&](int64_t off) { return wp + off; };
+                if (phase == 0) {
+                    hipLaunchKernelGGL(k_time_embed, dim3(grid1d((int64_t)M * 128, 256, 1 << 30)), dim3(256), 0, s, labels, e_, M);
+                    return;
+                }
+                GemmArgs g = gemm_defaults();
+                g.a0 = e_; g.a0_ld = NF; g.a0_C = NF; g.M = M; g.N = TEMB;
+                g.b = reinterpret_cast<const bf16*>(w(w0)); g.b_ld = NF; g.bias_n = reinterpret_cast<const float*>(w(b0)); g.act = ACT_SILU;
+                g.c = t1_; g.c_ld = TEMB;
+                launch_gemm(g, s);
+                g = gemm_defaults();
+                g.a0 = t1_; g.a0_ld = TEMB; g.a0_C = TEMB; g.M = M; g.N = TEMB;
+                g.b = reinterpret_cast<const bf16*>(w(w1)); g.b_ld = TEMB; g.bias_n = reinterpret_cast<const float*>(w(b1)); g.act = ACT_SILU;
+                g.c = t2_; g.c_ld = TEMB;
+                launch_gemm(g, s);
+                g = gemm_defaults();
+                g.a0 = t2_; g.a0_ld = TEMB; g.a0_C = TEMB; g.M = M; g.N = dtot;
+                g.b = reinterpret_cast<const bf16*>(w(dw)); g.b_ld = TEMB; g.bias_n = reinterpret_cast<const float*>(w(db));
+                g.c = dout_; g.c_ld = dtot; g.c_mode = OUT_F32;
+                launch_gemm(g, s);
+            };
+            natinf_ncsnpp* const eng = &E;
             op(CLS_OTHER, [=](const Ctx& c) {
-                hipLaunchKernelGGL(k_time_embed, dim3(grid1d((int64_t)c.B * 128, 256, 1 << 30)), dim3(256), 0, c.stream, c.labels, c.at<bf16>(emb), c.B);
+                if (c.temb_row) return;
+                eng->temb(c.stream, c.wp, c.labels, c.B, c.at<bf16>(emb), c.at<bf16>(t1), c.at<bf16>(t2), c.at<float>(dout), 0);
             });
             op(CLS_GEMM, [=](const Ctx& c) {
-                GemmArgs g = gemm_defaults();
-                g.a0 = c.at<bf16>(emb); g.a0_ld = NF; g.a0_C = NF; g.M = c.B; g.N = TEMB;
-                g.b = c.w<bf16>(w0); g.b_ld = NF; g.bias_n = c.w<float>(b0); g.act = ACT_SILU;
-                g.c = c.at<bf16>(t1); g.c_ld = TEMB;
-                launch_gemm(g, c.stream);
-                g = gemm_defaults();
-                g.a0 = c.at<bf16>(t1); g.a0_ld = TEMB; g.a0_C = TEMB; g.M = c.B; g.N = TEMB;
-                g.b = c.w<bf16>(w1); g.b_ld = TEMB; g.bias_n = c.w<float>(b1); g.act = ACT_SILU;
-                g.c = c.at<bf16>(t2); g.c_ld = TEMB;
-                launch_gemm(g, c.stream);
-                g = gemm_defaults();
-                g.a0 = c.at<bf16>(t2); g.a0_ld = TEMB; g.a0_C = TEMB; g.M = c.B; g.N = dtot;
-                g.b = c.w<bf16>(dw); g.b_ld = TEMB; g.bias_n = c.w<float>(db);
-                g.c = c.at<float>(dout); g.c_ld = dtot; g.c_mode = OUT_F32;
-                launch_gemm(g, c.stream);
+                if (c.temb_row) return;
+                eng->temb(c.stream, c.wp, c.labels, c.B, c.at<bf16>(emb), c.at<bf16>(t1), c.at<bf16>(t2), c.at<float>(dout), 1);
             });
         }
         int si = 0;
@@ -729,6 +784,33 @@
                 cur = dst; res /= 2;
             }
         }
+        if ((g_fuse_fin & 4) && !ddpm) {
+            for (const Cat& ct : cats) {
+                const int C = ct.ch_h + ct.ch_s, cg = C / 32;
+                if (ct.buf.res > 16 || C % 32 || C > 512 || cg % 4 || ct.ch_h % cg || ct.ch_s % cg || ct.ch_h != 256) continue;
+                const auto sp = parts.find({ct.buf.off, ct.ch_h});
+                if (sp == parts.end() || !sp->second.valid || sp->second.res != ct.buf.res || sp->second.quads * 4 != ct.ch_s) continue;
+                CatTab t; t.C = C; t.ch_h = ct.ch_h; t.res = ct.buf.res;
+                t.sc = arena.alloc((int64_t)C * 4); t.sh = arena.alloc((int64_t)C * 4);
+                cat_tabs[ct.buf.off] = t;
+            }
+            const std::shared_ptr<std::vector<SkipHalf>> halves = skip_halves;
+            op(CLS_OTHER, [=](const Ctx& c) {
+                for (size_t i0 = 0; i0 < halves->size(); i0 += GN_SKIP_MAX) {
+                    GnSkipArgs a;
+                    memset(&a, 0, sizeof(a));
+                    const int n = (int)std::min<size_t>(GN_SKIP_MAX, halves->size() - i0);
+                    for (int i = 0; i < n; ++i) {
+                        const SkipHalf& h = (*halves)[i0 + i];
+                        GnSkipDesc& d = a.d[i];
+                        d.part = c.at<float2>(h.p.off); d.gamma = c.w<float>(h.gamma); d.beta = c.w<float>(h.beta);
+                        d.scale = c.at<float>(h.sc); d.shift = c.at<float>(h.sh);
+                        d.tps = h.HW / c.part_bm[h.p.id]; d.quads = h.p.quads; d.C = h.C; d.coff = h.coff; d.HW = h.HW; d.out_mul = h.out_mul;
+                    }
+                    ncsn_gns::launch(&a, n, c.B, GN_EPS, (void*)c.stream);
+                }
+            });
+        }
         {
             TRef a = new_act(res, cur.C), b = new_act(res, cur.C);
             emit_res(M[mi++], cur, a);
@@ -746,6 +828,10 @@
                 TRef in = cats[j].buf;
                 TRef dst = level_end ? new_act(res, m.cout) : h_slot(j + 1);
                 emit_res(m, in, dst);
+                if (const auto ct = cat_tabs.find(in.off); ct != cat_tabs.end()) {
+                    if (!ct->second.claimed) { arena.release(ct->second.sc); arena.release(ct->second.sh); }
+                    cat_tabs.erase(ct);
+                }
                 arena.release(cats[j].buf.off);
                 last = dst; ++j;
             }
@@ -883,6 +969,7 @@
     if (!h) return NATINF_EINVAL;
     for (auto& r : h->recs) { (void)hipEventDestroy(r.a); (void)hipEventDestroy(r.b); }
     for (auto e : h->pool) (void)hipEventDestroy(e);
+    if (h->tcache.dev) (void)hipFree(h->tcache.dev);
     delete h;
     return NATINF_OK;
 }
@@ -903,7 +990,9 @@
 
 int natinf_ncsnpp_load(natinf_ncsnpp_t h, const float* params_f32, int64_t n_params, void* packed, int64_t packed_bytes,
                        natinf_stream_t stream) {
-    return h ? h->load(params_f32, n_params, packed, packed_bytes, (hipStream_t)stream) : NATINF_EINVAL;
+    if (!h) return NATINF_EINVAL;
+    h->tcache.clear();
+    return h->load(params_f32, n_params, packed, packed_bytes, (hipStream_t)stream);
 }
 
 int natinf_ncsnpp_share(natinf_ncsnpp_t h, natinf_ncsnpp_t loaded) {
@@ -913,12 +1002,13 @@
         h->packs.size() != loaded->packs.size() || h->plan_sig != loaded->plan_sig)
         return NATINF_EINVAL;
     h->packed = loaded->packed;
+    h->tcache.clear();
     return NATINF_OK;
 }
 
-int natinf_ncsnpp_forward(natinf_ncsnpp_t h, const float* x, const float* labels, float* out, int B, void* workspace,
+static int ncsnpp_forward(natinf_ncsnpp_t h, const float* x, const float* labels, float temb_t, float* out, int B, void* workspace,
                           int64_t workspace_bytes, natinf_stream_t stream) {
-    if (!h || !x || !labels || !out || !workspace || B <= 0) return NATINF_EINVAL;
+    if (!h || !x || !out || !workspace || B <= 0) return NATINF_EINVAL;
     if (!h->packed) return NATINF_ESTATE;
     if (workspace_bytes < h->ws_per_image * (int64_t)B || (int64_t)B * IMG * IMG >= (1LL << 31)) return NATINF_EINVAL;
     if (!h->configured) {
@@ -928,6 +1018,25 @@
     Ctx c{B, reinterpret_cast<unsigned char*>(workspace), h->packed, (hipStream_t)stream, x, labels, out, h->part_bm.data()};
     c.fin_done = h->fin_done.data();
     g_launch_error = 0;
+    if (!labels) {
+        auto& tc = h->tcache;
+        const int64_t row_bytes = (int64_t)h->dense_total * 4, rows_bytes = row_bytes * tc.SLOTS;
+        if (!tc.dev && hipMalloc(reinterpret_cast<void**>(&tc.dev), (size_t)(rows_bytes + 256 + (NF + 2 * TEMB) * 2)) != hipSuccess) { tc.dev = nullptr; (void)hipGetLastError(); return NATINF_ENODEV; }
+        if (tc.stream != c.stream) { tc.clear(); tc.stream = c.stream; }
+        uint32_t key; memcpy(&key, &temb_t, 4);
+        int slot = tc.find(key);
+        if (slot < 0) {
+            slot = (int)(tc.filled % tc.SLOTS);
+            float* lab = reinterpret_cast<float*>(tc.dev + rows_bytes);
+            bf16* emb = reinterpret_cast<bf16*>(tc.dev + rows_bytes + 256);
+            float* row = reinterpret_cast<float*>(tc.dev + slot * row_bytes);
+            hipLaunchKernelGGL(k_fill_f32, dim3(1), dim3(64), 0, c.stream, lab, temb_t, (int64_t)1);
+            h->temb(c.stream, h->packed, lab, 1, emb, emb + NF, emb + NF + TEMB, row, 0);
+            h->temb(c.stream, h->packed, lab, 1, emb, emb + NF, emb + NF + TEMB, row, 1);
+            tc.key[slot] = key; ++tc.filled;
+        }
+        c.temb_row = reinterpret_cast<const float*>(tc.dev + slot * row_bytes);
+    }
     if (!h->prof) {
         for (const auto& f : h->ops) f(c);
     } else {
@@ -946,6 +1055,17 @@
     h->last_B = B; h->last_ws = c.ws;
     if (g_launch_error) { g_launch_error = 0; return NATINF_ESTATE; }
     return hipGetLastError() == hipSuccess ? NATINF_OK : NATINF_ELAUNCH;
+}
+
+int natinf_ncsnpp_forward(natinf_ncsnpp_t h, const float* x, const float* labels, float* out, int B, void* workspace,
+                          int64_t workspace_bytes, natinf_stream_t stream) {
+    if (!labels) return NATINF_EINVAL;
+    return ncsnpp_forward(h, x, labels, 0.f, out, B, workspace, workspace_bytes, stream);
+}
+
+int natinf_ncsnpp_forward_t(natinf_ncsnpp_t h, const float* x, float t, float* out, int B, void* workspace,
+                            int64_t workspace_bytes, natinf_stream_t stream) {
+    return ncsnpp_forward(h, x, nullptr, t, out, B, workspace, workspace_bytes, stream);
 }
 
 int natinf_ncsnpp_describe_gemms(natinf_ncsnpp_t h, int B, char* buf, int cap) {
@@ -1102,6 +1222,13 @@
     return hipGetLastError() == hipSuccess ? NATINF_OK : NATINF_ELAUNCH;
 }
 
+float* g_dbg_afin_scale = nullptr; float* g_dbg_afin_shift = nullptr; const float* g_dbg_afin_gamma = nullptr; const float* g_dbg_afin_beta = nullptr; float g_dbg_afin_mul = 1.0f;
+int natinf_debug_attn_fin(float* fin_scale, float* fin_shift, const float* gamma, const float* beta, float mul) {
+    if (fin_scale && (!fin_shift || !gamma || !beta)) return NATINF_EINVAL;
+    g_dbg_afin_scale = fin_scale; g_dbg_afin_shift = fin_shift; g_dbg_afin_gamma = gamma; g_dbg_afin_beta = beta; g_dbg_afin_mul = mul;
+    return NATINF_OK;
+}
+
 int natinf_debug_attn_block(int plan, int B, const void* x, int x_ld, const float* scale, const float* shift, const float* w, const float* bias,
                             void* packed, void* scratch, void* out, int o_ld, float out_scale, float* gn_part, natinf_stream_t stream) {
     if (plan < 0 || plan > 2 || B < 1 || !x || !scale || !shift || !w || !bias || !packed || !out || x_ld < 256 || x_ld % 8 || o_ld < 256 || o_ld % 8 ||
@@ -1114,6 +1241,10 @@
     AttnBlk256 a;
     a.plan = plan; a.B = B; a.x = (const bf16*)x; a.x_ld = x_ld; a.sc = scale; a.sh = shift;
     a.out = (bf16*)out; a.o_ld = o_ld; a.out_scale = out_scale; a.gn_part = reinterpret_cast<float2*>(gn_part); a.gn_quads = 64;
+    if (g_dbg_afin_scale) {
+        if (plan != 2 || !gn_part) return NATINF_EINVAL;
+        a.fin_scale = g_dbg_afin_scale; a.fin_shift = g_dbg_afin_shift; a.fin_gamma = g_dbg_afin_gamma; a.fin_beta = g_dbg_afin_beta; a.fin_mul = g_dbg_afin_mul;
+    }
     if (plan == 2) {
         float* fq = reinterpret_cast<float*>(pk + NATINF_ATTN_BLOCK_OFF_FOLD_WQK); float* fv = reinterpret_cast<float*>(pk + NATINF_ATTN_BLOCK_OFF_FOLD_WVO);
         float* cq = reinterpret_cast<float*>(pk + NATINF_ATTN_BLOCK_OFF_FOLD_CQ); float* bo = reinterpret_cast<float*>(pk + NATINF_ATTN_BLOCK_OFF_FOLD_BO);
@@ -1172,9 +1303,9 @@
 int natinf_set_attn_waves8(int on) { g_attn_w8 = on != 0; return NATINF_OK; }
 int natinf_set_attn_proj(int on) { g_attn_proj = on != 0; return NATINF_OK; }
 int natinf_set_fuse_fin(int on) {
-    if (on < 0 || on > 3) return NATINF_EINVAL;
+    if (on < 0 || on > 15 || (on > 3 && !(on & 3))) return NATINF_EINVAL;
     static const int mask[4] = {0, 3, 1, 2};
-    g_fuse_fin = mask[on];
+    g_fuse_fin = on <= 3 ? mask[on] : on;
     return NATINF_OK;
 }
 int natinf_set_gemm_round_model(int on) { g_round_model = on != 0; g_round_model_w128 = on >= 10 ? on : 13; return NATINF_OK; }
@@ -1285,6 +1416,21 @@
     return hipGetLastError() == hipSuccess ? NATINF_OK : NATINF_ELAUNCH;
 }
 
+int natinf_debug_gn_finalize_skips(int n, const float* const* P, const int* tps, const int* quads, const int* coff, const int* C, const int* HW, const float* const* gamma,
+                                   const float* const* beta, float* const* scale, float* const* shift, const float* out_mul, int B, float eps, natinf_stream_t stream) {
+    if (n < 1 || n > GN_SKIP_MAX || !P || !tps || !quads || !coff || !C || !HW || !gamma || !beta || !scale || !shift || !out_mul || B < 1) return NATINF_EINVAL;
+    GnSkipArgs a;
+    memset(&a, 0, sizeof(a));
+    for (int i = 0; i < n; ++i) {
+        const int cg = C[i] / 32;
+        if (!P[i] || !gamma[i] || !beta[i] || !scale[i] || !shift[i] || tps[i] < 1 || quads[i] < 1 || HW[i] < 1 || dbg_misaligned(P[i], 8)) return NATINF_EINVAL;
+        if (C[i] < 128 || C[i] > 512 || C[i] % 128 || quads[i] > 128 || coff[i] < 0 || coff[i] % cg || (4 * quads[i]) % cg || coff[i] + 4 * quads[i] > C[i]) return NATINF_EINVAL;
+        a.d[i] = GnSkipDesc{reinterpret_cast<const float2*>(P[i]), gamma[i], beta[i], scale[i], shift[i], tps[i], quads[i], C[i], coff[i], HW[i], out_mul[i]};
+    }
+    ncsn_gns::launch(&a, n, B, eps, (void*)stream);
+    return hipGetLastError() == hipSuccess ? NATINF_OK : NATINF_ELAUNCH;
+}
+
 int natinf_debug_gn_apply(const void* x, int ld, int C, int logW, int logHW, int B, const float* scale, const float* shift, void* y, void* xr, int act, int mode, int pad,
                           natinf_stream_t stream) {
     if (!x || !scale || !shift || !y || B < 1 || B > 65535 || C < 8 || C % 8 || (C >> 3) > 256 || ld < C || ld % 8) return NATINF_EINVAL;
diff --git a/naturaldiffusion_amd/csrc/ncsnpp_kernels.h b/naturaldiffusion_amd/csrc/ncsnpp_kernels.h
--- a/naturaldiffusion_amd/csrc/ncsnpp_kernels.h
+++ b/naturaldiffusion_amd/csrc/ncsnpp_kernels.h
@@ -524,6 +524,10 @@
     }
 }
 
+constexpr int GN_SKIP_MAX = 16;
+struct GnSkipDesc { const float2* part; const float* gamma; const float* beta; float* scale; float* shift; int tps, quads, C, coff, HW; float out_mul; };
+struct GnSkipArgs { GnSkipDesc d[GN_SKIP_MAX]; };
+
 enum { RS_NONE = 0, RS_UP = 1, RS_DOWN = 2 };
 constexpr int GN_ROWS = 4;
 #ifndef GN_UNROLL
diff --git a/naturaldiffusion_amd/ncsnpp.py b/naturaldiffusion_amd/ncsnpp.py
--- a/naturaldiffusion_amd/ncsnpp.py
+++ b/naturaldiffusion_amd/ncsnpp.py
@@ -142,13 +142,19 @@
         other.workspace_bytes = ws
         return other
 
-    def __call__(self, x: torch.Tensor, labels: torch.Tensor, out: torch.Tensor = None) -> torch.Tensor:
+    def __call__(self, x: torch.Tensor, labels, out: torch.Tensor = None) -> torch.Tensor:
         if x.dtype != torch.float32 or x.dim() != 4 or tuple(x.shape[1:]) != (3, 32, 32) or not x.is_cuda:
             raise ValueError("x must be a CUDA fp32 tensor of shape [B,3,32,32]")
         B = x.shape[0]
         if B > self.max_batch:
             raise ValueError(f"batch {B} exceeds max_batch {self.max_batch}")
         x = x.contiguous()
+        if isinstance(labels, (float, int)):
+            if out is None:
+                out = torch.empty_like(x)
+            check(lib.natinf_ncsnpp_forward_t(self._h, ptr(x), float(labels), ptr(out), B, ptr(self._ws), self._ws.numel(),
+                                              stream_ptr()), "natinf_ncsnpp_forward_t")
+            return out
         labels = labels.to(x.device, torch.float32).contiguous()
         if labels.numel() != B:
             raise ValueError("labels must have one entry per sample")
diff --git a/naturaldiffusion_amd/sampler.py b/naturaldiffusion_amd/sampler.py
--- a/naturaldiffusion_amd/sampler.py
+++ b/naturaldiffusion_amd/sampler.py
@@ -415,8 +415,10 @@
             kw.update(known=flat(known), mask=flat(mask), known_final=known_final)
         x = self.first_input(noise, **kw) if inpaint or gray_u is not None else noise
         xs = [x.view(shape)]
+        from .ncsnpp import NCSNppEngine
+        scalar_label = isinstance(model_fn, NCSNppEngine)
         for k in range(self.n_step):
-            labels = torch.full((B,), self.labels[k], dtype=torch.float32, device=self.device)
+            labels = self.labels[k] if scalar_label else torch.full((B,), self.labels[k], dtype=torch.float32, device=self.device)
             out = model_fn(x.view(shape), labels)
             x = self.step(k, x.reshape(-1), out.contiguous().reshape(-1), noise.reshape(-1), **kw)
             if return_all:
```

Result: no change. 3649 images/s, median of 6 (+0.5%).
